# marekvinkler/NTrace

Hardware: AMD Instinct MI355X
Metric: Mrays/sec (primary + 8xAO) on Crytek Sponza (higher is better)
Workload: dtype f32

## Files before the change

include/ntrace_amd.h:

```cpp
#ifndef NTRACE_AMD_H
#define NTRACE_AMD_H

#include <stddef.h>
#include <stdint.h>

#ifdef __cplusplus
extern "C" {
#endif

#define NTR_API __attribute__((visibility("default")))

typedef enum NtrStatus {
    NTR_OK = 0,
    NTR_ERR_INVALID = -1,
    NTR_ERR_NO_DEVICE = -2,
    NTR_ERR_HIP = -3,
    NTR_ERR_LAYOUT = -4,
    NTR_ERR_UNKNOWN_KERNEL = -5,
    NTR_ERR_OVERFLOW = -6,
    NTR_ERR_NOMEM = -7
} NtrStatus;

typedef enum NtrBVHLayout {
    NTR_BVHLayout_AOS_AOS = 0,
    NTR_BVHLayout_AOS_SOA,
    NTR_BVHLayout_SOA_AOS,
    NTR_BVHLayout_SOA_SOA,
    NTR_BVHLayout_Compact,
    NTR_BVHLayout_Compact2,
    NTR_BVHLayout_CPU,
    NTR_BVHLayout_Max
} NtrBVHLayout;

typedef struct NtrKernelConfig {
    int32_t bvhLayout;
    int32_t blockWidth;
    int32_t blockHeight;
    int32_t usePersistentThreads;
} NtrKernelConfig;

typedef struct NtrRay {
    float ox, oy, oz, tmin;
    float dx, dy, dz, tmax;
} NtrRay;

typedef struct NtrRayResult {
    int32_t id;
    float   t;
    int32_t padA;
    int32_t padB;
} NtrRayResult;


NTR_API const char* ntr_last_error(void);
NTR_API int         ntr_version(void);

NTR_API int ntr_device_count(int* count);
NTR_API int ntr_set_device(int device);
NTR_API int ntr_malloc(void** d_ptr, size_t bytes);
NTR_API int ntr_free(void* d_ptr);
NTR_API int ntr_memcpy_h2d(void* d_dst, const void* h_src, size_t bytes, void* stream);
NTR_API int ntr_memcpy_d2h(void* h_dst, const void* d_src, size_t bytes, void* stream);
NTR_API int ntr_memcpy_d2d(void* d_dst, const void* d_src, size_t bytes, void* stream);
NTR_API int ntr_memset(void* d_dst, int value, size_t bytes, void* stream);
NTR_API int ntr_stream_synchronize(void* stream);


NTR_API int ntr_query_config(const char* kernelName, NtrKernelConfig* config);

NTR_API int ntr_trace_bvh(const char* kernelName, int32_t numRays, int32_t anyHit,
                          const NtrRay* d_rays, NtrRayResult* d_results,
                          const void* d_nodes, int64_t nodesBytes,
                          const void* d_triWoop, int64_t triWoopBytes, const int32_t* d_triIndex,
                          int32_t layout, uint32_t bvhFlags, void* stream, float* seconds);

NTR_API int ntr_trace_status(void* stream, uint32_t* statusBits);

NTR_API int ntr_selftest_gather_rate(int64_t tableBytes, int32_t waves, int32_t lanesPerWave, int32_t steps, void* stream, float* seconds);

NTR_API int ntr_trace_graph_reserve(int32_t launches, int32_t numRays);
NTR_API int ntr_trace_graph_release_all(void);

NTR_API int ntr_stream_release(void* stream);

NTR_API int ntr_selftest_auto_hint_table(int32_t devices, int32_t keysPerDevice, int32_t rounds, int32_t* hintedLastRound);

typedef struct NtrTracePlan {
    int32_t variant;
    int32_t launchVariant;
    int32_t launchBlocks;
    int32_t numBlocks;
    int32_t orderBlocks;
    int32_t chunk, fetchThreshold, leafSwitchBelow, octant, flatFetch, uniformPrologue, splitSlice;
    int32_t numHeads, shardRays, numBlocksIncoherent;
    int32_t numBlocksDivergent;
    int32_t wholeWave;
    int32_t prefetchAfter;
    int32_t unified;
    int32_t minipool;
    int32_t poolKConst;
    int32_t poolKFromDevice;
    int32_t minipoolWide;
    int32_t hintable;
    int32_t useAutoHint;
    int32_t predictable;
    int32_t persistentOrder;
    int32_t probeOnRefresh;
    int32_t coherentRoute;
    int32_t persistentVariant, persistentBlocks, persistentFetchThreshold;
    int32_t perrayBlocks, perrayFetchThreshold;
} NtrTracePlan;
#define NTR_PLAN_FLAG_STATS 1
#define NTR_PLAN_FLAG_CAPTURING 2
#define NTR_PLAN_FLAG_CALLER_HINT 4
NTR_API int ntr_trace_plan(const char* kernelName, int32_t numRays, int32_t anyHit, uint64_t nodesAddr, int64_t nodesBytes,
                           uint64_t triWoopAddr, int64_t triWoopBytes, uint32_t bvhFlags, int32_t numCUs, int32_t flags,
                           NtrTracePlan* plan);
NTR_API int ntr_trace_plan_hint_step(int32_t valid, int32_t predicted, int32_t uses, int32_t out[3]);
NTR_API int ntr_trace_plan_certain(int32_t anyHit, int32_t out[2]);

NTR_API int ntr_tunables_reload(void);

typedef struct NtrSchedHint NtrSchedHint;
NTR_API int ntr_sched_hint_create(NtrSchedHint** out);
NTR_API int ntr_sched_hint_destroy(NtrSchedHint* hint);
NTR_API int ntr_sched_hint_reset(NtrSchedHint* hint);
NTR_API int ntr_trace_bvh_hinted(const char* kernelName, int32_t numRays, int32_t anyHit,
                                 const NtrRay* d_rays, NtrRayResult* d_results,
                                 const void* d_nodes, int64_t nodesBytes,
                                 const void* d_triWoop, int64_t triWoopBytes, const int32_t* d_triIndex,
                                 int32_t layout, uint32_t bvhFlags, void* stream, float* seconds,
                                 NtrSchedHint* hint);

NTR_API int ntr_sched_hint_predict(NtrSchedHint* hint, const uint32_t* d_blockCost, int32_t numBlocks, void* stream);
NTR_API int ntr_bvh_leaf_depths(const void* d_nodes, int64_t nodesBytes, const void* d_triWoop, int64_t triWoopBytes,
                                const int32_t* d_triIndex, int32_t numTris, int32_t* d_depthByTri, int32_t* levels, void* stream);
NTR_API int ntr_secondary_block_costs(const NtrRayResult* d_inResults, int32_t first, int32_t count, int32_t numSamples,
                                      const int32_t* d_depthByTri, int32_t numTris, uint32_t* d_blockCost, void* stream);

NTR_API int ntr_predict_block_costs(int32_t numRays, const NtrRay* d_rays, const void* d_nodes, int64_t nodesBytes,
                                    uint32_t* d_blockCost, void* stream);

NTR_API int ntr_predict_batch_coherence(int32_t numRays, const NtrRay* d_rays, const void* d_nodes, int64_t nodesBytes,
                                        uint32_t* d_out, void* stream);

NTR_API int ntr_predict_dispatch_order(int32_t numRays, const NtrRay* d_rays, const void* d_nodes, int64_t nodesBytes,
                                       uint32_t* d_order, uint32_t* d_word, void* stream);

typedef struct {
    int32_t numBlocks;
    int32_t device;
    int32_t uses;
    int32_t valid;
    int32_t predicted;
} NtrSchedHintState;
NTR_API int ntr_sched_hint_inspect(const NtrSchedHint* hint, NtrSchedHintState* state, uint32_t* h_order, uint32_t* h_cost, void* stream);

typedef struct NtrTraceStats {
    int64_t numRays;
    int64_t numInnerVisits;
    int64_t numTriTests;
    int64_t numLeafVisits;
    int64_t numHits;
} NtrTraceStats;

NTR_API int ntr_trace_bvh_stats(const char* kernelName, int32_t numRays, int32_t anyHit,
                                const NtrRay* d_rays, NtrRayResult* d_results,
                                const void* d_nodes, int64_t nodesBytes,
                                const void* d_triWoop, int64_t triWoopBytes, const int32_t* d_triIndex,
                                int32_t layout, uint32_t bvhFlags, void* stream, NtrTraceStats* stats);

#define NTR_BVH_FINITE 1u
#define NTR_BVH_FASTDIV 2u
#define NTR_BVH_NOTINY 4u
#define NTR_BVH_ORDERED 8u
#define NTR_BVH_WIDE_LEAVES 16u
#define NTR_BATCH_DIVERGENT 0x10000u
NTR_API int ntr_bvh_validate(const void* d_nodes, int64_t nodesBytes, uint32_t* flags, void* stream);

NTR_API int ntr_selftest_division(const float* d_x, int32_t nx, const float* d_d, int32_t nd,
                                  uint32_t* mismatches, void* stream);
NTR_API int ntr_selftest_division_hard(int32_t xExp, int32_t dExp, uint64_t* pairs, uint64_t* mismatches, void* stream);


NTR_API int ntr_pixel_table(int32_t w, int32_t h, int32_t* d_indexToPixel, int32_t* d_pixelToIndex, void* stream);

NTR_API int ntr_raygen_primary(NtrRay* d_rays, int32_t* d_idToSlot, int32_t* d_slotToID,
                               const int32_t* d_indexToPixel, const float origin[3],
                               const float nscreenToWorld[16], int32_t w, int32_t h, float maxDist,
                               uint32_t kernelSeed, void* stream);

NTR_API int ntr_raygen_ao(NtrRay* d_outRays, int32_t* d_outIDToSlot, int32_t* d_outSlotToID,
                          const NtrRay* d_inRays, const NtrRayResult* d_inResults,
                          const float* d_triNormals, int32_t firstInputSlot, int32_t numInputRays,
                          int32_t numSamples, float maxDist, uint32_t kernelSeed, void* stream);

NTR_API int ntr_raygen_shadow(NtrRay* d_outRays, int32_t* d_outIDToSlot, int32_t* d_outSlotToID, const NtrRay* d_inRays,
                              const NtrRayResult* d_inResults, int32_t firstInputSlot, int32_t numInputRays, int32_t numSamples,
                              const float lightPos[3], float lightRadius, uint32_t kernelSeed, void* stream);

NTR_API int ntr_count_hits(const NtrRayResult* d_results, int32_t numRays, int32_t* count, void* stream);


typedef struct NtrLbvhResult {
    int32_t numNodes, numLeaves, numLevels, pad;
    int64_t nodesBytes, triWoopBytes, triIndexBytes;
    float   seconds;
    float   mortonMs, sortMs, woopMs, emitMs, refitMs;
} NtrLbvhResult;

NTR_API int ntr_lbvh_capacity(int32_t numTris, int64_t* nodesBytes, int64_t* triWoopBytes, int64_t* triIndexBytes);

NTR_API int ntr_lbvh_build(int32_t numTris, const int32_t* d_triVtxIndex, int32_t numVerts, const float* d_vtxPos,
                           const float sceneMin[3], const float sceneMax[3], int32_t leafSize, float epsilon,
                           void* d_nodes, int64_t nodesCapacity, void* d_triWoop, int64_t triWoopCapacity,
                           int32_t* d_triIndex, int64_t triIndexCapacity, NtrLbvhResult* result, void* stream);

typedef struct NtrHlbvhResult {
    NtrLbvhResult lbvh;
    int32_t numClusters, topNodes, topLevels, pad;
    float   clusterMs, topMs, bottomMs, pad2;
} NtrHlbvhResult;

NTR_API int ntr_hlbvh_build(int32_t numTris, const int32_t* d_triVtxIndex, int32_t numVerts, const float* d_vtxPos,
                            const float sceneMin[3], const float sceneMax[3], int32_t leafSize, float epsilon, int32_t hlbvhBits,
                            void* d_nodes, int64_t nodesCapacity, void* d_triWoop, int64_t triWoopCapacity,
                            int32_t* d_triIndex, int64_t triIndexCapacity, NtrHlbvhResult* result, void* stream);

NTR_API int ntr_lbvh_release_workspace(void);

typedef struct NtrPersistentBvhParams {
    int32_t triLimit, triMaxLimit, maxDepth, pad;
    float   ci, ct, epsilon, pad2;
} NtrPersistentBvhParams;
typedef struct NtrPersistentBvhResult {
    int32_t numNodes, numLeaves, numLevels, maxDepth;
    int32_t medianFallbacks, costLeaves, depthLeaves, pad;
    int64_t nodesBytes, triWoopBytes, triIndexBytes;
    float   seconds;
    float   prepMs, levelsMs, emitMs;
} NtrPersistentBvhResult;
NTR_API int ntr_persistent_bvh_params_default(NtrPersistentBvhParams* params);
NTR_API int ntr_persistent_bvh_build(int32_t numTris, const int32_t* d_triVtxIndex, int32_t numVerts, const float* d_vtxPos,
                                     const float sceneMin[3], const float sceneMax[3], const NtrPersistentBvhParams* params,
                                     void* d_nodes, int64_t nodesCapacity, void* d_triWoop, int64_t triWoopCapacity,
                                     int32_t* d_triIndex, int64_t triIndexCapacity, NtrPersistentBvhResult* result, void* stream);
NTR_API int ntr_persistent_bvh_scratch_bytes(int64_t* bytes);

typedef struct NtrSahDeviceResult {
    int32_t numNodes, numLeaves, numLevels, maxDepth;
    int32_t numDropped, pad[3];
    int64_t nodesBytes, triWoopBytes, triIndexBytes;
    float   seconds;
    float   prepMs, sortMs, levelsMs, emitMs;
} NtrSahDeviceResult;
NTR_API int ntr_sah_device_build(int32_t numTris, const int32_t* d_triVtxIndex, int32_t numVerts, const float* d_vtxPos,
                                 int32_t minLeafSize, int32_t maxLeafSize, void* d_nodes, int64_t nodesCapacity, void* d_triWoop,
                                 int64_t triWoopCapacity, int32_t* d_triIndex, int64_t triIndexCapacity, NtrSahDeviceResult* result,
                                 void* stream);
NTR_API int ntr_sah_device_scratch_bytes(int64_t* bytes);

typedef struct NtrBvhRefitResult {
    int32_t numNodes, numLeaves, numRows, pad;
    float   seconds;
} NtrBvhRefitResult;
NTR_API int ntr_bvh_refit(void* d_nodes, int64_t nodesBytes, void* d_triWoop, int64_t triWoopBytes,
                          const int32_t* d_triIndex, int64_t triIndexBytes,
                          int32_t numTris, const int32_t* d_triVtxIndex, int32_t numVerts, const float* d_vtxPos,
                          float epsilon, float* d_sceneBox ,
                          NtrBvhRefitResult* result , void* stream);
NTR_API int ntr_bvh_refit_scratch_bytes(int64_t* bytes);

typedef struct NtrBvhOptimizeResult {
    int32_t passes, numNodes, numLeafLinks, pad;
    int32_t formed[8], rewritten[8];
    int32_t heightBefore[8], heightAfter[8];
    float   seconds;
} NtrBvhOptimizeResult;
NTR_API int ntr_bvh_optimize(void* d_nodes, int64_t nodesBytes, int32_t passes, NtrBvhOptimizeResult* result ,
                             void* stream);
NTR_API int ntr_bvh_optimize_scratch_bytes(int64_t* bytes);

typedef struct NtrBvhSahResult {
    float   sahCost;
    int32_t numNodes, numLeaves, numTris, height;
    float   seconds;
} NtrBvhSahResult;
NTR_API int ntr_bvh_sah_cost(const void* d_nodes, int64_t nodesBytes, const void* d_triWoop, int64_t triWoopBytes,
                             NtrBvhSahResult* result, void* stream);

typedef struct NtrBvhReorderResult {
    int64_t nodesBytes, triWoopBytes, triIndexBytes;
    int32_t numNodes, numLeaves, numRows, numDroppedSlots;
    float   seconds;
} NtrBvhReorderResult;
NTR_API int ntr_bvh_reorder(const void* d_nodes, int64_t nodesBytes, const void* d_triWoop, int64_t triWoopBytes,
                            const int32_t* d_triIndex, int64_t triIndexBytes,
                            void* d_outNodes, int64_t outNodesCapacity, void* d_outTriWoop, int64_t outTriWoopCapacity,
                            int32_t* d_outTriIndex, int64_t outTriIndexCapacity,
                            NtrBvhReorderResult* result, void* stream);
NTR_API int ntr_bvh_reorder_scratch_bytes(int64_t* bytes);

NTR_API int ntr_reconstruct(int32_t rayType, int32_t numRaysPerPrimary, int32_t firstPrimary, int32_t numPrimary,
                            const int32_t* d_primarySlotToID, const NtrRayResult* d_primaryResults,
                            const int32_t* d_batchIDToSlot, const NtrRayResult* d_batchResults,
                            const uint32_t* d_triMaterialColor, const uint32_t* d_triShadedColor,
                            uint32_t* d_pixels, void* stream);

NTR_API int ntr_ray_morton_sort(int32_t numRays, const NtrRay* d_inRays, const int32_t* d_inSlotToID,
                                NtrRay* d_outRays, int32_t* d_outIDToSlot, int32_t* d_outSlotToID,
                                void* stream, float* seconds);

typedef struct NtrDist NtrDist;
#define NTR_DIST_ID_BYTES 128
NTR_API int ntr_frame_shard(int32_t numPrimary, int32_t rank, int32_t world, int32_t align, int32_t* lo, int32_t* hi);
NTR_API int ntr_frame_ao_batches(int32_t lo, int32_t hi, int32_t samples, int32_t maxBatchRays, int32_t* first, int32_t* count,
                                 int32_t capacity, int32_t* numBatches);
NTR_API int ntr_dist_unique_id(char id[NTR_DIST_ID_BYTES]);
NTR_API int ntr_dist_init(const char id[NTR_DIST_ID_BYTES], int32_t rank, int32_t world, NtrDist** out);
NTR_API int ntr_dist_init_all(int32_t numDevices, const int32_t* devices, NtrDist** out );
NTR_API int ntr_dist_info(const NtrDist* dist, int32_t* rank, int32_t* world);
NTR_API int ntr_dist_destroy(NtrDist* dist);
NTR_API int ntr_dist_broadcast(NtrDist* dist, void* d_buf, int64_t bytes, int32_t root, void* stream);
NTR_API int ntr_dist_broadcast_bvh(NtrDist* dist, void* d_nodes, int64_t nodesBytes, void* d_triWoop, int64_t triWoopBytes,
                                   int32_t* d_triIndex, int64_t triIndexBytes, int32_t root, void* stream);
NTR_API int ntr_dist_gather_records(NtrDist* dist, const NtrRayResult* d_ownRecords, int32_t numPrimary, int32_t align,
                                    NtrRayResult* d_fullRecords, int32_t root, void* stream);
NTR_API int ntr_dist_gather_records_cuts(NtrDist* dist, const NtrRayResult* d_ownRecords, const int32_t* cuts ,
                                         NtrRayResult* d_fullRecords, int32_t root, void* stream);
NTR_API int ntr_dist_gather_pixels(NtrDist* dist, const uint32_t* d_ownPixels, const int32_t* d_slotToPixel, int32_t numPrimary,
                                   int32_t align, uint32_t* d_fullPixels, uint32_t* d_scratch, int32_t root, void* stream);


typedef struct NtrHostBvh NtrHostBvh;
typedef struct NtrHostBvhInfo {
    const void*    nodes;     int64_t nodesBytes;
    const void*    triWoop;   int64_t triWoopBytes;
    const int32_t* triIndex;  int64_t triIndexBytes;
    int32_t layout;
    int32_t numInnerNodes, numLeafNodes, maxDepth;
    float   buildSeconds;
} NtrHostBvhInfo;
NTR_API int  ntr_sah_build(int32_t numTris, const int32_t* triVtxIndex ,
                           int32_t numVerts, const float* vtxPos ,
                           int32_t minLeafSize, int32_t maxLeafSize, NtrHostBvh** out);
NTR_API int  ntr_host_bvh_info(const NtrHostBvh* bvh, NtrHostBvhInfo* info);
NTR_API void ntr_host_bvh_free(NtrHostBvh* bvh);

NTR_API int ntr_host_bvh_wrap(const void* nodes, int64_t nodesBytes, const void* triWoop, int64_t triWoopBytes,
                              const int32_t* triIndex, int64_t triIndexBytes, NtrHostBvh** out);

NTR_API int ntr_host_bvh_trace(const NtrHostBvh* bvh, int32_t numRays, int32_t anyHit, const NtrRay* rays,
                               NtrRayResult* results, int32_t* visibility, int32_t numVisibility, NtrTraceStats* stats);


#define NTR_KDTREE_SPATIAL_MEDIAN 0
#define NTR_KDTREE_SAH 1
typedef struct NtrHostKdtree NtrHostKdtree;
typedef struct NtrHostKdtreeInfo {
    const void*    nodes;     int64_t nodesBytes;
    const void*    triWoop;   int64_t triWoopBytes;
    const int32_t* triIndex;  int64_t triIndexBytes;
    float   sceneMin[3], sceneMax[3];
    float   delta;
    int32_t numInnerNodes, numLeafNodes, numEmptyLeaves, numTriRefs;
    int32_t maxDepth;
    float   percentDuplicates;
    float   buildSeconds;
} NtrHostKdtreeInfo;
NTR_API int  ntr_kdtree_build(int32_t builder, int32_t numTris, const int32_t* triVtxIndex ,
                              int32_t numVerts, const float* vtxPos , int32_t maxLeafSize, NtrHostKdtree** out);
NTR_API int  ntr_host_kdtree_info(const NtrHostKdtree* kdtree, NtrHostKdtreeInfo* info);
NTR_API void ntr_host_kdtree_free(NtrHostKdtree* kdtree);

NTR_API int  ntr_host_kdtree_wrap(const void* nodes, int64_t nodesBytes, const void* triWoop, int64_t triWoopBytes,
                                  const int32_t* triIndex, int64_t triIndexBytes, const float sceneMin[3], const float sceneMax[3],
                                  NtrHostKdtree** out);

NTR_API int ntr_trace_kdtree(int32_t numRays, int32_t anyHit, const float sceneMin[3], const float sceneMax[3],
                             const NtrRay* d_rays, NtrRayResult* d_results, const void* d_nodes, int64_t nodesBytes,
                             const void* d_triWoop, int64_t triWoopBytes, const int32_t* d_triIndex, int64_t triIndexBytes,
                             void* stream, float* seconds);

typedef struct NtrKdtreeDeviceParams {
    int32_t triLimit, triMaxLimit, failureCount, pad;
    float   depthK1, depthK2, ci, ct, failRq;
} NtrKdtreeDeviceParams;
typedef struct NtrDeviceKdtree NtrDeviceKdtree;
typedef struct NtrDeviceKdtreeInfo {
    const void*    nodes;     int64_t nodesBytes;
    const void*    triWoop;   int64_t triWoopBytes;
    const int32_t* triIndex;  int64_t triIndexBytes;
    float   sceneMin[3], sceneMax[3], delta;
    int32_t numInnerNodes, numLeafNodes, numEmptyLeaves, numTriRefs;
    int32_t maxDepth;
    int32_t numLevels;
    float   percentDuplicates;
    float   seconds;
    float   prepMs, levelsMs, emitMs;
} NtrDeviceKdtreeInfo;
NTR_API int  ntr_kdtree_device_params_default(NtrKdtreeDeviceParams* params);
NTR_API int  ntr_kdtree_device_build(int32_t numTris, const int32_t* d_triVtxIndex, int32_t numVerts, const float* d_vtxPos,
                                     const NtrKdtreeDeviceParams* params, NtrDeviceKdtree** out, void* stream);
NTR_API int  ntr_device_kdtree_info(const NtrDeviceKdtree* tree, NtrDeviceKdtreeInfo* info);
NTR_API void ntr_device_kdtree_free(NtrDeviceKdtree* tree);
NTR_API int  ntr_kdtree_device_scratch_bytes(int64_t* bytes);
NTR_API int  ntr_device_kdtree_download(const NtrDeviceKdtree* tree, void* nodes, void* triWoop, int32_t* triIndex);


NTR_API int ntr_camera_decode(const char* signature, float out[16]);
NTR_API int ntr_camera_reencode(const char* signature, char* out, int32_t outSize);
NTR_API int ntr_camera_nscreen_to_world(const char* signature, int32_t viewW, int32_t viewH, float matrix[16],
                                        float position[3], float* cameraFar);

typedef struct NtrObjMesh NtrObjMesh;
NTR_API int  ntr_obj_load(const char* path, NtrObjMesh** out, int32_t* numTris, int32_t* numVerts, int32_t* numSubmeshes);
NTR_API int  ntr_obj_get(const NtrObjMesh* mesh, int32_t* triVtxIndex , float* vtxPos );
NTR_API void ntr_obj_free(NtrObjMesh* mesh);

#ifdef __cplusplus
}
#endif
#endif
```

ntrace_amd/__init__.py:

```python
from ._capi import (BvhView, RAY_DTYPE, RESULT_DTYPE, HostBvh, KernelConfig, NtrError, TraceStats, bvh_validate, lib,
                    lib_path, query_config, sah_build, trace_bvh, trace_bvh_stats, pixel_table,
                    raygen_primary, raygen_ao, raygen_shadow, count_hits, selftest_division, selftest_division_hard, bvh_leaf_depths, secondary_block_costs, lbvh_capacity,
                    lbvh_build, LbvhResult, hlbvh_build, HlbvhResult, reconstruct, ray_morton_sort, camera_decode, camera_reencode,
                    camera_nscreen_to_world, obj_load, SchedHint, trace_status, trace_plan, trace_plan_hint_step, trace_plan_certain, TracePlan, set_tunables, host_bvh_wrap, use_library, trace_graph_reserve, trace_graph_release_all, stream_release, selftest_auto_hint_table, selftest_gather_rate, frame_shard, frame_ao_batches, DistGroup,
                    lbvh_release_workspace, predict_block_costs, predict_batch_coherence, predict_dispatch_order, SchedHintState,
                    HostKdtree, kdtree_build, host_kdtree_wrap, trace_kdtree, KDTREE_SPATIAL_MEDIAN, KDTREE_SAH,
                    DeviceKdtree, KdtreeDeviceParams, kdtree_device_build, kdtree_device_params, KDTREE_DEVICE_DEFAULTS,
                    kdtree_device_scratch_bytes, PersistentBvhParams, PersistentBvhResult, persistent_bvh_params,
                    persistent_bvh_build, persistent_bvh_scratch_bytes, PERSISTENT_BVH_DEFAULTS, SahDeviceResult,
                    sah_device_build, sah_device_scratch_bytes, BvhRefitResult, bvh_refit,
                    bvh_refit_scratch_bytes, BvhOptimizeResult, BvhSahResult, bvh_optimize, bvh_optimize_scratch_bytes, bvh_sah_cost,
                    BvhReorderResult, bvh_reorder, bvh_reorder_scratch_bytes)

BVHLayout_Compact = 4
BVH_FINITE, BVH_FASTDIV, BVH_NOTINY, BVH_ORDERED, BVH_WIDE_LEAVES = 1, 2, 4, 8, 16
KERNELS = ("fermi_speculative_while_while", "tesla_persistent_while_while",
           "tesla_persistent_speculative_while_while", "kepler_dynamic_fetch")

__all__ = ["BvhView", "RAY_DTYPE", "RESULT_DTYPE", "HostBvh", "KernelConfig", "NtrError", "bvh_validate", "lib",
           "lib_path", "query_config", "sah_build", "trace_bvh", "trace_bvh_stats", "TraceStats", "pixel_table", "raygen_primary", "raygen_ao", "count_hits", "selftest_division", "selftest_division_hard", "bvh_leaf_depths", "secondary_block_costs", "lbvh_capacity", "lbvh_build", "LbvhResult", "hlbvh_build", "HlbvhResult", "reconstruct", "ray_morton_sort", "camera_decode", "camera_reencode", "camera_nscreen_to_world", "obj_load", "SchedHint", "trace_status", "set_tunables", "host_bvh_wrap", "BVHLayout_Compact", "KERNELS",
           "HostKdtree", "kdtree_build", "host_kdtree_wrap", "trace_kdtree", "KDTREE_SPATIAL_MEDIAN", "KDTREE_SAH",
           "DeviceKdtree", "KdtreeDeviceParams", "kdtree_device_build", "kdtree_device_params", "KDTREE_DEVICE_DEFAULTS",
           "kdtree_device_scratch_bytes", "PersistentBvhParams", "PersistentBvhResult", "persistent_bvh_params",
           "persistent_bvh_build", "persistent_bvh_scratch_bytes", "PERSISTENT_BVH_DEFAULTS", "SahDeviceResult",
           "sah_device_build", "sah_device_scratch_bytes", "BvhRefitResult", "bvh_refit",
           "bvh_refit_scratch_bytes", "BvhOptimizeResult", "BvhSahResult", "bvh_optimize", "bvh_optimize_scratch_bytes",
           "bvh_sah_cost", "BvhReorderResult", "bvh_reorder", "bvh_reorder_scratch_bytes"]
```

ntrace_amd/_capi.py:

```python
import ctypes as C
import os

import numpy as np

_HERE = os.path.dirname(os.path.abspath(__file__))

RAY_DTYPE = np.dtype([("ox", "<f4"), ("oy", "<f4"), ("oz", "<f4"), ("tmin", "<f4"),
                      ("dx", "<f4"), ("dy", "<f4"), ("dz", "<f4"), ("tmax", "<f4")])
RESULT_DTYPE = np.dtype([("id", "<i4"), ("t", "<f4"), ("padA", "<i4"), ("padB", "<i4")])


class NtrError(RuntimeError):
    def __init__(self, code, msg):
        super().__init__("ntrace_amd error %d: %s" % (code, msg))
        self.code = code


class SchedHintState(C.Structure):
    _fields_ = [(n, C.c_int32) for n in ("numBlocks", "device", "uses", "valid", "predicted")]


class KernelConfig(C.Structure):
    _fields_ = [("bvhLayout", C.c_int32), ("blockWidth", C.c_int32), ("blockHeight", C.c_int32),
                ("usePersistentThreads", C.c_int32)]


class TraceStats(C.Structure):
    _fields_ = [("numRays", C.c_int64), ("numInnerVisits", C.c_int64), ("numTriTests", C.c_int64),
                ("numLeafVisits", C.c_int64), ("numHits", C.c_int64)]

    def algorithmic_bytes(self):
        return (48 * self.numRays + 64 * self.numInnerVisits + 48 * self.numTriTests
                + 16 * self.numLeafVisits + 4 * self.numHits)

    def as_dict(self):
        return {k: int(getattr(self, k)) for k, _ in self._fields_}


class LbvhResult(C.Structure):
    _fields_ = [("numNodes", C.c_int32), ("numLeaves", C.c_int32), ("numLevels", C.c_int32), ("pad", C.c_int32),
                ("nodesBytes", C.c_int64), ("triWoopBytes", C.c_int64), ("triIndexBytes", C.c_int64),
                ("seconds", C.c_float), ("mortonMs", C.c_float), ("sortMs", C.c_float), ("woopMs", C.c_float),
                ("emitMs", C.c_float), ("refitMs", C.c_float)]

    def as_dict(self):
        return {k: getattr(self, k) for k, _ in self._fields_ if k != "pad"}


class HlbvhResult(C.Structure):
    _fields_ = [("lbvh", LbvhResult), ("numClusters", C.c_int32), ("topNodes", C.c_int32), ("topLevels", C.c_int32),
                ("pad", C.c_int32), ("clusterMs", C.c_float), ("topMs", C.c_float), ("bottomMs", C.c_float), ("pad2", C.c_float)]

    def as_dict(self):
        d = self.lbvh.as_dict()
        d.update({k: getattr(self, k) for k, _ in self._fields_ if k not in ("lbvh", "pad", "pad2")})
        return d


class _HostBvhInfo(C.Structure):
    _fields_ = [("nodes", C.c_void_p), ("nodesBytes", C.c_int64), ("triWoop", C.c_void_p),
                ("triWoopBytes", C.c_int64), ("triIndex", C.c_void_p), ("triIndexBytes", C.c_int64),
                ("layout", C.c_int32), ("numInnerNodes", C.c_int32), ("numLeafNodes", C.c_int32),
                ("maxDepth", C.c_int32), ("buildSeconds", C.c_float)]


class _HostKdtreeInfo(C.Structure):
    _fields_ = [("nodes", C.c_void_p), ("nodesBytes", C.c_int64), ("triWoop", C.c_void_p),
                ("triWoopBytes", C.c_int64), ("triIndex", C.c_void_p), ("triIndexBytes", C.c_int64),
                ("sceneMin", C.c_float * 3), ("sceneMax", C.c_float * 3), ("delta", C.c_float),
                ("numInnerNodes", C.c_int32), ("numLeafNodes", C.c_int32), ("numEmptyLeaves", C.c_int32), ("numTriRefs", C.c_int32),
                ("maxDepth", C.c_int32), ("percentDuplicates", C.c_float), ("buildSeconds", C.c_float)]


class KdtreeDeviceParams(C.Structure):
    _fields_ = [("triLimit", C.c_int32), ("triMaxLimit", C.c_int32), ("failureCount", C.c_int32), ("pad", C.c_int32),
                ("depthK1", C.c_float), ("depthK2", C.c_float), ("ci", C.c_float), ("ct", C.c_float), ("failRq", C.c_float)]


class PersistentBvhParams(C.Structure):
    _fields_ = [("triLimit", C.c_int32), ("triMaxLimit", C.c_int32), ("maxDepth", C.c_int32), ("pad", C.c_int32),
                ("ci", C.c_float), ("ct", C.c_float), ("epsilon", C.c_float), ("pad2", C.c_float)]


class PersistentBvhResult(C.Structure):
    _fields_ = [("numNodes", C.c_int32), ("numLeaves", C.c_int32), ("numLevels", C.c_int32), ("maxDepth", C.c_int32),
                ("medianFallbacks", C.c_int32), ("costLeaves", C.c_int32), ("depthLeaves", C.c_int32), ("pad", C.c_int32),
                ("nodesBytes", C.c_int64), ("triWoopBytes", C.c_int64), ("triIndexBytes", C.c_int64),
                ("seconds", C.c_float), ("prepMs", C.c_float), ("levelsMs", C.c_float), ("emitMs", C.c_float)]

    def as_dict(self):
        return {k: getattr(self, k) for k, _ in self._fields_ if k != "pad"}


class SahDeviceResult(C.Structure):
    _fields_ = [("numNodes", C.c_int32), ("numLeaves", C.c_int32), ("numLevels", C.c_int32), ("maxDepth", C.c_int32),
                ("numDropped", C.c_int32), ("pad", C.c_int32 * 3),
                ("nodesBytes", C.c_int64), ("triWoopBytes", C.c_int64), ("triIndexBytes", C.c_int64),
                ("seconds", C.c_float), ("prepMs", C.c_float), ("sortMs", C.c_float), ("levelsMs", C.c_float), ("emitMs", C.c_float)]

    def as_dict(self):
        return {k: getattr(self, k) for k, _ in self._fields_ if k != "pad"}


class BvhRefitResult(C.Structure):
    _fields_ = [("numNodes", C.c_int32), ("numLeaves", C.c_int32), ("numRows", C.c_int32), ("pad", C.c_int32), ("seconds", C.c_float)]

    def as_dict(self):
        return {k: getattr(self, k) for k, _ in self._fields_ if k != "pad"}


class BvhOptimizeResult(C.Structure):
    _fields_ = [("passes", C.c_int32), ("numNodes", C.c_int32), ("numLeafLinks", C.c_int32), ("pad", C.c_int32),
                ("formed", C.c_int32 * 8), ("rewritten", C.c_int32 * 8), ("heightBefore", C.c_int32 * 8), ("heightAfter", C.c_int32 * 8),
                ("seconds", C.c_float)]

    def as_dict(self):
        n = self.passes
        return {k: (list(getattr(self, k))[:n] if k in ("formed", "rewritten", "heightBefore", "heightAfter") else getattr(self, k))
                for k, _ in self._fields_ if k != "pad"}


class BvhReorderResult(C.Structure):
    _fields_ = [("nodesBytes", C.c_int64), ("triWoopBytes", C.c_int64), ("triIndexBytes", C.c_int64),
                ("numNodes", C.c_int32), ("numLeaves", C.c_int32), ("numRows", C.c_int32), ("numDroppedSlots", C.c_int32),
                ("seconds", C.c_float)]

    def as_dict(self):
        return {k: getattr(self, k) for k, _ in self._fields_}


class BvhSahResult(C.Structure):
    _fields_ = [("sahCost", C.c_float), ("numNodes", C.c_int32), ("numLeaves", C.c_int32), ("numTris", C.c_int32), ("height", C.c_int32),
                ("seconds", C.c_float)]

    def as_dict(self):
        return {k: getattr(self, k) for k, _ in self._fields_}


class _DeviceKdtreeInfo(C.Structure):
    _fields_ = [("nodes", C.c_void_p), ("nodesBytes", C.c_int64), ("triWoop", C.c_void_p),
                ("triWoopBytes", C.c_int64), ("triIndex", C.c_void_p), ("triIndexBytes", C.c_int64),
                ("sceneMin", C.c_float * 3), ("sceneMax", C.c_float * 3), ("delta", C.c_float),
                ("numInnerNodes", C.c_int32), ("numLeafNodes", C.c_int32), ("numEmptyLeaves", C.c_int32), ("numTriRefs", C.c_int32),
                ("maxDepth", C.c_int32), ("numLevels", C.c_int32), ("percentDuplicates", C.c_float), ("seconds", C.c_float),
                ("prepMs", C.c_float), ("levelsMs", C.c_float), ("emitMs", C.c_float)]


def lib_path():
    return os.environ.get("NTR_LIB_OVERRIDE") or os.path.join(_HERE, "libntrace_amd.so")


_lib = None
_libs = {}

_vp, _i32, _i64, _u32 = C.c_void_p, C.c_int32, C.c_int64, C.c_uint32
SYMBOLS = [
    ("ntr_last_error", C.c_char_p, []),
    ("ntr_version", C.c_int, []),
    ("ntr_device_count", C.c_int, [C.POINTER(C.c_int)]),
    ("ntr_set_device", C.c_int, [C.c_int]),
    ("ntr_malloc", C.c_int, [C.POINTER(_vp), C.c_size_t]),
    ("ntr_free", C.c_int, [_vp]),
    ("ntr_memcpy_h2d", C.c_int, [_vp, _vp, C.c_size_t, _vp]),
    ("ntr_memcpy_d2h", C.c_int, [_vp, _vp, C.c_size_t, _vp]),
    ("ntr_memcpy_d2d", C.c_int, [_vp, _vp, C.c_size_t, _vp]),
    ("ntr_memset", C.c_int, [_vp, C.c_int, C.c_size_t, _vp]),
    ("ntr_stream_synchronize", C.c_int, [_vp]),
    ("ntr_query_config", C.c_int, [C.c_char_p, C.POINTER(KernelConfig)]),
    ("ntr_trace_bvh", C.c_int, [C.c_char_p, _i32, _i32, _vp, _vp, _vp, _i64, _vp, _i64, _vp, _i32, _u32, _vp,
                                C.POINTER(C.c_float)]),
    ("ntr_trace_bvh_hinted", C.c_int, [C.c_char_p, _i32, _i32, _vp, _vp, _vp, _i64, _vp, _i64, _vp, _i32, _u32, _vp,
                                       C.POINTER(C.c_float), _vp]),
    ("ntr_trace_status", C.c_int, [_vp, C.POINTER(_u32)]),
    ("ntr_trace_plan", C.c_int, [C.c_char_p, _i32, _i32, C.c_uint64, _i64, C.c_uint64, _i64, _u32, _i32, _i32, _vp]),
    ("ntr_trace_plan_hint_step", C.c_int, [_i32, _i32, _i32, C.POINTER(_i32 * 3)]),
    ("ntr_trace_plan_certain", C.c_int, [_i32, C.POINTER(_i32 * 2)]),
    ("ntr_selftest_gather_rate", C.c_int, [_i64, _i32, _i32, _i32, _vp, C.POINTER(C.c_float)]),
    ("ntr_frame_shard", C.c_int, [_i32, _i32, _i32, _i32, C.POINTER(_i32), C.POINTER(_i32)]),
    ("ntr_frame_ao_batches", C.c_int, [_i32, _i32, _i32, _i32, C.POINTER(_i32), C.POINTER(_i32), _i32, C.POINTER(_i32)]),
    ("ntr_dist_unique_id", C.c_int, [C.c_char_p]),
    ("ntr_dist_init", C.c_int, [C.c_char_p, _i32, _i32, C.POINTER(_vp)]),
    ("ntr_dist_init_all", C.c_int, [_i32, C.POINTER(_i32), C.POINTER(_vp)]),
    ("ntr_dist_info", C.c_int, [_vp, C.POINTER(_i32), C.POINTER(_i32)]),
    ("ntr_dist_destroy", C.c_int, [_vp]),
    ("ntr_dist_broadcast", C.c_int, [_vp, _vp, _i64, _i32, _vp]),
    ("ntr_dist_broadcast_bvh", C.c_int, [_vp, _vp, _i64, _vp, _i64, _vp, _i64, _i32, _vp]),
    ("ntr_dist_gather_records", C.c_int, [_vp, _vp, _i32, _i32, _vp, _i32, _vp]),
    ("ntr_dist_gather_records_cuts", C.c_int, [_vp, _vp, C.POINTER(_i32), _vp, _i32, _vp]),
    ("ntr_dist_gather_pixels", C.c_int, [_vp, _vp, _vp, _i32, _i32, _vp, _vp, _i32, _vp]),
    ("ntr_tunables_reload", C.c_int, []),
    ("ntr_predict_block_costs", C.c_int, [_i32, _vp, _vp, _i64, _vp, _vp]),
    ("ntr_predict_batch_coherence", C.c_int, [_i32, _vp, _vp, _i64, _vp, _vp]),
    ("ntr_predict_dispatch_order", C.c_int, [_i32, _vp, _vp, _i64, _vp, _vp, _vp]),
    ("ntr_trace_graph_reserve", C.c_int, [_i32, _i32]),
    ("ntr_trace_graph_release_all", C.c_int, []),
    ("ntr_stream_release", C.c_int, [_vp]),
    ("ntr_selftest_auto_hint_table", C.c_int, [_i32, _i32, _i32, C.POINTER(_i32)]),
    ("ntr_lbvh_release_workspace", C.c_int, []),
    ("ntr_sched_hint_create", C.c_int, [C.POINTER(_vp)]),
    ("ntr_sched_hint_destroy", C.c_int, [_vp]),
    ("ntr_sched_hint_reset", C.c_int, [_vp]),
    ("ntr_sched_hint_predict", C.c_int, [_vp, _vp, _i32, _vp]),
    ("ntr_sched_hint_inspect", C.c_int, [_vp, _vp, _vp, _vp, _vp]),
    ("ntr_secondary_block_costs", C.c_int, [_vp, _i32, _i32, _i32, _vp, _i32, _vp, _vp]),
    ("ntr_bvh_leaf_depths", C.c_int, [_vp, _i64, _vp, _i64, _vp, _i32, _vp, C.POINTER(_i32), _vp]),
    ("ntr_selftest_division", C.c_int, [_vp, _i32, _vp, _i32, C.POINTER(_u32), _vp]),
    ("ntr_selftest_division_hard", C.c_int, [_i32, _i32, C.POINTER(C.c_uint64), C.POINTER(C.c_uint64), _vp]),
    ("ntr_trace_bvh_stats", C.c_int, [C.c_char_p, _i32, _i32, _vp, _vp, _vp, _i64, _vp, _i64, _vp, _i32, _u32, _vp,
                                      C.POINTER(TraceStats)]),
    ("ntr_bvh_validate", C.c_int, [_vp, _i64, C.POINTER(_u32), _vp]),
    ("ntr_pixel_table", C.c_int, [_i32, _i32, _vp, _vp, _vp]),
    ("ntr_raygen_primary", C.c_int, [_vp, _vp, _vp, _vp, C.POINTER(C.c_float), C.POINTER(C.c_float), _i32, _i32,
                                     C.c_float, _u32, _vp]),
    ("ntr_raygen_ao", C.c_int, [_vp, _vp, _vp, _vp, _vp, _vp, _i32, _i32, _i32, C.c_float, _u32, _vp]),
    ("ntr_raygen_shadow", C.c_int, [_vp, _vp, _vp, _vp, _vp, _i32, _i32, _i32, C.POINTER(C.c_float * 3), C.c_float, _u32, _vp]),
    ("ntr_count_hits", C.c_int, [_vp, _i32, C.POINTER(_i32), _vp]),
    ("ntr_lbvh_capacity", C.c_int, [_i32, C.POINTER(_i64), C.POINTER(_i64), C.POINTER(_i64)]),
    ("ntr_lbvh_build", C.c_int, [_i32, _vp, _i32, _vp, C.POINTER(C.c_float), C.POINTER(C.c_float), _i32, C.c_float,
                                 _vp, _i64, _vp, _i64, _vp, _i64, C.POINTER(LbvhResult), _vp]),
    ("ntr_hlbvh_build", C.c_int, [_i32, _vp, _i32, _vp, C.POINTER(C.c_float), C.POINTER(C.c_float), _i32, C.c_float, _i32,
                                  _vp, _i64, _vp, _i64, _vp, _i64, C.POINTER(HlbvhResult), _vp]),
    ("ntr_reconstruct", C.c_int, [_i32, _i32, _i32, _i32, _vp, _vp, _vp, _vp, _vp, _vp, _vp, _vp]),
    ("ntr_ray_morton_sort", C.c_int, [_i32, _vp, _vp, _vp, _vp, _vp, _vp, C.POINTER(C.c_float)]),
    ("ntr_camera_decode", C.c_int, [C.c_char_p, C.POINTER(C.c_float)]),
    ("ntr_camera_reencode", C.c_int, [C.c_char_p, C.c_char_p, _i32]),
    ("ntr_camera_nscreen_to_world", C.c_int, [C.c_char_p, _i32, _i32, C.POINTER(C.c_float), C.POINTER(C.c_float),
                                              C.POINTER(C.c_float)]),
    ("ntr_obj_load", C.c_int, [C.c_char_p, C.POINTER(_vp), C.POINTER(_i32), C.POINTER(_i32), C.POINTER(_i32)]),
    ("ntr_obj_get", C.c_int, [_vp, _vp, _vp]),
    ("ntr_obj_free", None, [_vp]),
    ("ntr_sah_build", C.c_int, [_i32, _vp, _i32, _vp, _i32, _i32, C.POINTER(_vp)]),
    ("ntr_host_bvh_info", C.c_int, [_vp, C.POINTER(_HostBvhInfo)]),
    ("ntr_host_bvh_free", None, [_vp]),
    ("ntr_host_bvh_wrap", C.c_int, [_vp, _i64, _vp, _i64, _vp, _i64, C.POINTER(_vp)]),
    ("ntr_host_bvh_trace", C.c_int, [_vp, _i32, _i32, _vp, _vp, _vp, _i32, C.POINTER(TraceStats)]),
    ("ntr_kdtree_build", C.c_int, [_i32, _i32, _vp, _i32, _vp, _i32, C.POINTER(_vp)]),
    ("ntr_kdtree_device_params_default", C.c_int, [C.POINTER(KdtreeDeviceParams)]),
    ("ntr_kdtree_device_build", C.c_int, [_i32, _vp, _i32, _vp, C.POINTER(KdtreeDeviceParams), C.POINTER(_vp), _vp]),
    ("ntr_device_kdtree_info", C.c_int, [_vp, C.POINTER(_DeviceKdtreeInfo)]),
    ("ntr_device_kdtree_free", None, [_vp]),
    ("ntr_device_kdtree_download", C.c_int, [_vp, _vp, _vp, _vp]),
    ("ntr_kdtree_device_scratch_bytes", C.c_int, [C.POINTER(_i64)]),
    ("ntr_persistent_bvh_params_default", C.c_int, [C.POINTER(PersistentBvhParams)]),
    ("ntr_persistent_bvh_build", C.c_int, [_i32, _vp, _i32, _vp, C.POINTER(C.c_float), C.POINTER(C.c_float), C.POINTER(PersistentBvhParams),
                                           _vp, _i64, _vp, _i64, _vp, _i64, C.POINTER(PersistentBvhResult), _vp]),
    ("ntr_persistent_bvh_scratch_bytes", C.c_int, [C.POINTER(_i64)]),
    ("ntr_sah_device_build", C.c_int, [_i32, _vp, _i32, _vp, _i32, _i32, _vp, _i64, _vp, _i64, _vp, _i64, C.POINTER(SahDeviceResult), _vp]),
    ("ntr_sah_device_scratch_bytes", C.c_int, [C.POINTER(_i64)]),
    ("ntr_bvh_refit", C.c_int, [_vp, _i64, _vp, _i64, _vp, _i64, _i32, _vp, _i32, _vp, C.c_float, _vp, C.POINTER(BvhRefitResult), _vp]),
    ("ntr_bvh_refit_scratch_bytes", C.c_int, [C.POINTER(_i64)]),
    ("ntr_bvh_optimize", C.c_int, [_vp, _i64, _i32, C.POINTER(BvhOptimizeResult), _vp]),
    ("ntr_bvh_optimize_scratch_bytes", C.c_int, [C.POINTER(_i64)]),
    ("ntr_bvh_sah_cost", C.c_int, [_vp, _i64, _vp, _i64, C.POINTER(BvhSahResult), _vp]),
    ("ntr_bvh_reorder", C.c_int, [_vp, _i64, _vp, _i64, _vp, _i64, _vp, _i64, _vp, _i64, _vp, _i64, C.POINTER(BvhReorderResult), _vp]),
    ("ntr_bvh_reorder_scratch_bytes", C.c_int, [C.POINTER(_i64)]),
    ("ntr_host_kdtree_info", C.c_int, [_vp, C.POINTER(_HostKdtreeInfo)]),
    ("ntr_host_kdtree_free", None, [_vp]),
    ("ntr_host_kdtree_wrap", C.c_int, [_vp, _i64, _vp, _i64, _vp, _i64, C.POINTER(C.c_float), C.POINTER(C.c_float), C.POINTER(_vp)]),
    ("ntr_trace_kdtree", C.c_int, [_i32, _i32, C.POINTER(C.c_float), C.POINTER(C.c_float), _vp, _vp, _vp, _i64, _vp, _i64, _vp, _i64,
                                   _vp, C.POINTER(C.c_float)]),
]


def _load(path):
    if path not in _libs:
        if not os.path.exists(path):
            raise ImportError("ntrace_amd: %s not found -- run `python -c 'import __graft_entry__ as g; g.build()'` "
                              "(the HIP extension is mandatory; there is no CPU fallback)" % path)
        try:
            import torch
        except ImportError:
            pass
        L = C.CDLL(path)
        for name, res, args in SYMBOLS:
            fn = getattr(L, name)
            fn.restype = res
            fn.argtypes = args
        _libs[path] = L
    return _libs[path]


def lib():
    global _lib
    if _lib is None:
        _lib = _load(lib_path())
    return _lib


def use_library(path=None):
    global _lib
    _lib = _load(path or lib_path())
    return _lib


def _check(rc):
    if rc != 0:
        raise NtrError(rc, (lib().ntr_last_error() or b"").decode("utf-8", "replace"))


def query_config(kernel):
    cfg = KernelConfig()
    _check(lib().ntr_query_config(kernel.encode(), C.byref(cfg)))
    return cfg


class SchedHint:

    def __init__(self):
        self._h = _vp()
        _check(lib().ntr_sched_hint_create(C.byref(self._h)))

    def reset(self):
        _check(lib().ntr_sched_hint_reset(self._h))

    def predict(self, d_block_cost, num_blocks, stream=0):
        _check(lib().ntr_sched_hint_predict(self._h, _vp(d_block_cost), int(num_blocks), _vp(stream)))

    def inspect(self, stream=0):
        st = SchedHintState()
        _check(lib().ntr_sched_hint_inspect(self._h, C.byref(st), None, None, _vp(stream)))
        out = {n: int(getattr(st, n)) for n, _ in st._fields_}
        if st.numBlocks > 0:
            order = np.zeros(st.numBlocks + 3, np.uint32)
            cost = np.zeros(st.numBlocks, np.uint32)
            _check(lib().ntr_sched_hint_inspect(self._h, C.byref(st), order.ctypes.data_as(_vp), cost.ctypes.data_as(_vp), _vp(stream)))
            out.update({n: int(getattr(st, n)) for n, _ in st._fields_})
            out["order"], out["words"], out["cost"] = order[:st.numBlocks], order[st.numBlocks:], cost
        return out

    def close(self):
        if self._h:
            lib().ntr_sched_hint_destroy(self._h)
            self._h = _vp()

    def __del__(self):
        try:
            self.close()
        except Exception:
            pass


def trace_bvh(kernel, num_rays, any_hit, d_rays, d_results, d_nodes, nodes_bytes, d_woop, woop_bytes, d_tri_index,
              layout=4, bvh_flags=0, stream=0, timed=True, hint=None):
    sec = C.c_float(0.0)
    args = (kernel.encode(), int(num_rays), int(bool(any_hit)), _vp(d_rays), _vp(d_results), _vp(d_nodes), int(nodes_bytes),
            _vp(d_woop), int(woop_bytes), _vp(d_tri_index), int(layout), int(bvh_flags), _vp(stream),
            C.byref(sec) if timed else None)
    if hint is None:
        _check(lib().ntr_trace_bvh(*args))
    else:
        _check(lib().ntr_trace_bvh_hinted(*args, hint._h))
    return float(sec.value) if timed else None


class TracePlan(C.Structure):
    _fields_ = [(n, C.c_int32) for n in (
        "variant", "launchVariant", "launchBlocks", "numBlocks", "orderBlocks", "chunk", "fetchThreshold", "leafSwitchBelow", "octant",
        "flatFetch", "uniformPrologue", "splitSlice", "numHeads", "shardRays", "numBlocksIncoherent", "numBlocksDivergent", "wholeWave", "prefetchAfter", "unified", "minipool", "poolKConst",
        "poolKFromDevice", "minipoolWide", "hintable", "useAutoHint", "predictable", "persistentOrder", "probeOnRefresh", "coherentRoute",
        "persistentVariant", "persistentBlocks", "persistentFetchThreshold", "perrayBlocks", "perrayFetchThreshold")]

    def as_dict(self):
        return {n: int(getattr(self, n)) for n, _ in self._fields_}


PLAN_FLAG_STATS, PLAN_FLAG_CAPTURING, PLAN_FLAG_CALLER_HINT = 1, 2, 4


def trace_plan(kernel, num_rays, any_hit, nodes_bytes, woop_bytes, nodes_addr=1 << 32, woop_addr=None, bvh_flags=0, num_cus=256, flags=0):
    if woop_addr is None:
        woop_addr = nodes_addr + nodes_bytes
    pl = TracePlan()
    _check(lib().ntr_trace_plan(kernel.encode(), int(num_rays), int(bool(any_hit)), int(nodes_addr), int(nodes_bytes), int(woop_addr),
                                int(woop_bytes), int(bvh_flags), int(num_cus), int(flags), C.byref(pl)))
    return pl


def trace_plan_hint_step(valid, predicted, uses):
    out = (_i32 * 3)()
    _check(lib().ntr_trace_plan_hint_step(int(bool(valid)), int(bool(predicted)), int(uses), C.byref(out)))
    return dict(zeroK=bool(out[0]), refresh=bool(out[1]), useOrder=bool(out[2]))


def trace_plan_certain(any_hit):
    out = (_i32 * 2)()
    _check(lib().ntr_trace_plan_certain(int(bool(any_hit)), C.byref(out)))
    return dict(certainSteps=bool(out[0]), certainDescent=bool(out[1]))


def trace_status(stream=0):
    bits = _u32(0)
    _check(lib().ntr_trace_status(_vp(stream), C.byref(bits)))
    return int(bits.value)


def selftest_gather_rate(table_bytes, waves, lanes_per_wave=64, steps=256, stream=0):
    sec = C.c_float(0.0)
    _check(lib().ntr_selftest_gather_rate(int(table_bytes), int(waves), int(lanes_per_wave), int(steps), _vp(stream), C.byref(sec)))
    return float(sec.value)


def frame_shard(num_primary, rank, world, align=64):
    lo, hi = _i32(0), _i32(0)
    _check(lib().ntr_frame_shard(int(num_primary), int(rank), int(world), int(align), C.byref(lo), C.byref(hi)))
    return int(lo.value), int(hi.value)


def frame_ao_batches(lo, hi, samples, max_batch_rays):
    n = _i32(0)
    _check(lib().ntr_frame_ao_batches(int(lo), int(hi), int(samples), int(max_batch_rays), None, None, 0, C.byref(n)))
    first, count = (_i32 * max(n.value, 1))(), (_i32 * max(n.value, 1))()
    _check(lib().ntr_frame_ao_batches(int(lo), int(hi), int(samples), int(max_batch_rays), first, count, n.value, C.byref(n)))
    return [(int(first[i]), int(count[i])) for i in range(n.value)]


class DistGroup:

    @staticmethod
    def unique_id():
        buf = C.create_string_buffer(128)
        _check(lib().ntr_dist_unique_id(buf))
        return buf.raw

    def __init__(self, uid, rank, world, _handle=None):
        if _handle is not None:
            self._h, self.rank, self.world = _handle, int(rank), int(world)
            return
        h = _vp()
        _check(lib().ntr_dist_init(C.c_char_p(uid), int(rank), int(world), C.byref(h)))
        self._h, self.rank, self.world = h, int(rank), int(world)

    @staticmethod
    def init_all(devices):
        n = len(devices)
        devs = (_i32 * n)(*[int(x) for x in devices])
        hs = (_vp * n)()
        _check(lib().ntr_dist_init_all(n, devs, hs))
        return [DistGroup(None, i, n, _handle=_vp(hs[i])) for i in range(n)]

    def broadcast(self, d_buf, nbytes, root=0, stream=0):
        _check(lib().ntr_dist_broadcast(self._h, _vp(d_buf), int(nbytes), int(root), _vp(stream)))

    def broadcast_bvh(self, d_nodes, nodes_bytes, d_woop, woop_bytes, d_tri_index, tri_index_bytes, root=0, stream=0):
        _check(lib().ntr_dist_broadcast_bvh(self._h, _vp(d_nodes), int(nodes_bytes), _vp(d_woop), int(woop_bytes), _vp(d_tri_index), int(tri_index_bytes),
                                            int(root), _vp(stream)))

    def gather_records(self, d_own, num_primary, d_full, root=0, stream=0, align=64):
        _check(lib().ntr_dist_gather_records(self._h, _vp(d_own), int(num_primary), int(align), _vp(d_full), int(root), _vp(stream)))

    def gather_records_cuts(self, d_own, cuts, d_full, root=0, stream=0):
        if len(cuts) != self.world + 1:
            raise ValueError("gather_records_cuts: %d cut points for %d ranks" % (len(cuts), self.world))
        c = (_i32 * (self.world + 1))(*[int(x) for x in cuts])
        _check(lib().ntr_dist_gather_records_cuts(self._h, _vp(d_own), c, _vp(d_full), int(root), _vp(stream)))

    def gather_pixels(self, d_own_pixels, d_slot_to_pixel, num_primary, d_full_pixels, d_scratch, root=0, stream=0, align=64):
        _check(lib().ntr_dist_gather_pixels(self._h, _vp(d_own_pixels), _vp(d_slot_to_pixel), int(num_primary), int(align), _vp(d_full_pixels), _vp(d_scratch),
                                            int(root), _vp(stream)))

    def close(self):
        if self._h:
            lib().ntr_dist_destroy(self._h)
            self._h = None


def predict_batch_coherence(num_rays, d_rays, d_nodes, nodes_bytes, d_out, stream=0):
    _check(lib().ntr_predict_batch_coherence(int(num_rays), _vp(d_rays), _vp(d_nodes), int(nodes_bytes), _vp(d_out), _vp(stream)))


def predict_dispatch_order(num_rays, d_rays, d_nodes, nodes_bytes, d_order, d_word, stream=0):
    _check(lib().ntr_predict_dispatch_order(int(num_rays), _vp(d_rays), _vp(d_nodes), int(nodes_bytes), _vp(d_order), _vp(d_word), _vp(stream)))


def predict_block_costs(num_rays, d_rays, d_nodes, nodes_bytes, d_block_cost, stream=0):
    _check(lib().ntr_predict_block_costs(int(num_rays), _vp(d_rays), _vp(d_nodes), int(nodes_bytes), _vp(d_block_cost), _vp(stream)))


def trace_graph_reserve(launches, num_rays):
    _check(lib().ntr_trace_graph_reserve(int(launches), int(num_rays)))


def trace_graph_release_all():
    _check(lib().ntr_trace_graph_release_all())


def stream_release(stream=0):
    _check(lib().ntr_stream_release(_vp(stream)))


def selftest_auto_hint_table(devices, keys_per_device, rounds=3):
    out = (_i32 * devices)()
    _check(lib().ntr_selftest_auto_hint_table(devices, keys_per_device, rounds, out))
    return [int(x) for x in out]


def lbvh_release_workspace():
    _check(lib().ntr_lbvh_release_workspace())


def set_tunables(**kv):
    for k, v in kv.items():
        if v is None:
            os.environ.pop(k, None)
        else:
            os.environ[k] = str(v)
    _check(lib().ntr_tunables_reload())


def bvh_leaf_depths(d_nodes, nodes_bytes, d_woop, woop_bytes, d_tri_index, num_tris, d_depth_by_tri, stream=0):
    m = _i32(0)
    _check(lib().ntr_bvh_leaf_depths(_vp(d_nodes), int(nodes_bytes), _vp(d_woop), int(woop_bytes), _vp(d_tri_index), int(num_tris),
                                     _vp(d_depth_by_tri), C.byref(m), _vp(stream)))
    return int(m.value)


def secondary_block_costs(d_in_results, first, count, num_samples, d_depth_by_tri, num_tris, d_block_cost, stream=0):
    _check(lib().ntr_secondary_block_costs(_vp(d_in_results), int(first), int(count), int(num_samples), _vp(d_depth_by_tri), int(num_tris),
                                           _vp(d_block_cost), _vp(stream)))


def selftest_division(d_x, nx, d_d, nd, stream=0):
    m = _u32(0)
    _check(lib().ntr_selftest_division(_vp(d_x), int(nx), _vp(d_d), int(nd), C.byref(m), _vp(stream)))
    return int(m.value)


def selftest_division_hard(x_exp, d_exp, stream=0):
    n, m = C.c_uint64(0), C.c_uint64(0)
    _check(lib().ntr_selftest_division_hard(int(x_exp), int(d_exp), C.byref(n), C.byref(m), _vp(stream)))
    return int(n.value), int(m.value)


def trace_bvh_stats(kernel, num_rays, any_hit, d_rays, d_results, d_nodes, nodes_bytes, d_woop, woop_bytes,
                    d_tri_index, layout=4, bvh_flags=0, stream=0):
    st = TraceStats()
    _check(lib().ntr_trace_bvh_stats(kernel.encode(), int(num_rays), int(bool(any_hit)), _vp(d_rays), _vp(d_results),
                                     _vp(d_nodes), int(nodes_bytes), _vp(d_woop), int(woop_bytes), _vp(d_tri_index),
                                     int(layout), int(bvh_flags), _vp(stream), C.byref(st)))
    return st


def bvh_validate(d_nodes, nodes_bytes, stream=0):
    flags = _u32(0)
    _check(lib().ntr_bvh_validate(_vp(d_nodes), int(nodes_bytes), C.byref(flags), _vp(stream)))
    return int(flags.value)


def pixel_table(w, h, d_index_to_pixel, d_pixel_to_index=0, stream=0):
    _check(lib().ntr_pixel_table(int(w), int(h), _vp(d_index_to_pixel), _vp(d_pixel_to_index), _vp(stream)))


def raygen_primary(d_rays, d_id_to_slot, d_slot_to_id, d_index_to_pixel, origin, nscreen_to_world, w, h, max_dist,
                   kernel_seed=0, stream=0):
    o = (C.c_float * 3)(*[float(x) for x in origin])
    m = (C.c_float * 16)(*[float(x) for x in np.asarray(nscreen_to_world, dtype=np.float32).reshape(-1)])
    _check(lib().ntr_raygen_primary(_vp(d_rays), _vp(d_id_to_slot), _vp(d_slot_to_id), _vp(d_index_to_pixel), o, m,
                                    int(w), int(h), float(max_dist), int(kernel_seed), _vp(stream)))


def raygen_ao(d_out_rays, d_out_id_to_slot, d_out_slot_to_id, d_in_rays, d_in_results, d_tri_normals, first_input_slot,
              num_input_rays, num_samples, max_dist, kernel_seed=0, stream=0):
    _check(lib().ntr_raygen_ao(_vp(d_out_rays), _vp(d_out_id_to_slot), _vp(d_out_slot_to_id), _vp(d_in_rays),
                               _vp(d_in_results), _vp(d_tri_normals), int(first_input_slot), int(num_input_rays),
                               int(num_samples), float(max_dist), int(kernel_seed), _vp(stream)))


def raygen_shadow(d_out_rays, d_out_id_to_slot, d_out_slot_to_id, d_in_rays, d_in_results, first_input_slot, num_input_rays, num_samples,
                  light_pos, light_radius, kernel_seed=0, stream=0):
    lp = (C.c_float * 3)(*[float(x) for x in light_pos])
    _check(lib().ntr_raygen_shadow(_vp(d_out_rays), _vp(d_out_id_to_slot), _vp(d_out_slot_to_id), _vp(d_in_rays), _vp(d_in_results),
                                   int(first_input_slot), int(num_input_rays), int(num_samples), C.byref(lp), float(light_radius),
                                   int(kernel_seed), _vp(stream)))


def count_hits(d_results, num_rays, stream=0):
    cnt = _i32(0)
    _check(lib().ntr_count_hits(_vp(d_results), int(num_rays), C.byref(cnt), _vp(stream)))
    return int(cnt.value)


def reconstruct(ray_type, rays_per_primary, first_primary, num_primary, d_primary_slot_to_id, d_primary_results,
                d_batch_id_to_slot, d_batch_results, d_tri_material_color, d_tri_shaded_color, d_pixels, stream=0):
    _check(lib().ntr_reconstruct(int(ray_type), int(rays_per_primary), int(first_primary), int(num_primary),
                                 _vp(d_primary_slot_to_id), _vp(d_primary_results), _vp(d_batch_id_to_slot),
                                 _vp(d_batch_results), _vp(d_tri_material_color), _vp(d_tri_shaded_color), _vp(d_pixels),
                                 _vp(stream)))


def ray_morton_sort(num_rays, d_in_rays, d_in_slot_to_id, d_out_rays, d_out_id_to_slot, d_out_slot_to_id, stream=0):
    sec = C.c_float(0.0)
    _check(lib().ntr_ray_morton_sort(int(num_rays), _vp(d_in_rays), _vp(d_in_slot_to_id), _vp(d_out_rays),
                                     _vp(d_out_id_to_slot), _vp(d_out_slot_to_id), _vp(stream), C.byref(sec)))
    return float(sec.value)


def lbvh_capacity(num_tris):
    a, b, c = _i64(0), _i64(0), _i64(0)
    _check(lib().ntr_lbvh_capacity(int(num_tris), C.byref(a), C.byref(b), C.byref(c)))
    return int(a.value), int(b.value), int(c.value)


def lbvh_build(num_tris, d_tri, num_verts, d_pos, scene_min, scene_max, leaf_size, epsilon, d_nodes, nodes_cap,
               d_woop, woop_cap, d_idx, idx_cap, stream=0):
    res = LbvhResult()
    mn = (C.c_float * 3)(*[float(x) for x in scene_min])
    mx = (C.c_float * 3)(*[float(x) for x in scene_max])
    _check(lib().ntr_lbvh_build(int(num_tris), _vp(d_tri), int(num_verts), _vp(d_pos), mn, mx, int(leaf_size),
                                float(epsilon), _vp(d_nodes), int(nodes_cap), _vp(d_woop), int(woop_cap), _vp(d_idx),
                                int(idx_cap), C.byref(res), _vp(stream)))
    return res


def hlbvh_build(num_tris, d_tri, num_verts, d_pos, scene_min, scene_max, leaf_size, epsilon, hlbvh_bits, d_nodes, nodes_cap,
                d_woop, woop_cap, d_idx, idx_cap, stream=0):
    res = HlbvhResult()
    mn = (C.c_float * 3)(*[float(x) for x in scene_min])
    mx = (C.c_float * 3)(*[float(x) for x in scene_max])
    _check(lib().ntr_hlbvh_build(int(num_tris), _vp(d_tri), int(num_verts), _vp(d_pos), mn, mx, int(leaf_size), float(epsilon),
                                 int(hlbvh_bits), _vp(d_nodes), int(nodes_cap), _vp(d_woop), int(woop_cap), _vp(d_idx), int(idx_cap),
                                 C.byref(res), _vp(stream)))
    return res


PERSISTENT_BVH_DEFAULTS = dict(triLimit=16, triMaxLimit=16, maxDepth=50, ci=1.0, ct=1.0, epsilon=float(np.finfo(np.float32).eps))


def persistent_bvh_params(**kw):
    p = PersistentBvhParams()
    _check(lib().ntr_persistent_bvh_params_default(C.byref(p)))
    for k, v in kw.items():
        if k not in PERSISTENT_BVH_DEFAULTS:
            raise TypeError("unknown persistent BVH parameter %r" % k)
        setattr(p, k, v)
    return p


def persistent_bvh_build(num_tris, d_tri, num_verts, d_pos, scene_min, scene_max, d_nodes, nodes_cap, d_woop, woop_cap, d_idx, idx_cap,
                         params=None, stream=0):
    if isinstance(params, dict):
        params = persistent_bvh_params(**params)
    res = PersistentBvhResult()
    mn = (C.c_float * 3)(*[float(x) for x in scene_min])
    mx = (C.c_float * 3)(*[float(x) for x in scene_max])
    _check(lib().ntr_persistent_bvh_build(int(num_tris), _vp(d_tri), int(num_verts), _vp(d_pos), mn, mx,
                                          C.byref(params) if params is not None else None, _vp(d_nodes), int(nodes_cap), _vp(d_woop),
                                          int(woop_cap), _vp(d_idx), int(idx_cap), C.byref(res), _vp(stream)))
    return res


def persistent_bvh_scratch_bytes():
    v = _i64(0)
    _check(lib().ntr_persistent_bvh_scratch_bytes(C.byref(v)))
    return int(v.value)


def sah_device_build(num_tris, d_tri, num_verts, d_pos, d_nodes, nodes_cap, d_woop, woop_cap, d_idx, idx_cap, min_leaf=1, max_leaf=1,
                     stream=0):
    res = SahDeviceResult()
    _check(lib().ntr_sah_device_build(int(num_tris), _vp(d_tri), int(num_verts), _vp(d_pos), int(min_leaf), int(max_leaf), _vp(d_nodes),
                                      int(nodes_cap), _vp(d_woop), int(woop_cap), _vp(d_idx), int(idx_cap), C.byref(res), _vp(stream)))
    return res


def sah_device_scratch_bytes():
    v = _i64(0)
    _check(lib().ntr_sah_device_scratch_bytes(C.byref(v)))
    return int(v.value)


def bvh_refit(d_nodes, nodes_bytes, d_woop, woop_bytes, d_idx, idx_bytes, num_tris, d_tri, num_verts, d_pos, epsilon=0.0, d_scene_box=0,
              stream=0, blocking=True):
    res = BvhRefitResult() if blocking else None
    _check(lib().ntr_bvh_refit(_vp(d_nodes), int(nodes_bytes), _vp(d_woop), int(woop_bytes), _vp(d_idx), int(idx_bytes), int(num_tris),
                               _vp(d_tri), int(num_verts), _vp(d_pos), float(epsilon), _vp(d_scene_box),
                               C.byref(res) if blocking else None, _vp(stream)))
    return res


def bvh_refit_scratch_bytes():
    v = _i64(0)
    _check(lib().ntr_bvh_refit_scratch_bytes(C.byref(v)))
    return int(v.value)


def bvh_optimize(d_nodes, nodes_bytes, passes=1, stream=0):
    res = BvhOptimizeResult()
    _check(lib().ntr_bvh_optimize(_vp(d_nodes), int(nodes_bytes), int(passes), C.byref(res), _vp(stream)))
    return res


def bvh_optimize_scratch_bytes():
    v = _i64(0)
    _check(lib().ntr_bvh_optimize_scratch_bytes(C.byref(v)))
    return int(v.value)


def bvh_reorder(d_nodes, nodes_bytes, d_woop, woop_bytes, d_idx, idx_bytes, d_out_nodes, out_nodes_capacity, d_out_woop, out_woop_capacity,
                d_out_idx, out_idx_capacity, stream=0, result=None):
    res = BvhReorderResult() if result is None else result
    _check(lib().ntr_bvh_reorder(_vp(d_nodes), int(nodes_bytes), _vp(d_woop), int(woop_bytes), _vp(d_idx), int(idx_bytes), _vp(d_out_nodes),
                                 int(out_nodes_capacity), _vp(d_out_woop), int(out_woop_capacity), _vp(d_out_idx), int(out_idx_capacity),
                                 C.byref(res), _vp(stream)))
    return res


def bvh_reorder_scratch_bytes():
    v = _i64(0)
    _check(lib().ntr_bvh_reorder_scratch_bytes(C.byref(v)))
    return int(v.value)


def bvh_sah_cost(d_nodes, nodes_bytes, d_woop, woop_bytes, stream=0):
    res = BvhSahResult()
    _check(lib().ntr_bvh_sah_cost(_vp(d_nodes), int(nodes_bytes), _vp(d_woop), int(woop_bytes), C.byref(res), _vp(stream)))
    return res


def camera_decode(signature):
    out = (C.c_float * 16)()
    _check(lib().ntr_camera_decode(signature.encode(), out))
    v = list(out)
    return dict(position=v[0:3], forward=v[3:6], up=v[6:9], speed=v[9], fov=v[10], near=v[11], far=v[12], keep_aligned=bool(v[13]))


def camera_reencode(signature):
    buf = C.create_string_buffer(256)
    _check(lib().ntr_camera_reencode(signature.encode(), buf, 256))
    return buf.value.decode()


def camera_nscreen_to_world(signature, w, h):
    m, p, f = (C.c_float * 16)(), (C.c_float * 3)(), C.c_float(0)
    _check(lib().ntr_camera_nscreen_to_world(signature.encode(), int(w), int(h), m, p, C.byref(f)))
    return np.array(list(m), dtype=np.float32).reshape(4, 4), np.array(list(p), dtype=np.float32), float(f.value)


def obj_load(path):
    h, nt_, nv, ns = _vp(), _i32(0), _i32(0), _i32(0)
    _check(lib().ntr_obj_load(path.encode(), C.byref(h), C.byref(nt_), C.byref(nv), C.byref(ns)))
    try:
        tri = np.zeros((nt_.value, 3), dtype=np.int32)
        pos = np.zeros((nv.value, 3), dtype=np.float32)
        _check(lib().ntr_obj_get(h, tri.ctypes.data_as(_vp), pos.ctypes.data_as(_vp)))
    finally:
        lib().ntr_obj_free(h)
    return tri, pos, int(ns.value)


class BvhView:

    def __init__(self, d_nodes, nodes_bytes, d_woop, woop_bytes, d_tri_index, flags=0, layout=4):
        self.d_nodes, self.nodes_bytes = int(d_nodes), int(nodes_bytes)
        self.d_woop, self.woop_bytes = int(d_woop), int(woop_bytes)
        self.d_tri_index, self.flags, self.layout = int(d_tri_index), int(flags), int(layout)

    def validate(self, stream=0):
        self.flags = bvh_validate(self.d_nodes, self.nodes_bytes, stream)
        return self.flags

    def trace(self, kernel, num_rays, any_hit, d_rays, d_results, stream=0, timed=True, flags=None, hint=None):
        return trace_bvh(kernel, num_rays, any_hit, d_rays, d_results, self.d_nodes, self.nodes_bytes, self.d_woop,
                         self.woop_bytes, self.d_tri_index, self.layout, self.flags if flags is None else flags,
                         stream, timed, hint)

    def trace_stats(self, kernel, num_rays, any_hit, d_rays, d_results, stream=0):
        return trace_bvh_stats(kernel, num_rays, any_hit, d_rays, d_results, self.d_nodes, self.nodes_bytes,
                               self.d_woop, self.woop_bytes, self.d_tri_index, self.layout, self.flags, stream)


class HostBvh:

    def __init__(self, nodes, woop, tri_index, info=None):
        self.nodes = nodes
        self.woop = woop
        self.tri_index = tri_index
        self.info = info or {}
        self.layout = 4
        self._h = None

    def host_trace(self, rays, any_hit=False, num_visibility=0, want_stats=False):
        if self._h is None:
            raise NtrError(-1, "host_trace needs sah_build(..., keep_handle=True)")
        rays = np.ascontiguousarray(rays)
        n = rays.shape[0]
        res = np.zeros(n, dtype=RESULT_DTYPE)
        vis = np.zeros(num_visibility, dtype=np.int32) if num_visibility else None
        st = TraceStats() if want_stats else None
        _check(lib().ntr_host_bvh_trace(self._h, n, int(bool(any_hit)), rays.ctypes.data_as(_vp), res.ctypes.data_as(_vp),
                                        vis.ctypes.data_as(_vp) if vis is not None else None, int(num_visibility),
                                        C.byref(st) if st is not None else None))
        return res, vis, st

    def close(self):
        if self._h is not None:
            lib().ntr_host_bvh_free(self._h)
            self._h = None

    def __del__(self):
        try:
            self.close()
        except Exception:
            pass


def host_bvh_wrap(nodes, woop, tri_index):
    nodes = np.ascontiguousarray(nodes).view(np.uint8).reshape(-1)
    woop = np.ascontiguousarray(woop).view(np.uint8).reshape(-1)
    tri_index = np.ascontiguousarray(tri_index, dtype=np.int32).reshape(-1)
    h = _vp()
    _check(lib().ntr_host_bvh_wrap(nodes.ctypes.data_as(_vp), nodes.nbytes, woop.ctypes.data_as(_vp), woop.nbytes,
                                   tri_index.ctypes.data_as(_vp), tri_index.nbytes, C.byref(h)))
    out = HostBvh(nodes.copy(), woop.copy(), tri_index.copy())
    out._h = h
    return out


def sah_build(tri_vtx_index, vtx_pos, min_leaf=1, max_leaf=1, keep_handle=False):
    tri = np.ascontiguousarray(tri_vtx_index, dtype=np.int32).reshape(-1, 3)
    pos = np.ascontiguousarray(vtx_pos, dtype=np.float32).reshape(-1, 3)
    h = _vp()
    _check(lib().ntr_sah_build(tri.shape[0], tri.ctypes.data_as(_vp), pos.shape[0], pos.ctypes.data_as(_vp),
                               int(min_leaf), int(max_leaf), C.byref(h)))
    try:
        info = _HostBvhInfo()
        _check(lib().ntr_host_bvh_info(h, C.byref(info)))
        nodes = np.ctypeslib.as_array(C.cast(info.nodes, C.POINTER(C.c_uint8)), (info.nodesBytes,)).copy()
        woop = np.ctypeslib.as_array(C.cast(info.triWoop, C.POINTER(C.c_uint8)), (info.triWoopBytes,)).copy()
        tidx = np.ctypeslib.as_array(C.cast(info.triIndex, C.POINTER(C.c_int32)), (info.triIndexBytes // 4,)).copy()
        meta = dict(numInnerNodes=info.numInnerNodes, numLeafNodes=info.numLeafNodes, maxDepth=info.maxDepth,
                    buildSeconds=float(info.buildSeconds))
    except Exception:
        lib().ntr_host_bvh_free(h)
        raise
    out = HostBvh(nodes, woop, tidx, meta)
    if keep_handle:
        out._h = h
    else:
        lib().ntr_host_bvh_free(h)
    return out


KDTREE_SPATIAL_MEDIAN, KDTREE_SAH = 0, 1
_KDTREE_BUILDERS = {"SpatialMedianKDTree": KDTREE_SPATIAL_MEDIAN, "SAHKDTree": KDTREE_SAH,
                    KDTREE_SPATIAL_MEDIAN: KDTREE_SPATIAL_MEDIAN, KDTREE_SAH: KDTREE_SAH}


def _f3(v):
    return (C.c_float * 3)(*[float(np.float32(x)) for x in v])


class HostKdtree:

    def __init__(self, nodes, woop, tri_index, scene_min, scene_max, delta, info=None):
        self.nodes = nodes
        self.woop = woop
        self.tri_index = tri_index
        self.scene_min = scene_min
        self.scene_max = scene_max
        self.delta = delta
        self.info = info or {}

    def trace(self, num_rays, any_hit, d_rays, d_results, d_nodes, d_woop, d_tri_index, stream=0, timed=True):
        return trace_kdtree(num_rays, any_hit, self.scene_min, self.scene_max, d_rays, d_results, d_nodes, self.nodes.nbytes,
                            d_woop, self.woop.nbytes, d_tri_index, self.tri_index.nbytes, stream, timed)


def _kdtree_from_handle(h):
    info = _HostKdtreeInfo()
    _check(lib().ntr_host_kdtree_info(h, C.byref(info)))
    nodes = np.ctypeslib.as_array(C.cast(info.nodes, C.POINTER(C.c_int32)), (info.nodesBytes // 4,)).copy().reshape(-1, 4)
    woop = np.ctypeslib.as_array(C.cast(info.triWoop, C.POINTER(C.c_uint8)), (info.triWoopBytes,)).copy()
    tidx = np.ctypeslib.as_array(C.cast(info.triIndex, C.POINTER(C.c_int32)), (info.triIndexBytes // 4,)).copy()
    meta = dict(numInnerNodes=info.numInnerNodes, numLeafNodes=info.numLeafNodes, numEmptyLeaves=info.numEmptyLeaves,
                numTriRefs=info.numTriRefs, maxDepth=info.maxDepth, percentDuplicates=float(info.percentDuplicates),
                buildSeconds=float(info.buildSeconds))
    return HostKdtree(nodes, woop, tidx, np.array(info.sceneMin[:], dtype=np.float32), np.array(info.sceneMax[:], dtype=np.float32),
                      np.float32(info.delta), meta)


def kdtree_build(tri_vtx_index, vtx_pos, builder="SAHKDTree", max_leaf=1):
    tri = np.ascontiguousarray(tri_vtx_index, dtype=np.int32).reshape(-1, 3)
    pos = np.ascontiguousarray(vtx_pos, dtype=np.float32).reshape(-1, 3)
    h = _vp()
    _check(lib().ntr_kdtree_build(_KDTREE_BUILDERS.get(builder, -1) if not isinstance(builder, int) else builder, tri.shape[0],
                                  tri.ctypes.data_as(_vp), pos.shape[0], pos.ctypes.data_as(_vp), int(max_leaf), C.byref(h)))
    try:
        return _kdtree_from_handle(h)
    finally:
        lib().ntr_host_kdtree_free(h)


def host_kdtree_wrap(nodes, woop, tri_index, scene_min, scene_max):
    nodes = np.ascontiguousarray(nodes).view(np.uint8).reshape(-1)
    woop = np.ascontiguousarray(woop).view(np.uint8).reshape(-1)
    tri_index = np.ascontiguousarray(tri_index, dtype=np.int32).reshape(-1)
    h = _vp()
    _check(lib().ntr_host_kdtree_wrap(nodes.ctypes.data_as(_vp), nodes.nbytes, woop.ctypes.data_as(_vp), woop.nbytes,
                                      tri_index.ctypes.data_as(_vp), tri_index.nbytes, _f3(scene_min), _f3(scene_max), C.byref(h)))
    try:
        return _kdtree_from_handle(h)
    finally:
        lib().ntr_host_kdtree_free(h)


def trace_kdtree(num_rays, any_hit, scene_min, scene_max, d_rays, d_results, d_nodes, nodes_bytes, d_woop, woop_bytes, d_tri_index,
                 tri_index_bytes, stream=0, timed=True):
    sec = C.c_float(0.0)
    _check(lib().ntr_trace_kdtree(int(num_rays), int(bool(any_hit)), _f3(scene_min), _f3(scene_max), _vp(d_rays), _vp(d_results),
                                  _vp(d_nodes), int(nodes_bytes), _vp(d_woop), int(woop_bytes), _vp(d_tri_index), int(tri_index_bytes),
                                  _vp(stream), C.byref(sec) if timed else None))
    return float(sec.value) if timed else None


KDTREE_DEVICE_DEFAULTS = dict(triLimit=16, triMaxLimit=16, failureCount=0, depthK1=1.2, depthK2=2.0, ci=1.0, ct=1.0, failRq=0.9)


def kdtree_device_params(**kw):
    p = KdtreeDeviceParams()
    _check(lib().ntr_kdtree_device_params_default(C.byref(p)))
    for k, v in kw.items():
        if k not in KDTREE_DEVICE_DEFAULTS:
            raise TypeError("unknown kd-tree parameter %r" % k)
        setattr(p, k, v)
    return p


class DeviceKdtree:

    def __init__(self, handle):
        self._h = handle
        info = _DeviceKdtreeInfo()
        _check(lib().ntr_device_kdtree_info(handle, C.byref(info)))
        for name, _ in _DeviceKdtreeInfo._fields_:
            v = getattr(info, name)
            setattr(self, name, v[:] if name in ("sceneMin", "sceneMax") else v)
        self.scene_min = np.array(info.sceneMin[:], dtype=np.float32)
        self.scene_max = np.array(info.sceneMax[:], dtype=np.float32)
        self.delta = np.float32(info.delta)

    @property
    def info(self):
        return {name: getattr(self, name) for name, _ in _DeviceKdtreeInfo._fields_}

    def trace(self, num_rays, any_hit, d_rays, d_results, stream=0, timed=True):
        if self._h is None:
            raise NtrError(-1, "DeviceKdtree: closed")
        return trace_kdtree(num_rays, any_hit, self.scene_min, self.scene_max, d_rays, d_results, self.nodes, self.nodesBytes,
                            self.triWoop, self.triWoopBytes, self.triIndex, self.triIndexBytes, stream, timed)

    def download(self):
        if self._h is None:
            raise NtrError(-1, "DeviceKdtree: closed")
        nodes = np.zeros(self.nodesBytes // 4, np.int32)
        woop = np.zeros(self.triWoopBytes, np.uint8)
        idx = np.zeros(self.triIndexBytes // 4, np.int32)
        _check(lib().ntr_device_kdtree_download(self._h, nodes.ctypes.data_as(_vp), woop.ctypes.data_as(_vp), idx.ctypes.data_as(_vp)))
        return nodes.reshape(-1, 4), woop, idx

    def close(self):
        if self._h is not None:
            lib().ntr_device_kdtree_free(self._h)
            self._h = None

    def __del__(self):
        try:
            self.close()
        except Exception:
            pass


def kdtree_device_scratch_bytes():
    v = _i64(0)
    _check(lib().ntr_kdtree_device_scratch_bytes(C.byref(v)))
    return int(v.value)


def kdtree_device_build(d_tri, num_tris, d_pos, num_verts, params=None, stream=0):
    if isinstance(params, dict):
        params = kdtree_device_params(**params)
    h = _vp()
    _check(lib().ntr_kdtree_device_build(int(num_tris), _vp(d_tri), int(num_verts), _vp(d_pos),
                                         C.byref(params) if params is not None else None, C.byref(h), _vp(stream)))
    return DeviceKdtree(h)
```

ntrace_amd/csrc/ntr_api.cpp:

```cpp

#include <hip/hip_runtime.h>

#include <cstdarg>
#include <cstdio>
#include <cstring>
#include <mutex>

#include "ntrace_amd.h"
#include "ntr_internal.h"
#include "compact_bvh.h"
#include "device_scratch.h"
#include "sched_state.h"
#include "trace_kernels.h"
#include "trace_plan.h"

namespace {

thread_local char g_err[512] = "";

}

namespace ntr {

int set_error(int code, const char* fmt, ...)
{
    va_list ap;
    va_start(ap, fmt);
    vsnprintf(g_err, sizeof(g_err), fmt, ap);
    va_end(ap);
    return code;
}

int hip_fail(hipError_t e, const char* what)
{
    int code = (e == hipErrorNoDevice || e == hipErrorInvalidDevice || e == hipErrorInsufficientDriver)
                   ? NTR_ERR_NO_DEVICE : NTR_ERR_HIP;
    return set_error(code, "%s: %s", what, hipGetErrorString(e));
}

bool stream_is_capturing(hipStream_t s)
{
    hipStreamCaptureStatus st = hipStreamCaptureStatusNone;
    if (hipStreamIsCapturing(s, &st) != hipSuccess) { (void)hipGetLastError(); return false; }
    return st != hipStreamCaptureStatusNone;
}

struct KernelInfo {
    const char* name;
    int variant;
    NtrKernelConfig cfg;
};

static const KernelInfo kKernels[] = {
    {"fermi_speculative_while_while", NTR_VARIANT_PERRAY,
     {NTR_BVHLayout_Compact, 64, 1, 0}},
    {"tesla_persistent_while_while", NTR_VARIANT_PERSISTENT,
     {NTR_BVHLayout_Compact, 64, NTR_TRACE_WAVES_PER_BLOCK, 1}},
    {"tesla_persistent_speculative_while_while", NTR_VARIANT_PERSISTENT,
     {NTR_BVHLayout_Compact, 64, NTR_TRACE_WAVES_PER_BLOCK, 1}},
    {"kepler_dynamic_fetch", NTR_VARIANT_PERSISTENT,
     {NTR_BVHLayout_Compact, 64, NTR_TRACE_WAVES_PER_BLOCK, 1}},
};

static const KernelInfo* find_kernel(const char* name)
{
    if (!name) return nullptr;
    for (const KernelInfo& k : kKernels)
        if (strcmp(k.name, name) == 0) return &k;
    return nullptr;
}

static TraceBatchDesc describe_batch(const KernelInfo* k, int32_t numRays, int32_t anyHit, uint64_t nodesAddr, int64_t nodesBytes,
                                     uint64_t woopAddr, int64_t triWoopBytes, uint32_t bvhFlags, bool wantStats, bool capturing,
                                     bool callerHint, int numCUs)
{
    TraceBatchDesc bd;
    bd.variant = k->variant; bd.dynamicFetch = strcmp(k->name, "kepler_dynamic_fetch") == 0;
    bd.numRays = numRays; bd.anyHit = anyHit != 0; bd.bvhFlags = bvhFlags;
    bd.nodesBytes = nodesBytes; bd.triWoopBytes = triWoopBytes;
    bd.nodesAddr = nodesAddr; bd.woopAddr = woopAddr;
    bd.wantStats = wantStats; bd.capturing = capturing; bd.callerHint = callerHint;
    bd.numCUs = numCUs;
    return bd;
}

struct TraceLaunch {
    TraceParams p{};
    TraceParams pp{};
    bool persistentSide = false, perraySide = false;
    NtrSchedHint* hint = nullptr;
    bool refresh = false;
    bool probeCoherence = false;
    TopTable* predTable = nullptr;
    PredictScratch* predScratch = nullptr;
};

static int bind_trace(DeviceState* ds, const Tunables& tun, const TracePlan& pl, bool capturing, int64_t nodesBytes, hipStream_t s,
                      NtrSchedHint* hint, TraceLaunch* L)
{
    TraceParams& p = L->p;
    const int variant = pl.variant, orderBlocks = pl.orderBlocks;
    int rc = NTR_OK;
    if (pl.useAutoHint) {
        rc = auto_hint_get(ds, p.rays, p.nodes, p.numRays, p.anyHit, s, orderBlocks, &hint);
        if (rc != NTR_OK) return rc;
    }
    L->hint = hint;
    if (hint && pl.hintable) {
        if (hint->numBlocks != orderBlocks || hint->device != ds->device) {
            rc = sched_hint_bind(hint, orderBlocks, ds->device, s);
            if (rc != NTR_OK) return rc;
        }
        const HintStep hs = plan_hint_step(tun, hint->valid, hint->predicted, hint->uses);
        if (hs.zeroK) {
            const hipError_t zk = ntr_launch_zero_words(hint->order + orderBlocks, 3, s);
            if (zk != hipSuccess) return hip_fail(zk, "zero_words launch");
        }
        L->refresh = hs.refresh;
        hint->predicted = false;
        hint->uses++;
        if (hs.useOrder) p.order = hint->order;
        if (L->refresh) {
            const hipError_t ze = ntr_launch_zero_words(hint->cost, orderBlocks, s);
            if (ze != hipSuccess) return hip_fail(ze, "zero_words launch");
            p.cost = hint->cost;
        }
    }

    if (pl.predictable && !(hint && hint->valid) && !p.order) {
        rc = top_table_get(ds, p.nodes, nodesBytes, s, false, &L->predTable);
        if (rc != NTR_OK) return rc;
        rc = predict_scratch_get(ds, s, orderBlocks, &L->predScratch);
        if (rc != NTR_OK) return rc;
        if (L->predScratch) p.order = (hint && pl.hintable) ? hint->order : L->predScratch->order;
        else L->predTable = nullptr;
    }

    L->probeCoherence = !L->predScratch && hint && L->refresh && pl.probeOnRefresh;
    if (L->probeCoherence) {
        rc = top_table_get(ds, p.nodes, nodesBytes, s, false, &L->predTable);
        if (rc != NTR_OK) return rc;
    }
    const unsigned int* word = nullptr;
    if (L->predScratch) word = L->predScratch->classCount + NTR_SCHED_PRED_CLASSES + 2;
    else if (hint && pl.hintable && hint->numBlocks == orderBlocks && hint->order) word = hint->order + orderBlocks + 2;
    const bool routed = pl.coherentRoute == 1 && word != nullptr;
    L->persistentSide = variant == NTR_VARIANT_PERSISTENT || routed;
    L->perraySide = variant != NTR_VARIANT_PERSISTENT || routed;
    if ((pl.minipool && pl.poolKFromDevice) || L->persistentSide) p.poolK = word;

    TraceParams& pp = L->pp = p;
    if (L->persistentSide) {
        rc = counter_set_take(ds, capturing, &pp.counter);
        if (rc != NTR_OK) return rc;
        pp.numBlocks = pl.persistentBlocks; pp.numBlocksIncoherent = pl.numBlocksIncoherent; pp.numBlocksDivergent = pl.numBlocksDivergent;
        pp.fetchThreshold = pl.persistentFetchThreshold;
        pp.shardRays = pl.shardRays;
        if (pp.order) {
            pp.orderBlocks = orderBlocks;
            pp.shardRays = ((orderBlocks + pp.numHeads - 1) / pp.numHeads) * 256;
        }
        pp.routeSkip = routed ? NTR_ROUTE_SKIP_COHERENT : 0;
    }
    if (routed) {
        p.routeSkip = NTR_ROUTE_SKIP_INCOHERENT;
        if (variant == NTR_VARIANT_PERSISTENT) { p.fetchThreshold = pl.perrayFetchThreshold; p.poolKConst = 1; }
    }
    return NTR_OK;
}

static int launch_trace(DeviceState* ds, const Tunables& tun, const TracePlan& pl, const TraceLaunch& L, hipStream_t s, float* seconds,
                        NtrTraceStats* stats)
{
    const TraceParams& p = L.p;
    NtrSchedHint* hint = L.hint;
    const int orderBlocks = pl.orderBlocks;
    StreamEvents<2> ev(s);
    if (seconds) {
        NTR_HIP(ev.create());
        NTR_HIP(hipStreamSynchronize(s));
        NTR_HIP(ev.record(0));
    }
    if (L.predScratch) {
        const hipError_t pe = ntr_launch_predict(p.rays, p.numRays, orderBlocks, L.predTable->table, L.predTable->count, L.predScratch->classCount,
                                                 L.predScratch->classList, (hint && pl.hintable) ? hint->order : L.predScratch->order,
                                                 (hint && pl.hintable) ? hint->order + orderBlocks + 2 : nullptr, pl.minipoolWide, s);
        if (pe != hipSuccess) return hip_fail(pe, "predict launch");
    } else if (L.probeCoherence) {
        const hipError_t ce = ntr_launch_coherence(p.rays, p.numRays, orderBlocks, L.predTable->table, L.predTable->count, hint->order + orderBlocks,
                                                  pl.minipoolWide, s);
        if (ce != hipSuccess) return hip_fail(ce, "coherence launch");
    }
    hipError_t le = hipSuccess;
    if (L.persistentSide) {
        le = ntr_launch_zero_words(L.pp.counter, kPoolHeadsMax * 16, s);
        if (le != hipSuccess) return hip_fail(le, "zero_words launch");
        le = ntr_launch_trace(pl.persistentVariant, &L.pp, pl.persistentBlocks, s);
        if (le != hipSuccess) return hip_fail(le, "trace_bvh launch");
    }
    if (L.perraySide) {
        le = pl.variant == NTR_VARIANT_PERSISTENT ? ntr_launch_trace(NTR_VARIANT_PERRAY_UNIFIED_MINI, &p, pl.perrayBlocks, s)
                                                  : ntr_launch_trace(pl.launchVariant, &p, pl.launchBlocks, s);
        if (le != hipSuccess) return hip_fail(le, "trace_bvh launch");
    }
    if (seconds) NTR_HIP(ev.record(1));
    if (L.refresh) {
        le = ntr_launch_sched_order(hint->cost, orderBlocks, tun.schedClasses, hint->order, 1, s);
        if (le != hipSuccess) return hip_fail(le, "sched_order launch");
        hint->valid = true;
    }
    if (seconds) {
        float ms = 0.0f;
        NTR_HIP(ev.elapsed(0, 1, &ms));
        *seconds = ms * 1e-3f;
        unsigned int st = 0;
        const int rc = status_fetch(ds, s, &st);
        if (rc != NTR_OK) return rc;
        if (st & NTR_STATUS_STACK_OVERFLOW) return set_error(NTR_ERR_OVERFLOW, "trace_bvh: traversal stack overflow");
    }
    if (stats) {
        unsigned long long h[4];
        NTR_HIP(hipMemcpyAsync(h, ds->stats, sizeof(h), hipMemcpyDeviceToHost, s));
        NTR_HIP(hipStreamSynchronize(s));
        stats->numRays = p.numRays;
        stats->numInnerVisits = (int64_t)h[0]; stats->numTriTests = (int64_t)h[1]; stats->numLeafVisits = (int64_t)h[2]; stats->numHits = (int64_t)h[3];
    }
    return NTR_OK;
}

static int32_t certain_steps_of(const Tunables& tun, bool anyHit) { return (tun.certainSteps >= 2 || (tun.certainSteps == 1 && anyHit)) ? 1 : 0; }

static int trace_impl(const char* kernelName, int32_t numRays, int32_t anyHit, const NtrRay* d_rays,
                      NtrRayResult* d_results, const void* d_nodes, int64_t nodesBytes, const void* d_triWoop,
                      int64_t triWoopBytes, const int32_t* d_triIndex, int32_t layout, uint32_t bvhFlags,
                      void* stream, float* seconds, NtrTraceStats* stats, NtrSchedHint* hint = nullptr)
{
    if (seconds) *seconds = 0.0f;
    if (stats) memset(stats, 0, sizeof(*stats));
    const KernelInfo* k = find_kernel(kernelName);
    if (!k) return set_error(NTR_ERR_UNKNOWN_KERNEL, "unknown kernel '%s'", kernelName ? kernelName : "(null)");
    if (numRays < 0) return set_error(NTR_ERR_INVALID, "ntr_trace_bvh: numRays < 0");
    if (numRays == 0) return NTR_OK;
    if (!d_nodes || !d_triWoop || !d_triIndex)
        return set_error(NTR_ERR_INVALID, "CudaBVHTracer: No BVH!");
    if (layout != k->cfg.bvhLayout)
        return set_error(NTR_ERR_LAYOUT, "CudaBVHTracer: Incorrect BVH layout!");
    if (!d_rays || !d_results) return set_error(NTR_ERR_INVALID, "ntr_trace_bvh: null ray/result buffer");
    int rc = check_nodes_bytes("ntr_trace_bvh", "node buffer size", nodesBytes);
    if (rc != NTR_OK) return rc;
    if (triWoopBytes < 16 || (triWoopBytes % 16) != 0 || triWoopBytes > 0xFFFFFFFFll)
        return set_error(NTR_ERR_INVALID, "ntr_trace_bvh: triWoop buffer size must be a multiple of 16 in [16, 4 GiB)");

    DeviceState* ds = nullptr;
    rc = current_device_state_ready(&ds);
    if (rc != NTR_OK) return rc;
    hipStream_t s = (hipStream_t)stream;

    const Tunables tun = tunables();
    const TraceBatchDesc bd = describe_batch(k, numRays, anyHit, (uint64_t)d_nodes, nodesBytes, (uint64_t)d_triWoop, triWoopBytes, bvhFlags,
                                             stats != nullptr, stream_is_capturing(s), hint != nullptr, ds->numCUs);
    const TracePlan pl = plan_trace(tun, bd);

    TraceLaunch L;
    TraceParams& p = L.p;
    p.numRays = numRays; p.anyHit = anyHit ? 1 : 0; p.rays = d_rays; p.results = d_results; p.bvhFlags = bvhFlags;
    p.nodes = d_nodes; p.woop = d_triWoop; p.triIndex = d_triIndex; p.nodesBytes = (uint32_t)nodesBytes; p.woopBytes = (uint32_t)triWoopBytes;
    p.status = ds->status; p.stats = ds->stats;
    p.numHeads = pl.numHeads; p.chunk = pl.chunk; p.fetchThreshold = pl.fetchThreshold; p.wholeWave = pl.wholeWave; p.prefetchAfter = pl.prefetchAfter;
    p.flatFetch = pl.flatFetch; p.uniformPrologue = pl.uniformPrologue; p.splitSlice = pl.splitSlice; p.leafSwitchBelow = pl.leafSwitchBelow;
    p.octant = pl.octant; p.poolKConst = pl.poolKConst;
    p.certainSteps = certain_steps_of(tun, anyHit != 0);
    p.certainDescent = tun.certainDescent != 0 ? 1 : 0;
    if (stats) NTR_HIP(hipMemsetAsync(ds->stats, 0, 4 * sizeof(unsigned long long), s));

    rc = bind_trace(ds, tun, pl, bd.capturing, nodesBytes, s, hint, &L);
    if (rc != NTR_OK) return rc;
    return launch_trace(ds, tun, pl, L, s, seconds, stats);
}

}

static int env_int(const char* name, int def)
{
    const char* v = getenv(name);
    return (v && *v) ? atoi(v) : def;
}

namespace ntr {
static Tunables g_tun;
static bool g_tunLoaded = false;
static std::mutex g_tunMu;

static void tunables_load_locked()
{
    Tunables t;
    t.chunk = env_int("NTR_TRACE_CHUNK", 64);
    t.fetchThreshold = env_int("NTR_TRACE_FETCH_THRESHOLD", -1);
    t.leafSwitchBelow = env_int("NTR_TRACE_LEAF_SWITCH", -1);
    t.blocksPerCU = env_int("NTR_TRACE_BLOCKS_PER_CU", 7);
    t.blocksPerCUIncoherent = env_int("NTR_TRACE_BLOCKS_PER_CU_INCOHERENT", 3);
    t.blocksPerCUDivergent = env_int("NTR_TRACE_BLOCKS_PER_CU_DIVERGENT", 4);
    t.octant = env_int("NTR_TRACE_OCTANT", 1);
    t.flatFetch = env_int("NTR_TRACE_FLAT_FETCH", 1);
    t.uniformPrologue = env_int("NTR_TRACE_UNIFORM_PROLOGUE", 1);
    t.certainSteps = env_int("NTR_TRACE_CERTAIN_STEPS", 1);
    t.certainDescent = env_int("NTR_TRACE_CERTAIN_DESCENT", 1);
    t.splitSlice = env_int("NTR_TRACE_SPLIT_SLICE", 8);
    t.wholeWave = env_int("NTR_TRACE_WHOLE_WAVE", 1);
    t.prefetchAfter = env_int("NTR_TRACE_PREFETCH_AFTER", 8);
    t.minipool = env_int("NTR_TRACE_MINIPOOL", -1);
    t.minipoolWide = env_int("NTR_TRACE_MINIPOOL_WIDE", -1);
    t.minipoolThreshold = env_int("NTR_TRACE_MINIPOOL_THRESHOLD", 48);
    t.unified = env_int("NTR_TRACE_UNIFIED", 1);
    t.poolHeads = env_int("NTR_TRACE_POOL_HEADS", 128);
    t.autoHint = env_int("NTR_TRACE_AUTO_HINT", 1);
    t.autoHintMinRays = env_int("NTR_TRACE_AUTO_HINT_MIN_RAYS", 1 << 17);
    t.route = env_int("NTR_TRACE_ROUTE", 1);
    t.persistentHints = env_int("NTR_TRACE_PERSISTENT_HINTS", 1);
    t.predict = env_int("NTR_TRACE_PREDICT", 1);
    t.predictPersistent = env_int("NTR_TRACE_PREDICT_PERSISTENT", 1);
    t.predictDepth = env_int("NTR_TRACE_PREDICT_DEPTH", 9);
    t.predictMinRays = env_int("NTR_TRACE_PREDICT_MIN_RAYS", 1 << 20);
    t.predictMinNodes = env_int("NTR_TRACE_PREDICT_MIN_NODES", 4096);
    t.schedRefreshEvery = env_int("NTR_SCHED_REFRESH_EVERY", 16);
    t.schedClasses = env_int("NTR_SCHED_CLASSES", 32);
    t.lbvhSplit = env_int("NTR_LBVH_SPLIT", 3072);
    t.lbvhAggLds = env_int("NTR_LBVH_AGG_LDS", 1);
    t.lbvhSortItems = env_int("NTR_LBVH_SORT_ITEMS", 0);
    t.lbvhAggStaged = env_int("NTR_LBVH_AGG_STAGED", -1);
    if (t.chunk < 1) t.chunk = 1;
    g_tun = t;
    g_tunLoaded = true;
}

Tunables tunables()
{
    std::lock_guard<std::mutex> lk(g_tunMu);
    if (!g_tunLoaded) tunables_load_locked();
    return g_tun;
}
}

extern "C" int ntr_tunables_reload(void)
{
    std::lock_guard<std::mutex> lk(ntr::g_tunMu);
    ntr::tunables_load_locked();
    return NTR_OK;
}


using namespace ntr;

extern "C" {

const char* ntr_last_error(void) { return g_err; }
int ntr_version(void) { return 100; }

int ntr_device_count(int* count)
{
    if (!count) return set_error(NTR_ERR_INVALID, "ntr_device_count: null argument");
    hipError_t e = hipGetDeviceCount(count);
    if (e != hipSuccess) { *count = 0; return hip_fail(e, "hipGetDeviceCount"); }
    return NTR_OK;
}

int ntr_set_device(int device) { NTR_HIP(hipSetDevice(device)); return NTR_OK; }

int ntr_malloc(void** d_ptr, size_t bytes)
{
    if (!d_ptr) return set_error(NTR_ERR_INVALID, "ntr_malloc: null argument");
    *d_ptr = nullptr;
    if (bytes == 0) return NTR_OK;
    NTR_HIP(hipMalloc(d_ptr, bytes));
    return NTR_OK;
}

int ntr_free(void* d_ptr)
{
    if (d_ptr) NTR_HIP(hipFree(d_ptr));
    return NTR_OK;
}

int ntr_memcpy_h2d(void* d, const void* h, size_t n, void* stream)
{
    if (n == 0) return NTR_OK;
    NTR_HIP(hipMemcpyAsync(d, h, n, hipMemcpyHostToDevice, (hipStream_t)stream));
    NTR_HIP(hipStreamSynchronize((hipStream_t)stream));
    return NTR_OK;
}

int ntr_memcpy_d2h(void* h, const void* d, size_t n, void* stream)
{
    if (n == 0) return NTR_OK;
    NTR_HIP(hipMemcpyAsync(h, d, n, hipMemcpyDeviceToHost, (hipStream_t)stream));
    NTR_HIP(hipStreamSynchronize((hipStream_t)stream));
    return NTR_OK;
}

int ntr_memcpy_d2d(void* dst, const void* src, size_t n, void* stream)
{
    if (n == 0) return NTR_OK;
    NTR_HIP(hipMemcpyAsync(dst, src, n, hipMemcpyDeviceToDevice, (hipStream_t)stream));
    return NTR_OK;
}

int ntr_memset(void* d, int value, size_t n, void* stream)
{
    if (n == 0) return NTR_OK;
    NTR_HIP(hipMemsetAsync(d, value, n, (hipStream_t)stream));
    return NTR_OK;
}

int ntr_stream_synchronize(void* stream)
{
    NTR_HIP(hipStreamSynchronize((hipStream_t)stream));
    return NTR_OK;
}

int ntr_query_config(const char* kernelName, NtrKernelConfig* config)
{
    if (!config) return set_error(NTR_ERR_INVALID, "ntr_query_config: null config");
    const KernelInfo* k = find_kernel(kernelName);
    if (!k) {
        config->bvhLayout = NTR_BVHLayout_Max;
        config->blockWidth = config->blockHeight = config->usePersistentThreads = 0;
        return set_error(NTR_ERR_UNKNOWN_KERNEL, "unknown kernel '%s'", kernelName ? kernelName : "(null)");
    }
    *config = k->cfg;
    return NTR_OK;
}

int ntr_trace_bvh(const char* kernelName, int32_t numRays, int32_t anyHit, const NtrRay* d_rays,
                  NtrRayResult* d_results, const void* d_nodes, int64_t nodesBytes, const void* d_triWoop,
                  int64_t triWoopBytes, const int32_t* d_triIndex, int32_t layout, uint32_t bvhFlags, void* stream,
                  float* seconds)
{
    return trace_impl(kernelName, numRays, anyHit, d_rays, d_results, d_nodes, nodesBytes, d_triWoop, triWoopBytes,
                      d_triIndex, layout, bvhFlags, stream, seconds, nullptr);
}

int ntr_trace_bvh_hinted(const char* kernelName, int32_t numRays, int32_t anyHit, const NtrRay* d_rays,
                         NtrRayResult* d_results, const void* d_nodes, int64_t nodesBytes, const void* d_triWoop,
                         int64_t triWoopBytes, const int32_t* d_triIndex, int32_t layout, uint32_t bvhFlags, void* stream,
                         float* seconds, NtrSchedHint* hint)
{
    return trace_impl(kernelName, numRays, anyHit, d_rays, d_results, d_nodes, nodesBytes, d_triWoop, triWoopBytes,
                      d_triIndex, layout, bvhFlags, stream, seconds, nullptr, hint);
}

int ntr_trace_plan(const char* kernelName, int32_t numRays, int32_t anyHit, uint64_t nodesAddr, int64_t nodesBytes, uint64_t triWoopAddr,
                   int64_t triWoopBytes, uint32_t bvhFlags, int32_t numCUs, int32_t flags, NtrTracePlan* plan)
{
    if (!plan) return set_error(NTR_ERR_INVALID, "ntr_trace_plan: null plan");
    memset(plan, 0, sizeof(*plan));
    const KernelInfo* k = find_kernel(kernelName);
    if (!k) return set_error(NTR_ERR_UNKNOWN_KERNEL, "unknown kernel '%s'", kernelName ? kernelName : "(null)");
    if (numRays < 0 || numCUs < 1 || nodesBytes < 0 || triWoopBytes < 0) return set_error(NTR_ERR_INVALID, "ntr_trace_plan: bad argument");
    const TraceBatchDesc bd = describe_batch(k, numRays, anyHit, nodesAddr, nodesBytes, triWoopAddr, triWoopBytes, bvhFlags,
                                             (flags & NTR_PLAN_FLAG_STATS) != 0, (flags & NTR_PLAN_FLAG_CAPTURING) != 0,
                                             (flags & NTR_PLAN_FLAG_CALLER_HINT) != 0, numCUs);
    *plan = plan_trace(tunables(), bd);
    return NTR_OK;
}

int ntr_trace_plan_certain(int32_t anyHit, int32_t out[2])
{
    if (!out) return set_error(NTR_ERR_INVALID, "ntr_trace_plan_certain: null argument");
    const Tunables tun = tunables();
    out[0] = certain_steps_of(tun, anyHit != 0); out[1] = tun.certainDescent != 0 ? 1 : 0;
    return NTR_OK;
}

int ntr_trace_plan_hint_step(int32_t valid, int32_t predicted, int32_t uses, int32_t out[3])
{
    if (!out || uses < 0) return set_error(NTR_ERR_INVALID, "ntr_trace_plan_hint_step: bad argument");
    const HintStep h = plan_hint_step(tunables(), valid != 0, predicted != 0, uses);
    out[0] = h.zeroK; out[1] = h.refresh; out[2] = h.useOrder;
    return NTR_OK;
}

int ntr_trace_status(void* stream, uint32_t* statusBits)
{
    if (statusBits) *statusBits = 0;
    unsigned int st = 0;
    DeviceState* ds = nullptr;
    int rc = current_device_state_ready(&ds);
    if (rc == NTR_OK) rc = status_fetch(ds, (hipStream_t)stream, &st);
    if (rc != NTR_OK) return rc;
    if (statusBits) *statusBits = st;
    if (st & NTR_STATUS_STACK_OVERFLOW)
        return set_error(NTR_ERR_OVERFLOW, "trace_bvh: traversal stack overflow in a launch since the last status check");
    return NTR_OK;
}

static int query_table(const char* fn, const void* d_nodes, int64_t nodesBytes, hipStream_t s, DeviceState** ds, TopTable** t)
{
    int rc = check_nodes_bytes(fn, "node buffer size", nodesBytes);
    if (rc == NTR_OK) rc = current_device_state(ds, "hipGetDevice(&dev)");
    if (rc == NTR_OK) rc = top_table_get(*ds, d_nodes, nodesBytes, s, false, t);
    return rc;
}

int ntr_predict_block_costs(int32_t numRays, const NtrRay* d_rays, const void* d_nodes, int64_t nodesBytes, uint32_t* d_blockCost, void* stream)
{
    if (numRays < 0) return set_error(NTR_ERR_INVALID, "ntr_predict_block_costs: numRays < 0");
    if (numRays == 0) return NTR_OK;
    if (!d_rays || !d_nodes || !d_blockCost) return set_error(NTR_ERR_INVALID, "ntr_predict_block_costs: null argument");
    DeviceState* ds = nullptr;
    TopTable* t = nullptr;
    const int rc = query_table("ntr_predict_block_costs", d_nodes, nodesBytes, (hipStream_t)stream, &ds, &t);
    if (rc != NTR_OK) return rc;
    const hipError_t e = ntr_launch_predict_costs(d_rays, numRays, (numRays + 255) / 256, t->table, t->count, d_blockCost, (hipStream_t)stream);
    if (e != hipSuccess) return hip_fail(e, "predict_costs launch");
    return NTR_OK;
}

int ntr_predict_batch_coherence(int32_t numRays, const NtrRay* d_rays, const void* d_nodes, int64_t nodesBytes, uint32_t* d_out, void* stream)
{
    if (numRays < 0) return set_error(NTR_ERR_INVALID, "ntr_predict_batch_coherence: numRays < 0");
    if (!d_out) return set_error(NTR_ERR_INVALID, "ntr_predict_batch_coherence: null argument");
    if (numRays > 0 && (!d_rays || !d_nodes)) return set_error(NTR_ERR_INVALID, "ntr_predict_batch_coherence: null argument");
    if (numRays == 0) {
        const unsigned int none[3] = {0u, 0u, 1u};
        NTR_HIP(hipMemcpyAsync(d_out, none, sizeof(none), hipMemcpyHostToDevice, (hipStream_t)stream));
        NTR_HIP(hipStreamSynchronize((hipStream_t)stream));
        return NTR_OK;
    }
    DeviceState* ds = nullptr;
    TopTable* t = nullptr;
    const int rc = query_table("ntr_predict_batch_coherence", d_nodes, nodesBytes, (hipStream_t)stream, &ds, &t);
    if (rc != NTR_OK) return rc;
    const hipError_t e = ntr_launch_coherence(d_rays, numRays, (numRays + 255) / 256, t->table, t->count, d_out, minipool_wide(tunables(), nodesBytes, numRays),
                                              (hipStream_t)stream);
    if (e != hipSuccess) return hip_fail(e, "coherence launch");
    return NTR_OK;
}

int ntr_predict_dispatch_order(int32_t numRays, const NtrRay* d_rays, const void* d_nodes, int64_t nodesBytes, uint32_t* d_order, uint32_t* d_word,
                               void* stream)
{
    if (numRays < 0) return set_error(NTR_ERR_INVALID, "ntr_predict_dispatch_order: numRays < 0");
    if (numRays == 0) return NTR_OK;
    if (!d_rays || !d_nodes || !d_order || !d_word) return set_error(NTR_ERR_INVALID, "ntr_predict_dispatch_order: null argument");
    hipStream_t s = (hipStream_t)stream;
    DeviceState* ds = nullptr;
    TopTable* t = nullptr;
    int rc = query_table("ntr_predict_dispatch_order", d_nodes, nodesBytes, s, &ds, &t);
    if (rc != NTR_OK) return rc;
    std::lock_guard<std::mutex> lk(ds->queryMu);
    const int numBlocks = (numRays + 255) / 256;
    PredictScratch* p = &ds->query;
    if (p->capBlocks < numBlocks && p->classList) NTR_HIP(hipStreamSynchronize(s));
    rc = scratch_alloc(p, numBlocks);
    if (rc != NTR_OK) return rc;
    const hipError_t e = ntr_launch_predict(d_rays, numRays, numBlocks, t->table, t->count, p->classCount, p->classList, d_order, d_word,
                                            minipool_wide(tunables(), nodesBytes, numRays), s);
    if (e != hipSuccess) return hip_fail(e, "predict launch");
    NTR_HIP(hipStreamSynchronize(s));
    return NTR_OK;
}

int ntr_secondary_block_costs(const NtrRayResult* d_inResults, int32_t first, int32_t count, int32_t numSamples, const int32_t* d_depthByTri,
                              int32_t numTris, uint32_t* d_blockCost, void* stream)
{
    if (first < 0 || count < 0 || numSamples < 1 || numTris < 0 || (count > 0 && (!d_inResults || !d_depthByTri || !d_blockCost)))
        return set_error(NTR_ERR_INVALID, "ntr_secondary_block_costs: bad argument");
    if (count == 0) return NTR_OK;
    hipStream_t s = (hipStream_t)stream;
    const int64_t blocks = ((int64_t)count * numSamples + 255) / 256;
    if (blocks > 0x7FFFFFFF) return set_error(NTR_ERR_INVALID, "ntr_secondary_block_costs: batch too large");
    hipError_t e = ntr_launch_zero_words(d_blockCost, (int)blocks, s);
    if (e == hipSuccess) e = ntr_launch_secondary_block_costs(d_inResults, first, count, numSamples, d_depthByTri, numTris, d_blockCost, s);
    if (e != hipSuccess) return hip_fail(e, "secondary_block_costs launch");
    return NTR_OK;
}

int ntr_bvh_leaf_depths(const void* d_nodes, int64_t nodesBytes, const void* d_triWoop, int64_t triWoopBytes, const int32_t* d_triIndex,
                        int32_t numTris, int32_t* d_depthByTri, int32_t* maxDepth, void* stream)
{
    if (maxDepth) *maxDepth = 0;
    if (!d_nodes || nodesBytes < 64 || (nodesBytes % 64) != 0 || nodesBytes > kMaxNodesBytes || !d_triWoop || triWoopBytes < 16 || !d_triIndex ||
        numTris < 1 || !d_depthByTri)
        return set_error(NTR_ERR_INVALID, "ntr_bvh_leaf_depths: bad argument");
    hipStream_t s = (hipStream_t)stream;
    const unsigned int capacity = (unsigned int)(nodesBytes / 64);
    unsigned int* d_q = nullptr;
    NTR_HIP(hipMalloc((void**)&d_q, (2 * (size_t)capacity + 2) * sizeof(unsigned int)));
    unsigned int* q[2] = {d_q, d_q + capacity};
    unsigned int* cnt = d_q + 2 * (size_t)capacity;
    hipError_t e = hipMemsetAsync(d_depthByTri, 0, (size_t)numTris * sizeof(int32_t), s);
    const unsigned int init[3] = {0u, 1u, 0u};
    if (e == hipSuccess) e = hipMemcpyAsync(q[0], &init[0], sizeof(unsigned int), hipMemcpyHostToDevice, s);
    if (e == hipSuccess) e = hipMemcpyAsync(cnt, &init[1], 2 * sizeof(unsigned int), hipMemcpyHostToDevice, s);
    int depth = 0;
    unsigned long long bound = 1;
    unsigned int frontier = 1;
    while (e == hipSuccess && frontier > 0 && depth < 4096) {
        const int in = depth & 1, out = in ^ 1;
        e = ntr_launch_zero_words(cnt + out, 1, s);
        const unsigned int threads = (unsigned int)(bound < capacity ? bound : capacity);
        if (e == hipSuccess)
            e = ntr_launch_leaf_depth_level(d_nodes, (unsigned int)nodesBytes, d_triWoop, (unsigned int)(triWoopBytes / 16), d_triIndex, numTris, q[in], cnt + in,
                                            q[out], cnt + out, capacity, threads, depth, d_depthByTri, s);
        depth++;
        bound = bound < capacity ? bound * 2 : bound;
        if ((depth & 3) == 0 && e == hipSuccess) {
            e = hipMemcpyAsync(&frontier, cnt + (depth & 1), sizeof(frontier), hipMemcpyDeviceToHost, s);
            if (e == hipSuccess) e = hipStreamSynchronize(s);
            if (frontier > capacity) frontier = capacity;
        }
    }
    if (e == hipSuccess) e = hipStreamSynchronize(s);
    (void)hipFree(d_q);
    if (e != hipSuccess) return hip_fail(e, "ntr_bvh_leaf_depths");
    if (depth >= 4096) return set_error(NTR_ERR_INVALID, "ntr_bvh_leaf_depths: the tree is deeper than 4096 levels (a cycle in the child references?)");
    if (maxDepth) *maxDepth = depth;
    return NTR_OK;
}

int ntr_trace_bvh_stats(const char* kernelName, int32_t numRays, int32_t anyHit, const NtrRay* d_rays,
                        NtrRayResult* d_results, const void* d_nodes, int64_t nodesBytes, const void* d_triWoop,
                        int64_t triWoopBytes, const int32_t* d_triIndex, int32_t layout, uint32_t bvhFlags,
                        void* stream, NtrTraceStats* stats)
{
    if (!stats) return set_error(NTR_ERR_INVALID, "ntr_trace_bvh_stats: null stats");
    return trace_impl(kernelName, numRays, anyHit, d_rays, d_results, d_nodes, nodesBytes, d_triWoop, triWoopBytes,
                      d_triIndex, layout, bvhFlags, stream, nullptr, stats);
}

int ntr_selftest_division(const float* d_x, int32_t nx, const float* d_d, int32_t nd, uint32_t* mismatches, void* stream)
{
    if (!mismatches || !d_x || !d_d || nx <= 0 || nd <= 0) return set_error(NTR_ERR_INVALID, "ntr_selftest_division: bad argument");
    hipStream_t s = (hipStream_t)stream;
    unsigned int* d_m = nullptr;
    NTR_HIP(hipMalloc((void**)&d_m, sizeof(unsigned int)));
    NTR_HIP(hipMemsetAsync(d_m, 0, sizeof(unsigned int), s));
    hipError_t le = ntr_launch_selftest_division(d_x, d_d, nx, nd, d_m, s);
    if (le != hipSuccess) return hip_fail(le, "selftest launch");
    unsigned int m = 0;
    NTR_HIP(hipMemcpyAsync(&m, d_m, sizeof(m), hipMemcpyDeviceToHost, s));
    NTR_HIP(hipStreamSynchronize(s));
    NTR_HIP(hipFree(d_m));
    *mismatches = m;
    return NTR_OK;
}

int ntr_selftest_division_hard(int32_t xExp, int32_t dExp, uint64_t* pairs, uint64_t* mismatches, void* stream)
{
    if (!pairs || !mismatches || xExp < -84 || xExp > 51 || dExp < -40 || dExp > 16)
        return set_error(NTR_ERR_INVALID, "ntr_selftest_division_hard: bad argument (x exponents in [-84, 51], d exponents in [-40, 16])");
    hipStream_t s = (hipStream_t)stream;
    unsigned long long* d_c = nullptr;
    NTR_HIP(hipMalloc((void**)&d_c, 2 * sizeof(unsigned long long)));
    hipError_t e = hipMemsetAsync(d_c, 0, 2 * sizeof(unsigned long long), s);
    if (e == hipSuccess) e = ntr_launch_selftest_division_hard(xExp, dExp, d_c, s);
    unsigned long long h[2] = {0, 0};
    if (e == hipSuccess) e = hipMemcpyAsync(h, d_c, sizeof(h), hipMemcpyDeviceToHost, s);
    if (e == hipSuccess) e = hipStreamSynchronize(s);
    (void)hipFree(d_c);
    if (e != hipSuccess) return hip_fail(e, "ntr_selftest_division_hard");
    *pairs = h[0];
    *mismatches = h[1];
    return NTR_OK;
}

}
```

ntrace_amd/csrc/ntr_internal.h:

```cpp
#pragma once
#include <hip/hip_runtime.h>

#include "ntrace_amd.h"

namespace ntr {
constexpr int kMaxDevices = 64;

int set_error(int code, const char* fmt, ...) __attribute__((format(printf, 2, 3)));
int hip_fail(hipError_t e, const char* what);

struct Tunables {
    int chunk, fetchThreshold, leafSwitchBelow, blocksPerCU, blocksPerCUIncoherent, blocksPerCUDivergent, poolHeads, octant, unified, flatFetch, uniformPrologue, certainSteps, certainDescent, splitSlice, wholeWave, prefetchAfter, minipool, minipoolThreshold, minipoolWide;
    int autoHint, autoHintMinRays, persistentHints, route, predict, predictPersistent, predictDepth, predictMinRays, predictMinNodes;
    int schedRefreshEvery, schedClasses;
    int lbvhSplit, lbvhAggLds, lbvhAggStaged, lbvhSortItems;
};
Tunables tunables();

bool stream_is_capturing(hipStream_t s);

size_t lbvh_sort_scratch_bytes(int n);
int lbvh_sort_codes(int n, const int32_t* d_tri, const float* d_pos, const float sceneMin[3], const float sceneMax[3], void* scratch,
                    hipStream_t s, const unsigned int** keys, const int** idx, const unsigned int** errWord);
}

extern "C" int ntr_top_table_refresh(const void* d_nodes, int64_t nodesBytes, void* stream);

#define NTR_HIP(call)                                            \
    do {                                                         \
        hipError_t _e = (call);                                  \
        if (_e != hipSuccess) return ::ntr::hip_fail(_e, #call); \
    } while (0)
```

ntrace_amd/csrc/sched_kernels.hip:

```cpp
#include <hip/hip_runtime.h>
#include <stdint.h>

#include "trace_kernels.h"

namespace ntr {

__global__ __launch_bounds__(256) void top_table_kernel(const float4* __restrict__ nodes, unsigned int nodesBytes, int depth,
                                                        float4* __restrict__ table, unsigned int* __restrict__ tableCount)
{
    __shared__ int s_q[2][1 << (NTR_TOP_DEPTH_MAX - 1)];
    __shared__ unsigned int s_cnt[2], s_out;
    const int tid = threadIdx.x;
    if (tid == 0) { s_q[0][0] = 0; s_cnt[0] = 1; s_cnt[1] = 0; s_out = 0; }
    __syncthreads();
    for (int d = 0; d < depth; d++) {
        const int cur = d & 1, nxt = cur ^ 1;
        const unsigned int n = s_cnt[cur];
        for (unsigned int e = tid; e < n; e += 256) {
            const unsigned int ofs = (unsigned int)s_q[cur][e];
            if (ofs + 64u > nodesBytes) continue;
            const float4* nd = nodes + (ofs >> 4);
            const float4 a = nd[0], b = nd[1], c = nd[2];
            const int4 ch = *reinterpret_cast<const int4*>(nd + 3);
            const unsigned int o = atomicAdd(&s_out, 2u);
            table[2 * o + 0] = a;
            table[2 * o + 1] = make_float4(c.x, c.y, 0.0f, 0.0f);
            table[2 * o + 2] = b;
            table[2 * o + 3] = make_float4(c.z, c.w, 0.0f, 0.0f);
            if (d + 1 < depth) {
                if (ch.x >= 0) s_q[nxt][atomicAdd(&s_cnt[nxt], 1u)] = ch.x;
                if (ch.y >= 0) s_q[nxt][atomicAdd(&s_cnt[nxt], 1u)] = ch.y;
            }
        }
        __syncthreads();
        if (tid == 0) s_cnt[cur] = 0;
        __syncthreads();
    }
    if (tid == 0) *tableCount = s_out;
}

constexpr int PRED_WAVES = 16;
constexpr int PRED_SAMPLE = 100;
constexpr int PRED_SAMPLE2 = 227;

__device__ __forceinline__ unsigned int block_incoherence(const float4* __restrict__ rays, int numRays, int block, const float4 o, const float4 d,
                                                          const float4* __restrict__ table)
{
    if (!(o.w < d.w)) return 8u;
    const int r2 = min(block * 256 + PRED_SAMPLE2, numRays - 1);
    const float4 o2 = rays[2 * r2], d2 = rays[2 * r2 + 1];
    const float4 a0 = table[0], a1 = table[1], b0 = table[2], b1 = table[3];
    const float ext = fmaxf(fmaxf(fmaxf(a0.y, b0.y) - fminf(a0.x, b0.x), fmaxf(a0.w, b0.w) - fminf(a0.z, b0.z)),
                            fmaxf(a1.y, b1.y) - fminf(a1.x, b1.x));
    const float dist = fmaxf(fmaxf(fabsf(o2.x - o.x), fabsf(o2.y - o.y)), fabsf(o2.z - o.z));
    if (dist > 0.125f * ext) return 1u;
    const float dot = d.x * d2.x + d.y * d2.y + d.z * d2.z;
    const float l1 = d.x * d.x + d.y * d.y + d.z * d.z, l2 = d2.x * d2.x + d2.y * d2.y + d2.z * d2.z;
    if (!(dot < 0.0f || 4.0f * dot * dot < l1 * l2)) return 0u;
    const float reach = (d.w - o.w) * (d.w - o.w) * l1;
    return reach > (0.125f * ext) * (0.125f * ext) ? 6u : 2u;
}

__global__ __launch_bounds__(PRED_WAVES * 64) void predict_kernel(const float4* __restrict__ rays, int numRays, int numBlocks,
                                                                  const float4* __restrict__ table,
                                                                  const unsigned int* __restrict__ tableCount,
                                                                  unsigned int* __restrict__ classCount, unsigned int* __restrict__ classList,
                                                                  unsigned int* __restrict__ blockCost )
{
    constexpr int PER_MAX = ((2 << NTR_TOP_DEPTH_MAX) + PRED_WAVES - 1) / PRED_WAVES;
    __shared__ float2 s_tab[PRED_WAVES][PER_MAX * 3];
    __shared__ unsigned int s_cnt[64];
    __shared__ unsigned int s_hist[NTR_SCHED_PRED_CLASSES], s_base[NTR_SCHED_PRED_CLASSES];
    const int tid = threadIdx.x, lane = tid & 63;
    const int wave = __builtin_amdgcn_readfirstlane(tid >> 6);
    const int block = blockIdx.x * 64 + lane;
    if (tid < 64) s_cnt[tid] = 0;
    if (tid < NTR_SCHED_PRED_CLASSES) s_hist[tid] = 0;
    const int nBoxes = (int)*tableCount;
    const int per = min((nBoxes + PRED_WAVES - 1) / PRED_WAVES, PER_MAX);
    const int b0 = wave * per, n = max(min(b0 + per, nBoxes) - b0, 0);
    for (int i = lane; i < n; i += 64) {
        const float4 xy = table[2 * (b0 + i)], z = table[2 * (b0 + i) + 1];
        s_tab[wave][3 * i + 0] = make_float2(xy.x, xy.y);
        s_tab[wave][3 * i + 1] = make_float2(xy.z, xy.w);
        s_tab[wave][3 * i + 2] = make_float2(z.x, z.y);
    }
    const int r = min(min(block, numBlocks - 1) * 256 + PRED_SAMPLE, numRays - 1);
    const float4 o = rays[2 * r], d = rays[2 * r + 1];
    const float ix = __frcp_rn(d.x), iy = __frcp_rn(d.y), iz = __frcp_rn(d.z);
    const float ax = -o.x * ix, ay = -o.y * iy, az = -o.z * iz;
    __syncthreads();
    unsigned int cnt = 0;
    const float2* tb = &s_tab[wave][0];
#pragma unroll 8
    for (int i = 0; i < n; i++) {
        const float2 bx = tb[3 * i], by = tb[3 * i + 1], bz = tb[3 * i + 2];
        const float x0 = fmaf(bx.x, ix, ax), x1 = fmaf(bx.y, ix, ax);
        const float y0 = fmaf(by.x, iy, ay), y1 = fmaf(by.y, iy, ay);
        const float z0 = fmaf(bz.x, iz, az), z1 = fmaf(bz.y, iz, az);
        const float tn = fmaxf(fmaxf(fminf(x0, x1), fminf(y0, y1)), fmaxf(fminf(z0, z1), o.w));
        const float tf = fminf(fminf(fmaxf(x0, x1), fmaxf(y0, y1)), fminf(fmaxf(z0, z1), d.w));
        cnt += (tn <= tf) ? 1u : 0u;
    }
    if (cnt) atomicAdd(&s_cnt[lane], cnt);
    __syncthreads();
    if (blockCost) {
        if (tid < 64 && block < numBlocks) blockCost[block] = s_cnt[lane];
        return;
    }
    if (wave == 0) {
        const unsigned int inc = (block < numBlocks && nBoxes >= 2) ? block_incoherence(rays, numRays, block, o, d, table) : 0u;
        const unsigned long long m1 = __ballot(inc == 1u), m2 = __ballot(inc == 6u), m3 = __ballot(inc == 8u);
        if (lane == 0 && m1) atomicAdd(&classCount[NTR_SCHED_PRED_CLASSES], (unsigned int)__popcll(m1));
        if (lane == 0 && (m2 | m3)) atomicAdd(&classCount[NTR_SCHED_PRED_CLASSES + 1], 4u * (unsigned int)__popcll(m2) + (unsigned int)__popcll(m3));
    }
    unsigned int cls = 0;
    if (tid < 64 && block < numBlocks) {
        cls = min(s_cnt[lane] >> 1, (unsigned int)(NTR_SCHED_PRED_CLASSES - 1));
        atomicAdd(&s_hist[cls], 1u);
        s_cnt[lane] = cls;
    }
    __syncthreads();
    if (tid < NTR_SCHED_PRED_CLASSES && s_hist[tid]) s_base[tid] = atomicAdd(&classCount[tid], s_hist[tid]);
    __syncthreads();
    if (tid < 64 && block < numBlocks) {
        unsigned int rank = 0;
        for (int j = 0; j < lane; j++) rank += (s_cnt[j] == cls) ? 1u : 0u;
        classList[(size_t)cls * numBlocks + s_base[cls] + rank] = (unsigned int)block;
    }
}

constexpr int FLATTEN_THREADS = 1024;

__device__ __forceinline__ unsigned int pool_k(unsigned int originApart, unsigned int divergenceScore, int numBlocks, int poolKWide)
{
    const unsigned int k = (originApart > 0u && 2u * originApart >= (unsigned int)numBlocks) ? (unsigned int)poolKWide : 1u;
    return k | ((numBlocks > 0 && 4u * originApart + divergenceScore >= (unsigned int)numBlocks) ? (unsigned int)NTR_BATCH_DIVERGENT : 0u);
}
__global__ __launch_bounds__(FLATTEN_THREADS) void flatten_kernel(unsigned int* __restrict__ classCount, const unsigned int* __restrict__ classList,
                                                                  int numBlocks, unsigned int* __restrict__ order,
                                                                  unsigned int* __restrict__ poolKCopy, int poolKWide)
{
    __shared__ unsigned int s_end[NTR_SCHED_PRED_CLASSES];
    const int tid = threadIdx.x;
    if (tid == 64) {
        const unsigned int k = pool_k(classCount[NTR_SCHED_PRED_CLASSES], classCount[NTR_SCHED_PRED_CLASSES + 1], numBlocks, poolKWide);
        classCount[NTR_SCHED_PRED_CLASSES] = 0;
        classCount[NTR_SCHED_PRED_CLASSES + 1] = 0;
        classCount[NTR_SCHED_PRED_CLASSES + 2] = k;
        if (poolKCopy) *poolKCopy = k;
    }
    if (tid < 64) {
        static_assert(NTR_SCHED_PRED_CLASSES == 64, "one class per lane");
        unsigned int incl = classCount[NTR_SCHED_PRED_CLASSES - 1 - tid];
#pragma unroll
        for (int off = 1; off < 64; off <<= 1) {
            const unsigned int u = (unsigned int)__shfl_up((int)incl, off);
            if (tid >= off) incl += u;
        }
        s_end[tid] = incl;
        classCount[NTR_SCHED_PRED_CLASSES - 1 - tid] = 0;
    }
    __syncthreads();
    for (int e = tid; e < numBlocks; e += FLATTEN_THREADS) {
        int k = 0;
#pragma unroll
        for (int step = 32; step > 0; step >>= 1)
            if (k + step <= NTR_SCHED_PRED_CLASSES - 1 && s_end[k + step - 1] <= (unsigned int)e) k += step;
        const unsigned int begin = k ? s_end[k - 1] : 0u;
        const int cls = NTR_SCHED_PRED_CLASSES - 1 - k;
        order[e] = classList[(size_t)cls * numBlocks + ((unsigned int)e - begin)];
    }
}

__global__ __launch_bounds__(256) void coherence_kernel(const float4* __restrict__ rays, int numRays, int numBlocks, const float4* __restrict__ table,
                                                        const unsigned int* __restrict__ tableCount, unsigned int* __restrict__ out)
{
    const int block = blockIdx.x * 256 + threadIdx.x;
    unsigned int inc = 0;
    if (block < numBlocks && *tableCount >= 2u) {
        const int r = min(block * 256 + PRED_SAMPLE, numRays - 1);
        inc = block_incoherence(rays, numRays, block, rays[2 * r], rays[2 * r + 1], table);
    }
    const unsigned long long m1 = __ballot(inc == 1u), m2 = __ballot(inc == 6u), m3 = __ballot(inc == 8u);
    if ((threadIdx.x & 63) == 0 && m1) atomicAdd(&out[0], (unsigned int)__popcll(m1));
    if ((threadIdx.x & 63) == 0 && (m2 | m3)) atomicAdd(&out[1], 4u * (unsigned int)__popcll(m2) + (unsigned int)__popcll(m3));
}
__global__ void coherence_finish_kernel(unsigned int* __restrict__ out, int numBlocks, int poolKWide)
{
    if (threadIdx.x == 0 && blockIdx.x == 0) out[2] = pool_k(out[0], out[1], numBlocks, poolKWide);
}

__global__ __launch_bounds__(256) void identity_order_kernel(unsigned int* __restrict__ order, int n)
{
    for (int i = blockIdx.x * 256 + threadIdx.x; i < n; i += gridDim.x * 256) order[i] = (unsigned int)i;
}

__global__ __launch_bounds__(256) void zero_words_kernel(unsigned int* __restrict__ p, int words)
{
    for (int i = blockIdx.x * 256 + threadIdx.x; i < words; i += gridDim.x * 256) p[i] = 0;
}

__global__ void status_exchange_kernel(unsigned int* __restrict__ status, unsigned int* __restrict__ out)
{
    if (threadIdx.x == 0 && blockIdx.x == 0) out[0] = atomicExch(status, 0u);
}

__global__ __launch_bounds__(256) void leaf_depth_level_kernel(const int4* __restrict__ nodes, unsigned int nodesBytes, const uint4* __restrict__ woop,
                                                               unsigned int woopVec4, const int* __restrict__ triIndex, int numTris,
                                                               const unsigned int* __restrict__ qin, const unsigned int* __restrict__ nIn,
                                                               unsigned int* __restrict__ qout, unsigned int* __restrict__ nOut, unsigned int capacity,
                                                               int depth, int* __restrict__ depthByTri)
{
    const unsigned int i = blockIdx.x * 256u + threadIdx.x;
    if (i >= *nIn) return;
    const unsigned int ofs = qin[i];
    if ((unsigned long long)ofs + 64ull > nodesBytes) return;
    const int4 ch = nodes[(ofs >> 4) + 3];
    const int c[2] = {ch.x, ch.y};
    for (int k = 0; k < 2; k++) {
        if (c[k] >= 0) {
            if ((c[k] & 63) == 0 && (unsigned int)c[k] != 0x76543210u) {
                const unsigned int slot = atomicAdd(nOut, 1u);
                if (slot < capacity) qout[slot] = (unsigned int)c[k];
            }
        } else {
            for (unsigned int a = (unsigned int)~c[k], guard = 0; a < woopVec4 && guard < 4096u; a += 3, guard++) {
                if (woop[a].x == 0x80000000u) break;
                const int t = triIndex[a];
                if (t >= 0 && t < numTris) depthByTri[t] = depth + 1;
            }
        }
    }
}

__global__ __launch_bounds__(256) void secondary_block_cost_kernel(const int4* __restrict__ inResults, int first, int count, int numSamples,
                                                                   const int* __restrict__ depthByTri, int numTris, unsigned int* __restrict__ blockCost)
{
    const int i = blockIdx.x * 256 + threadIdx.x;
    if (i >= count) return;
    const int id = inResults[first + i].x;
    const unsigned int d = (id >= 0 && id < numTris) ? (unsigned int)depthByTri[id] : 0u;
    if (d == 0u) return;
    const long long o0 = (long long)i * numSamples, o1 = o0 + numSamples - 1;
    for (long long b = o0 >> 8; b <= (o1 >> 8); b++) atomicMax(&blockCost[b], d);
}

}

extern "C" hipError_t ntr_launch_leaf_depth_level(const void* d_nodes, unsigned int nodesBytes, const void* d_woop, unsigned int woopVec4, const int* d_triIndex,
                                                  int numTris, const unsigned int* d_qin, const unsigned int* d_nIn, unsigned int* d_qout, unsigned int* d_nOut,
                                                  unsigned int capacity, unsigned int gridThreads, int depth, int* d_depthByTri, hipStream_t stream)
{
    if (gridThreads == 0) return hipSuccess;
    hipLaunchKernelGGL(ntr::leaf_depth_level_kernel, dim3((gridThreads + 255u) / 256u), dim3(256), 0, stream, (const int4*)d_nodes, nodesBytes,
                       (const uint4*)d_woop, woopVec4, d_triIndex, numTris, d_qin, d_nIn, d_qout, d_nOut, capacity, depth, d_depthByTri);
    return hipGetLastError();
}

extern "C" hipError_t ntr_launch_secondary_block_costs(const void* d_inResults, int first, int count, int numSamples, const int* d_depthByTri, int numTris,
                                                       unsigned int* d_blockCost, hipStream_t stream)
{
    if (count <= 0) return hipSuccess;
    hipLaunchKernelGGL(ntr::secondary_block_cost_kernel, dim3((count + 255) / 256), dim3(256), 0, stream, (const int4*)d_inResults, first, count, numSamples,
                       d_depthByTri, numTris, d_blockCost);
    return hipGetLastError();
}

extern "C" hipError_t ntr_launch_status_exchange(unsigned int* d_status, unsigned int* d_out, hipStream_t stream)
{
    hipLaunchKernelGGL(ntr::status_exchange_kernel, dim3(1), dim3(64), 0, stream, d_status, d_out);
    return hipGetLastError();
}

extern "C" hipError_t ntr_launch_top_table(const void* d_nodes, unsigned int nodesBytes, int depth, void* d_table,
                                           unsigned int* d_tableCount, hipStream_t stream)
{
    if (depth < 1) depth = 1;
    if (depth > NTR_TOP_DEPTH_MAX) depth = NTR_TOP_DEPTH_MAX;
    hipLaunchKernelGGL(ntr::top_table_kernel, dim3(1), dim3(256), 0, stream, (const float4*)d_nodes, nodesBytes, depth, (float4*)d_table,
                       d_tableCount);
    return hipGetLastError();
}

extern "C" hipError_t ntr_launch_predict(const void* d_rays, int numRays, int numBlocks, const void* d_table,
                                         const unsigned int* d_tableCount, unsigned int* d_classCount, unsigned int* d_classList,
                                         unsigned int* d_order, unsigned int* d_poolKCopy, int poolKWide, hipStream_t stream)
{
    const int grid = (numBlocks + 63) / 64;
    hipLaunchKernelGGL(ntr::predict_kernel, dim3(grid), dim3(ntr::PRED_WAVES * 64), 0, stream, (const float4*)d_rays, numRays, numBlocks,
                       (const float4*)d_table, d_tableCount, d_classCount, d_classList, (unsigned int*)nullptr);
    hipLaunchKernelGGL(ntr::flatten_kernel, dim3(1), dim3(ntr::FLATTEN_THREADS), 0, stream, d_classCount, (const unsigned int*)d_classList,
                       numBlocks, d_order, d_poolKCopy, poolKWide);
    return hipGetLastError();
}

extern "C" hipError_t ntr_launch_predict_costs(const void* d_rays, int numRays, int numBlocks, const void* d_table,
                                               const unsigned int* d_tableCount, unsigned int* d_blockCost, hipStream_t stream)
{
    const int grid = (numBlocks + 63) / 64;
    hipLaunchKernelGGL(ntr::predict_kernel, dim3(grid), dim3(ntr::PRED_WAVES * 64), 0, stream, (const float4*)d_rays, numRays, numBlocks,
                       (const float4*)d_table, d_tableCount, (unsigned int*)nullptr, (unsigned int*)nullptr, d_blockCost);
    return hipGetLastError();
}

extern "C" hipError_t ntr_launch_coherence(const void* d_rays, int numRays, int numBlocks, const void* d_table, const unsigned int* d_tableCount,
                                           unsigned int* d_out, int poolKWide, hipStream_t stream)
{
    hipLaunchKernelGGL(ntr::zero_words_kernel, dim3(1), dim3(256), 0, stream, d_out, 3);
    if (numBlocks > 0)
        hipLaunchKernelGGL(ntr::coherence_kernel, dim3((numBlocks + 255) / 256), dim3(256), 0, stream, (const float4*)d_rays, numRays, numBlocks,
                           (const float4*)d_table, d_tableCount, d_out);
    hipLaunchKernelGGL(ntr::coherence_finish_kernel, dim3(1), dim3(64), 0, stream, d_out, numBlocks, poolKWide);
    return hipGetLastError();
}

extern "C" hipError_t ntr_launch_identity_order(unsigned int* d_order, int numBlocks, hipStream_t stream)
{
    if (numBlocks <= 0) return hipSuccess;
    int grid = (numBlocks + 255) / 256;
    if (grid > 1024) grid = 1024;
    hipLaunchKernelGGL(ntr::identity_order_kernel, dim3(grid), dim3(256), 0, stream, d_order, numBlocks);
    return hipGetLastError();
}

extern "C" hipError_t ntr_launch_zero_words(void* d_ptr, int words, hipStream_t stream)
{
    if (words <= 0) return hipSuccess;
    int grid = (words + 255) / 256;
    if (grid > 1024) grid = 1024;
    hipLaunchKernelGGL(ntr::zero_words_kernel, dim3(grid), dim3(256), 0, stream, (unsigned int*)d_ptr, words);
    return hipGetLastError();
}

namespace ntr {

constexpr int SCHED_THREADS = 256;
constexpr int SCHED_MAX_CLASSES = 64;

template <int MAXC>
__global__ __launch_bounds__(SCHED_THREADS) void sched_order_kernel(const unsigned int* __restrict__ cost, int numBlocks, int classes,
                                                                    int keepIfAllZero, unsigned int* __restrict__ order)
{
    __shared__ unsigned int s_cnt[MAXC][SCHED_THREADS];
    __shared__ unsigned int s_tot[MAXC][SCHED_THREADS / 64];
    __shared__ unsigned int s_red[SCHED_THREADS / 64];
    const int tid = threadIdx.x, lane = tid & 63, wave = tid >> 6;
    const int seg = (numBlocks + SCHED_THREADS - 1) / SCHED_THREADS;
    const int b0 = min(tid * seg, numBlocks), b1 = min(b0 + seg, numBlocks);

    unsigned int mx = 0;
    for (int i = tid; i < numBlocks; i += SCHED_THREADS) mx = max(mx, cost[i]);
#pragma unroll
    for (int off = 32; off > 0; off >>= 1) mx = max(mx, (unsigned int)__shfl_xor((int)mx, off));
    if (lane == 0) s_red[wave] = mx;
    for (int c = 0; c < classes; c++) s_cnt[c][tid] = 0;
    __syncthreads();
    mx = 0;
    for (int w = 0; w < SCHED_THREADS / 64; w++) mx = max(mx, s_red[w]);
    if (keepIfAllZero && mx == 0u) return;
    const float toClass = (float)classes / ((float)mx + 1.0f);
    auto cls = [&](unsigned int c) { return (classes - 1) - min((int)((float)c * toClass), classes - 1); };

    for (int i = b0; i < b1; i++) s_cnt[cls(cost[i])][tid]++;
    __syncthreads();
    unsigned int v[MAXC], incl[MAXC];
#pragma unroll
    for (int c = 0; c < MAXC; c++) {
        v[c] = c < classes ? s_cnt[c][tid] : 0u;
        incl[c] = v[c];
    }
#pragma unroll
    for (int off = 1; off < 64; off <<= 1) {
#pragma unroll
        for (int c = 0; c < MAXC; c++) {
            const unsigned int u = (unsigned int)__shfl_up((int)incl[c], off);
            if (lane >= off) incl[c] += u;
        }
    }
    if (lane == 63) {
#pragma unroll
        for (int c = 0; c < MAXC; c++) s_tot[c][wave] = incl[c];
    }
    __syncthreads();
    unsigned int running = 0;
#pragma unroll
    for (int c = 0; c < MAXC; c++) {
        if (c < classes) {
            unsigned int before = 0, total = 0;
#pragma unroll
            for (int w = 0; w < SCHED_THREADS / 64; w++) {
                const unsigned int t = s_tot[c][w];
                if (w < wave) before += t;
                total += t;
            }
            s_cnt[c][tid] = running + before + incl[c] - v[c];
            running += total;
        }
    }
    for (int i = b0; i < b1; i++) {
        const int c = cls(cost[i]);
        order[s_cnt[c][tid]++] = (unsigned int)i;
    }
}

}

extern "C" hipError_t ntr_launch_sched_order(const unsigned int* d_cost, int numBlocks, int classes, unsigned int* d_order,
                                             int keepIfAllZero, hipStream_t stream)
{
    if (classes < 1) classes = 1;
    if (classes > ntr::SCHED_MAX_CLASSES) classes = ntr::SCHED_MAX_CLASSES;
    if (classes <= 32)
        hipLaunchKernelGGL(ntr::sched_order_kernel<32>, dim3(1), dim3(ntr::SCHED_THREADS), 0, stream, d_cost, numBlocks, classes, keepIfAllZero, d_order);
    else
        hipLaunchKernelGGL(ntr::sched_order_kernel<ntr::SCHED_MAX_CLASSES>, dim3(1), dim3(ntr::SCHED_THREADS), 0, stream, d_cost, numBlocks, classes, keepIfAllZero, d_order);
    return hipGetLastError();
}
```

ntrace_amd/csrc/sched_state.cpp:

```cpp

#include <new>

#include "sched_state.h"
#include "trace_kernels.h"
#include "trace_plan.h"

namespace ntr {

static constexpr size_t kTopTableBytes = (((size_t)2 << NTR_TOP_DEPTH_MAX) + 16) * 32;
static constexpr int kScratchSpares = 4;
static constexpr int kScratchLive = 16;

static std::atomic<DeviceState*> g_state[kMaxDevices];
static std::mutex g_stateMu;

int current_device_state(DeviceState** out, const char* what)
{
    int dev = 0;
    const hipError_t e = hipGetDevice(&dev);
    if (e != hipSuccess) return hip_fail(e, what);
    if (dev < 0 || dev >= kMaxDevices) return set_error(NTR_ERR_INVALID, "device index %d out of range", dev);
    DeviceState* ds = g_state[dev].load(std::memory_order_acquire);
    if (!ds) {
        std::lock_guard<std::mutex> lk(g_stateMu);
        ds = g_state[dev].load(std::memory_order_relaxed);
        if (!ds) {
            ds = new (std::nothrow) DeviceState();
            if (!ds) return set_error(NTR_ERR_NOMEM, "out of host memory (scheduling state of device %d)", dev);
            ds->device = dev;
            g_state[dev].store(ds, std::memory_order_release);
        }
    }
    *out = ds;
    return NTR_OK;
}

static int alloc_device_memory(DeviceState& s)
{
    const int dev = s.device;
    hipDeviceProp_t prop;
    NTR_HIP(hipGetDeviceProperties(&prop, dev));
    s.numCUs = prop.multiProcessorCount;
    NTR_HIP(hipMalloc((void**)&s.counters, (kNumCounters + kPinnedCounters) * kPoolHeadsMax * 64));
    NTR_HIP(hipMalloc((void**)&s.status, 64));
    NTR_HIP(hipMalloc((void**)&s.stats, 256));
    NTR_HIP(hipMemset(s.status, 0, 64));
    return NTR_OK;
}

int current_device_state_ready(DeviceState** out)
{
    int rc = current_device_state(out);
    if (rc != NTR_OK || (*out)->ready.load(std::memory_order_acquire)) return rc;
    DeviceState& s = **out;
    std::lock_guard<std::mutex> lk(s.mu);
    if (s.ready.load(std::memory_order_relaxed)) return NTR_OK;
    rc = alloc_device_memory(s);
    if (rc != NTR_OK) {
        if (s.counters) (void)hipFree(s.counters);
        if (s.status) (void)hipFree(s.status);
        if (s.stats) (void)hipFree(s.stats);
        s.counters = nullptr; s.status = nullptr; s.stats = nullptr;
        return rc;
    }
    s.ready.store(true, std::memory_order_release);
    return NTR_OK;
}

int status_fetch(DeviceState* ds, hipStream_t s, unsigned int* bits)
{
    *bits = 0;
    unsigned int st = 0;
    std::lock_guard<std::mutex> lk(ds->statusMu);
    const hipError_t xe = ntr_launch_status_exchange(ds->status, ds->status + 8, s);
    if (xe != hipSuccess) return hip_fail(xe, "status_exchange launch");
    NTR_HIP(hipMemcpyAsync(&st, ds->status + 8, sizeof(st), hipMemcpyDeviceToHost, s));
    NTR_HIP(hipStreamSynchronize(s));
    *bits = st;
    return NTR_OK;
}

int counter_set_take(DeviceState* ds, bool capturing, int32_t** out)
{
    std::lock_guard<std::mutex> lk(ds->mu);
    if (capturing) {
        if (ds->nextPinned >= kPinnedCounters)
            return set_error(NTR_ERR_NOMEM, "ntr_trace_bvh: more than %d persistent launches captured into HIP graphs", kPinnedCounters);
        *out = ds->counters + kPoolHeadsMax * 16 * (kNumCounters + ds->nextPinned++);
    } else {
        *out = ds->counters + kPoolHeadsMax * 16 * ds->next;
        ds->next = (ds->next + 1) % kNumCounters;
    }
    return NTR_OK;
}

int top_table_get(DeviceState* ds, const void* d_nodes, int64_t nodesBytes, hipStream_t s, bool rebuild, TopTable** out)
{
    std::lock_guard<std::mutex> lk(ds->mu);
    const bool capturing = stream_is_capturing(s);
    TopTable* t = nullptr;
    TopTable* lru = nullptr;
    for (auto& e : ds->top) {
        if (e.nodes == d_nodes && e.bytes == nodesBytes) { t = &e; break; }
        if (!e.pinned && (!lru || e.lastUse < lru->lastUse)) lru = &e;
    }
    bool build = rebuild;
    if (!t) {
        if (!lru) return set_error(NTR_ERR_NOMEM, "ntr_trace_bvh: every top-of-tree table is held by a captured HIP graph");
        if (capturing) return set_error(NTR_ERR_INVALID, "ntr_trace_bvh: first launch on a BVH cannot be captured (trace it once, or call ntr_bvh_validate, before capturing)");
        t = lru;
        if (!t->table) {
            NTR_HIP(hipMalloc(&t->table, kTopTableBytes));
            NTR_HIP(hipMalloc((void**)&t->count, sizeof(unsigned int)));
        }
        t->nodes = d_nodes; t->bytes = nodesBytes;
        build = true;
    }
    t->lastUse = ++ds->clock;
    if (capturing) t->pinned = true;
    if (build) {
        const hipError_t e = ntr_launch_top_table(d_nodes, (unsigned int)nodesBytes, tunables().predictDepth, t->table, t->count, s);
        if (e != hipSuccess) return hip_fail(e, "top_table launch");
    }
    *out = t;
    return NTR_OK;
}

int scratch_alloc(PredictScratch* p, int numBlocks)
{
    if (!p->classCount) {
        NTR_HIP(hipMalloc((void**)&p->classCount, NTR_SCHED_PRED_WORDS * sizeof(unsigned int)));
        NTR_HIP(hipMemset(p->classCount, 0, NTR_SCHED_PRED_WORDS * sizeof(unsigned int)));
    }
    if (p->capBlocks < numBlocks) {
        if (p->classList) { (void)hipFree(p->classList); (void)hipFree(p->order); p->classList = p->order = nullptr; p->capBlocks = 0; }
        NTR_HIP(hipMalloc((void**)&p->classList, (size_t)NTR_SCHED_PRED_CLASSES * numBlocks * sizeof(unsigned int)));
        NTR_HIP(hipMalloc((void**)&p->order, (size_t)numBlocks * sizeof(unsigned int)));
        p->capBlocks = numBlocks;
    }
    return NTR_OK;
}

static void scratch_free(PredictScratch* p)
{
    if (p->classCount) (void)hipFree(p->classCount);
    if (p->classList) (void)hipFree(p->classList);
    if (p->order) (void)hipFree(p->order);
    *p = PredictScratch();
}

static int scratch_count_spares(DeviceState* ds, int numBlocks)
{
    int n = 0;
    for (auto& e : ds->scratch)
        if (e.state == PredictScratch::SPARE && e.capBlocks >= numBlocks) n++;
    return n;
}

static int scratch_provision_spares(DeviceState* ds, int numBlocks, int want)
{
    int have = scratch_count_spares(ds, numBlocks);
    for (auto& e : ds->scratch) {
        if (have >= want) break;
        if (e.state == PredictScratch::SPARE && e.capBlocks < numBlocks) {
            const int rc = scratch_alloc(&e, numBlocks);
            if (rc != NTR_OK) return rc;
            have++;
        }
    }
    for (auto& e : ds->scratch) {
        if (have >= want) break;
        if (e.state != PredictScratch::FREE) continue;
        const int rc = scratch_alloc(&e, numBlocks);
        if (rc != NTR_OK) return rc;
        e.state = PredictScratch::SPARE;
        have++;
    }
    return NTR_OK;
}

int predict_scratch_get(DeviceState* ds, hipStream_t s, int numBlocks, PredictScratch** out)
{
    std::lock_guard<std::mutex> lk(ds->mu);
    const bool capturing = stream_is_capturing(s);
    if (capturing) {
        PredictScratch* best = nullptr;
        for (auto& e : ds->scratch)
            if (e.state == PredictScratch::SPARE && e.capBlocks >= numBlocks && (!best || e.capBlocks < best->capBlocks)) best = &e;
        if (!best) { *out = nullptr; return NTR_OK; }
        best->state = PredictScratch::PINNED;
        best->lastUse = ++ds->clock;
        *out = best;
        return NTR_OK;
    }
    PredictScratch* p = nullptr;
    PredictScratch* lru = nullptr;
    PredictScratch* empty = nullptr;
    int live = 0;
    for (auto& e : ds->scratch) {
        if (e.state == PredictScratch::LIVE) {
            live++;
            if (e.stream == (void*)s) { p = &e; break; }
            if (!lru || e.lastUse < lru->lastUse) lru = &e;
        } else if (e.state == PredictScratch::FREE && !empty) {
            empty = &e;
        }
    }
    if (!p) {
        p = (empty && live < kScratchLive) ? empty : (lru ? lru : empty);
        if (!p) return set_error(NTR_ERR_NOMEM, "ntr_trace_bvh: every prediction scratch is held by a captured HIP graph (ntr_trace_graph_release_all)");
        if (p->state == PredictScratch::LIVE) {
            NTR_HIP(hipDeviceSynchronize());
            scratch_free(p);
        }
    } else if (p->capBlocks < numBlocks && p->classList) {
        NTR_HIP(hipStreamSynchronize(s));
    }
    int rc = scratch_alloc(p, numBlocks);
    if (rc != NTR_OK) return rc;
    p->state = PredictScratch::LIVE;
    p->stream = (void*)s;
    p->lastUse = ++ds->clock;
    rc = scratch_provision_spares(ds, numBlocks, kScratchSpares);
    if (rc != NTR_OK) return rc;
    *out = p;
    return NTR_OK;
}

static void sched_hint_release(NtrSchedHint* h)
{
    if (h->order) (void)hipFree(h->order);
    if (h->cost) (void)hipFree(h->cost);
    h->order = h->cost = nullptr;
    h->numBlocks = 0; h->capBlocks = 0; h->uses = 0; h->valid = false; h->predicted = false;
}

int sched_hint_bind(NtrSchedHint* h, int numBlocks, int dev, hipStream_t s)
{
    if (h->device != dev || h->capBlocks < numBlocks || !h->order) {
        sched_hint_release(h);
        NTR_HIP(hipMalloc((void**)&h->order, ((size_t)numBlocks + 3) * sizeof(unsigned int)));
        NTR_HIP(hipMalloc((void**)&h->cost, (size_t)numBlocks * sizeof(unsigned int)));
        h->capBlocks = numBlocks;
        h->device = dev;
    }
    if (h->numBlocks != numBlocks) {
        h->numBlocks = numBlocks;
        h->uses = 0; h->valid = false; h->predicted = false;
        const hipError_t e = ntr_launch_identity_order(h->order, numBlocks, s);
        if (e != hipSuccess) return hip_fail(e, "identity_order launch");
    }
    return NTR_OK;
}

static void auto_hint_release_async(NtrSchedHint* h, hipStream_t s)
{
    if (h->order) (void)hipFreeAsync(h->order, s);
    if (h->cost) (void)hipFreeAsync(h->cost, s);
    h->order = h->cost = nullptr;
    h->numBlocks = 0; h->uses = 0; h->valid = false; h->predicted = false;
}

static AutoHint* auto_hint_lookup(DeviceState* ds, const void* d_rays, const void* d_nodes, int numRays, int anyHit, void* stream,
                                  NtrSchedHint** evicted, bool* noEntry)
{
    *evicted = nullptr;
    *noEntry = false;
    AutoHint* hit = nullptr;
    AutoHint* freeE = nullptr;
    for (auto& e : ds->autoHints) {
        if (e.used && e.rays == d_rays && e.nodes == d_nodes && e.numRays == numRays && e.anyHit == anyHit && e.stream == stream) { hit = &e; break; }
        if (!e.used && !freeE) freeE = &e;
    }
    if (hit) {
        hit->lastUse = ++ds->clock;
        hit->sightings++;
        return hit;
    }
    AutoHint* v = freeE;
    if (!v) {
        for (auto& e : ds->autoHints) {
            if (e.hint.order && e.stream != stream) continue;
            if (!v || e.lastUse < v->lastUse) v = &e;
        }
        if (!v) { *noEntry = true; return nullptr; }
        if (v->hint.order) *evicted = &v->hint;
    }
    v->rays = d_rays; v->nodes = d_nodes; v->numRays = numRays; v->anyHit = anyHit; v->stream = stream;
    v->used = true;
    v->sightings = 1;
    v->lastUse = ++ds->clock;
    v->hint.uses = 0; v->hint.valid = false;
    return nullptr;
}

int auto_hint_get(DeviceState* ds, const void* d_rays, const void* d_nodes, int numRays, int anyHit, hipStream_t s, int numBlocks,
                  NtrSchedHint** out)
{
    *out = nullptr;
    const int dev = ds->device;
    std::lock_guard<std::mutex> lk(ds->mu);
    NtrSchedHint* evicted = nullptr;
    bool noEntry = false;
    AutoHint* hit = auto_hint_lookup(ds, d_rays, d_nodes, numRays, anyHit, (void*)s, &evicted, &noEntry);
    if (evicted) auto_hint_release_async(evicted, s);
    if (!hit) return NTR_OK;
    NtrSchedHint* h = &hit->hint;
    if (h->numBlocks != numBlocks || h->device != dev) {
        if (h->order) auto_hint_release_async(h, s);
        unsigned int* order = nullptr;
        unsigned int* cost = nullptr;
        if (hipMallocAsync((void**)&order, ((size_t)numBlocks + 3) * sizeof(unsigned int), s) != hipSuccess) { (void)hipGetLastError(); return NTR_OK; }
        if (hipMallocAsync((void**)&cost, (size_t)numBlocks * sizeof(unsigned int), s) != hipSuccess) { (void)hipGetLastError(); (void)hipFreeAsync(order, s); return NTR_OK; }
        h->order = order; h->cost = cost;
        h->numBlocks = numBlocks;
        h->device = dev;
        h->uses = 0; h->valid = false;
        if (ntr_launch_identity_order(order, numBlocks, s) != hipSuccess) {
            (void)hipGetLastError();
            auto_hint_release_async(h, s);
            return NTR_OK;
        }
    }
    *out = h;
    return NTR_OK;
}

}

using namespace ntr;

extern "C" {

int ntr_top_table_refresh(const void* d_nodes, int64_t nodesBytes, void* stream)
{
    DeviceState* ds = nullptr;
    const int rc = current_device_state(&ds, "hipGetDevice(&dev)");
    if (rc != NTR_OK) return rc;
    TopTable* t = nullptr;
    return top_table_get(ds, d_nodes, nodesBytes, (hipStream_t)stream, true, &t);
}

int ntr_trace_graph_reserve(int32_t launches, int32_t numRays)
{
    if (launches < 0 || numRays < 0) return set_error(NTR_ERR_INVALID, "ntr_trace_graph_reserve: negative argument");
    DeviceState* ds = nullptr;
    int rc = current_device_state_ready(&ds);
    if (rc != NTR_OK) return rc;
    const int numBlocks = (numRays + 255) / 256;
    std::lock_guard<std::mutex> lk(ds->mu);
    if (numBlocks > 0 && launches > 0) {
        rc = scratch_provision_spares(ds, numBlocks, launches);
        if (rc != NTR_OK) return rc;
        if (scratch_count_spares(ds, numBlocks) < launches)
            return set_error(NTR_ERR_NOMEM, "ntr_trace_graph_reserve: at most %d prediction scratches exist (ntr_trace_graph_release_all returns the pinned ones)", kScratch);
    }
    return NTR_OK;
}

int ntr_trace_graph_release_all(void)
{
    DeviceState* ds = nullptr;
    const int rc = current_device_state(&ds, "hipGetDevice(&dev)");
    if (rc != NTR_OK) return rc;
    NTR_HIP(hipDeviceSynchronize());
    std::lock_guard<std::mutex> lk(ds->mu);
    for (auto& e : ds->scratch)
        if (e.state == PredictScratch::PINNED) e.state = PredictScratch::SPARE;
    for (auto& t : ds->top) t.pinned = false;
    ds->nextPinned = 0;
    return NTR_OK;
}

int ntr_stream_release(void* stream)
{
    DeviceState* ds = nullptr;
    const int rc = current_device_state(&ds, "hipGetDevice(&dev)");
    if (rc != NTR_OK) return rc;
    hipStream_t s = (hipStream_t)stream;
    if (stream_is_capturing(s)) return set_error(NTR_ERR_INVALID, "ntr_stream_release: the stream is being captured");
    NTR_HIP(hipStreamSynchronize(s));
    std::lock_guard<std::mutex> lk(ds->mu);
    for (auto& e : ds->autoHints)
        if (e.used && e.stream == stream) {
            if (e.hint.order) auto_hint_release_async(&e.hint, s);
            e = AutoHint();
        }
    for (auto& e : ds->scratch)
        if (e.state == PredictScratch::LIVE && e.stream == stream) scratch_free(&e);
    return NTR_OK;
}

int ntr_selftest_auto_hint_table(int32_t devices, int32_t keysPerDevice, int32_t rounds, int32_t* hintedLastRound)
{
    if (devices < 1 || devices > kMaxDevices || keysPerDevice < 1 || rounds < 1 || !hintedLastRound)
        return set_error(NTR_ERR_INVALID, "ntr_selftest_auto_hint_table: bad argument");
    for (int d = 0; d < devices; d++) hintedLastRound[d] = 0;
    DeviceState* fake = new (std::nothrow) DeviceState[devices];
    if (!fake) return set_error(NTR_ERR_NOMEM, "ntr_selftest_auto_hint_table: out of host memory");
    for (int r = 0; r < rounds; r++)
        for (int k = 0; k < keysPerDevice; k++)
            for (int d = 0; d < devices; d++) {
                NtrSchedHint* evicted = nullptr;
                bool noEntry = false;
                std::lock_guard<std::mutex> lk(fake[d].mu);
                AutoHint* hit = auto_hint_lookup(&fake[d], (const void*)(uintptr_t)(0x1000 + 64 * k), (const void*)(uintptr_t)0x10, 1 << 20, k & 1,
                                                 (void*)(uintptr_t)(d + 1), &evicted, &noEntry);
                if (hit) hit->hint.order = (unsigned int*)(uintptr_t)1;
                if (hit && r == rounds - 1) hintedLastRound[d]++;
            }
    delete[] fake;
    return NTR_OK;
}

int ntr_sched_hint_create(NtrSchedHint** out)
{
    if (!out) return set_error(NTR_ERR_INVALID, "ntr_sched_hint_create: null out");
    *out = new (std::nothrow) NtrSchedHint();
    return *out ? NTR_OK : set_error(NTR_ERR_NOMEM, "ntr_sched_hint_create: out of memory");
}

int ntr_sched_hint_destroy(NtrSchedHint* hint)
{
    if (!hint) return NTR_OK;
    sched_hint_release(hint);
    delete hint;
    return NTR_OK;
}

int ntr_sched_hint_reset(NtrSchedHint* hint)
{
    if (!hint) return set_error(NTR_ERR_INVALID, "ntr_sched_hint_reset: null hint");
    hint->uses = 0;
    hint->valid = false;
    hint->predicted = false;
    return NTR_OK;
}

int ntr_sched_hint_inspect(const NtrSchedHint* hint, NtrSchedHintState* state, uint32_t* h_order, uint32_t* h_cost, void* stream)
{
    if (!hint || !state) return set_error(NTR_ERR_INVALID, "ntr_sched_hint_inspect: null argument");
    if (hint->numBlocks == 0 && (h_order || h_cost)) return set_error(NTR_ERR_INVALID, "ntr_sched_hint_inspect: the hint is not bound (it has no arrays)");
    hipStream_t s = (hipStream_t)stream;
    if (hint->numBlocks > 0) {
        NTR_HIP(hipStreamSynchronize(s));
        if (h_order) NTR_HIP(hipMemcpyAsync(h_order, hint->order, ((size_t)hint->numBlocks + 3) * sizeof(unsigned int), hipMemcpyDeviceToHost, s));
        if (h_cost) NTR_HIP(hipMemcpyAsync(h_cost, hint->cost, (size_t)hint->numBlocks * sizeof(unsigned int), hipMemcpyDeviceToHost, s));
        if (h_order || h_cost) NTR_HIP(hipStreamSynchronize(s));
    }
    state->numBlocks = hint->numBlocks;
    state->device = hint->device;
    state->uses = hint->uses;
    state->valid = hint->valid ? 1 : 0;
    state->predicted = hint->predicted ? 1 : 0;
    return NTR_OK;
}

int ntr_sched_hint_predict(NtrSchedHint* hint, const uint32_t* d_blockCost, int32_t numBlocks, void* stream)
{
    if (!hint || !d_blockCost || numBlocks < 1) return set_error(NTR_ERR_INVALID, "ntr_sched_hint_predict: bad argument");
    hipStream_t s = (hipStream_t)stream;
    int dev = 0;
    NTR_HIP(hipGetDevice(&dev));
    if (hint->numBlocks != numBlocks || hint->device != dev) {
        const int rc = sched_hint_bind(hint, numBlocks, dev, s);
        if (rc != NTR_OK) return rc;
    }
    NTR_HIP(hipMemcpyAsync(hint->cost, d_blockCost, (size_t)numBlocks * sizeof(unsigned int), hipMemcpyDeviceToDevice, s));
    hipError_t le = ntr_launch_sched_order(hint->cost, numBlocks, tunables().schedClasses, hint->order, 0, s);
    if (le == hipSuccess) le = ntr_launch_zero_words(hint->order + numBlocks, 3, s);
    if (le != hipSuccess) return hip_fail(le, "sched_order launch");
    hint->uses = 0;
    hint->valid = true;
    hint->predicted = true;
    return NTR_OK;
}

}
```

ntrace_amd/csrc/sched_state.h:

```cpp
#pragma once
#include <hip/hip_runtime.h>

#include <atomic>
#include <mutex>

#include "ntr_internal.h"

struct NtrSchedHint {
    unsigned int* order = nullptr;
    unsigned int* cost = nullptr;
    int numBlocks = 0;
    int capBlocks = 0;
    int device = -1;
    int uses = 0;
    bool valid = false;
    bool predicted = false;
};

namespace ntr {

struct TopTable {
    const void* nodes = nullptr;
    int64_t bytes = 0;
    void* table = nullptr;
    unsigned int* count = nullptr;
    unsigned long long lastUse = 0;
    bool pinned = false;
};
constexpr int kTopTables = 16;

struct PredictScratch {
    enum State { FREE = 0, LIVE, SPARE, PINNED };
    State state = FREE;
    void* stream = nullptr;
    unsigned int* classCount = nullptr;
    unsigned int* classList = nullptr;
    unsigned int* order = nullptr;
    int capBlocks = 0;
    unsigned long long lastUse = 0;
};
constexpr int kScratch = 48;

struct AutoHint {
    const void* rays = nullptr;
    const void* nodes = nullptr;
    void* stream = nullptr;
    int numRays = 0, anyHit = 0;
    bool used = false;
    int sightings = 0;
    unsigned long long lastUse = 0;
    NtrSchedHint hint;
};
constexpr int kAutoHints = 96;

constexpr int kNumCounters = 64;
constexpr int kPinnedCounters = 192;

struct DeviceState {
    int device = -1;
    std::mutex mu;
    std::atomic<bool> ready{false};
    int numCUs = 0;
    int32_t* counters = nullptr;
    unsigned int* status = nullptr;
    unsigned long long* stats = nullptr;
    int next = 0;
    int nextPinned = 0;
    unsigned long long clock = 0;
    TopTable top[kTopTables];
    PredictScratch scratch[kScratch];
    AutoHint autoHints[kAutoHints];
    std::mutex queryMu;
    PredictScratch query;
    std::mutex statusMu;
};

int current_device_state(DeviceState** out, const char* what = "hipGetDevice");
int current_device_state_ready(DeviceState** out);
int status_fetch(DeviceState* ds, hipStream_t s, unsigned int* bits);

int top_table_get(DeviceState* ds, const void* d_nodes, int64_t nodesBytes, hipStream_t s, bool rebuild, TopTable** out);
int scratch_alloc(PredictScratch* p, int numBlocks);
int predict_scratch_get(DeviceState* ds, hipStream_t s, int numBlocks, PredictScratch** out);
int auto_hint_get(DeviceState* ds, const void* d_rays, const void* d_nodes, int numRays, int anyHit, hipStream_t s, int numBlocks, NtrSchedHint** out);
int sched_hint_bind(NtrSchedHint* h, int numBlocks, int dev, hipStream_t s);
int counter_set_take(DeviceState* ds, bool capturing, int32_t** out);

}
```

ntrace_amd/csrc/trace_kernels.h:

```cpp
#pragma once
#include <hip/hip_runtime.h>
#include <stdint.h>

#include "ntrace_amd.h"

#ifndef NTR_TRACE_WAVES_PER_BLOCK
#define NTR_TRACE_WAVES_PER_BLOCK 4
#endif
#ifndef NTR_TRACE_MIN_WAVES_PER_SIMD
#define NTR_TRACE_MIN_WAVES_PER_SIMD 1
#endif
#ifndef NTR_TRACE_PERSISTENT_MIN_WAVES_PER_SIMD
#define NTR_TRACE_PERSISTENT_MIN_WAVES_PER_SIMD 1
#endif

#define NTR_VARIANT_PERRAY 0
#define NTR_VARIANT_PERSISTENT 1
#define NTR_VARIANT_PERRAY_STATS 2
#define NTR_VARIANT_PERSISTENT_UNIFIED 5
#define NTR_VARIANT_PERRAY_UNIFIED_W1 6
#define NTR_MINIPOOL_MAX_K 16
#define NTR_VARIANT_PERRAY_UNIFIED_MINI 7

#define NTR_ROUTE_SKIP_COHERENT 1
#define NTR_ROUTE_SKIP_INCOHERENT 2
#define NTR_BATCH_WORD_K(w) ((w) & 0xFFFFu)
#define NTR_BATCH_WORD_INCOHERENT(w) (NTR_BATCH_WORD_K(w) > 1u || ((w) & NTR_BATCH_DIVERGENT) != 0u)

#define NTR_STATUS_STACK_OVERFLOW 1u


namespace ntr {

struct TraceParams {
    int32_t numRays;
    int32_t anyHit;
    const NtrRay* rays;
    NtrRayResult* results;
    const void* nodes;
    const void* woop;
    uint32_t nodesBytes;
    uint32_t woopBytes;
    const int32_t* triIndex;
    int32_t* counter;
    unsigned int* status;
    int32_t chunk;
    int32_t shardRays;
    int32_t numHeads;
    int32_t numBlocks;
    int32_t numBlocksIncoherent;
    int32_t numBlocksDivergent;
    int32_t orderBlocks;
    int32_t fetchThreshold;
    int32_t wholeWave;
    int32_t prefetchAfter;
    uint32_t bvhFlags;
    int32_t leafSwitchBelow;
    int32_t octant;
    int32_t flatFetch;
    int32_t uniformPrologue;
    int32_t certainSteps;
    int32_t certainDescent;
    int32_t splitSlice;
    const unsigned int* order;
    unsigned int* cost;
    unsigned long long* stats;
    const unsigned int* poolK;
    int32_t poolKConst;
    int32_t routeSkip;
};

}

extern "C" hipError_t ntr_launch_trace(int variant, const ntr::TraceParams* p, int numBlocks, hipStream_t stream);
#define NTR_TOP_DEPTH_MAX 10
#define NTR_SCHED_PRED_CLASSES 64
#define NTR_SCHED_PRED_WORDS (NTR_SCHED_PRED_CLASSES + 3)
extern "C" hipError_t ntr_launch_top_table(const void* d_nodes, unsigned int nodesBytes, int depth, void* d_table,
                                           unsigned int* d_tableCount, hipStream_t stream);
extern "C" hipError_t ntr_launch_predict(const void* d_rays, int numRays, int numBlocks, const void* d_table,
                                         const unsigned int* d_tableCount, unsigned int* d_classCount, unsigned int* d_classList,
                                         unsigned int* d_order, unsigned int* d_poolKCopy, int poolKWide, hipStream_t stream);
extern "C" hipError_t ntr_launch_predict_costs(const void* d_rays, int numRays, int numBlocks, const void* d_table,
                                               const unsigned int* d_tableCount, unsigned int* d_blockCost, hipStream_t stream);
extern "C" hipError_t ntr_launch_coherence(const void* d_rays, int numRays, int numBlocks, const void* d_table, const unsigned int* d_tableCount,
                                           unsigned int* d_out, int poolKWide, hipStream_t stream);
extern "C" hipError_t ntr_launch_leaf_depth_level(const void* d_nodes, unsigned int nodesBytes, const void* d_woop, unsigned int woopVec4, const int* d_triIndex,
                                                  int numTris, const unsigned int* d_qin, const unsigned int* d_nIn, unsigned int* d_qout, unsigned int* d_nOut,
                                                  unsigned int capacity, unsigned int gridThreads, int depth, int* d_depthByTri, hipStream_t stream);
extern "C" hipError_t ntr_launch_secondary_block_costs(const void* d_inResults, int first, int count, int numSamples, const int* d_depthByTri, int numTris,
                                                       unsigned int* d_blockCost, hipStream_t stream);
extern "C" hipError_t ntr_launch_zero_words(void* d_ptr, int words, hipStream_t stream);
extern "C" hipError_t ntr_launch_status_exchange(unsigned int* d_status, unsigned int* d_out, hipStream_t stream);
extern "C" hipError_t ntr_launch_sched_order(const unsigned int* d_cost, int numBlocks, int classes, unsigned int* d_order,
                                             int keepIfAllZero, hipStream_t stream);
extern "C" hipError_t ntr_launch_identity_order(unsigned int* d_order, int numBlocks, hipStream_t stream);
extern "C" hipError_t ntr_launch_selftest_division(const float* d_x, const float* d_d, int nx, int nd,
                                                   unsigned int* d_mismatches, hipStream_t stream);
extern "C" hipError_t ntr_launch_selftest_division_hard(int xe0, int de0, unsigned long long* d_counts, hipStream_t stream);
```

ntrace_amd/csrc/trace_plan.h:

```cpp
#pragma once
#include <stdint.h>
#include <string.h>

#include "ntrace_amd.h"
#include "ntr_internal.h"
#include "trace_kernels.h"

namespace ntr {

static constexpr int kPoolHeadsMax = 1024;

struct TraceBatchDesc {
    int variant;
    bool dynamicFetch;
    int32_t numRays;
    bool anyHit;
    int64_t nodesBytes, triWoopBytes;
    uint64_t nodesAddr, woopAddr;
    uint32_t bvhFlags;
    bool wantStats;
    bool capturing;
    bool callerHint;
    int numCUs;
};

typedef NtrTracePlan TracePlan;

inline int minipool_wide(const Tunables& tun, int64_t nodesBytes, int numRays)
{
    if (tun.minipoolWide >= 2 && tun.minipoolWide <= NTR_MINIPOOL_MAX_K) return tun.minipoolWide;
    return (nodesBytes >= (int64_t)32 << 20 && numRays >= (3 << 19)) ? 4 : 2;
}

inline TracePlan plan_trace(const Tunables& tun, const TraceBatchDesc& b)
{
    TracePlan pl;
    memset(&pl, 0, sizeof(pl));
    pl.chunk = tun.chunk;
    {
        const uint64_t an = b.nodesAddr, aw = b.woopAddr;
        const uint64_t lo = an < aw ? an : aw;
        const uint64_t hiN = an + (uint64_t)b.nodesBytes, hiW = aw + (uint64_t)b.triWoopBytes;
        const bool oneWindow = ((hiN > hiW ? hiN : hiW) - lo) <= 0xFFFFFFFFull;
        pl.flatFetch = (tun.flatFetch != 0 && b.nodesBytes >= 64 && b.triWoopBytes >= 64 && oneWindow) ? 1 : 0;
    }
    pl.uniformPrologue = tun.uniformPrologue != 0 ? 1 : 0;
    pl.wholeWave = tun.wholeWave != 0 ? 1 : 0;
    pl.prefetchAfter = tun.prefetchAfter;
    pl.splitSlice = tun.splitSlice > 0 ? tun.splitSlice : 0;
    pl.leafSwitchBelow = tun.leafSwitchBelow >= 0 ? tun.leafSwitchBelow : (b.anyHit ? 24 : 32);
    pl.octant = tun.octant;
    pl.numHeads = 8;
    pl.poolKConst = 1;
    pl.minipoolWide = minipool_wide(tun, b.nodesBytes, b.numRays);
    pl.orderBlocks = (b.numRays + 255) / 256;
    const bool bigEnough = b.numRays >= tun.predictMinRays && b.nodesBytes >= (int64_t)tun.predictMinNodes * 64 && tun.predict != 0;

    pl.variant = b.wantStats ? NTR_VARIANT_PERRAY_STATS : b.variant;

    const bool route = tun.route != 0 && !b.wantStats;
    if (route && b.variant == NTR_VARIANT_PERSISTENT && b.anyHit) {
        pl.variant = NTR_VARIANT_PERRAY;
        pl.coherentRoute = 2;
    }
    const bool routedPersistentName = route && b.variant == NTR_VARIANT_PERSISTENT && !b.anyHit && bigEnough && (256 % pl.chunk) == 0 &&
                                      tun.minipool < 0 && tun.predictPersistent != 0;
    const bool persistentDynamic = (b.variant == NTR_VARIANT_PERSISTENT && !routedPersistentName) ? b.dynamicFetch : true;
    pl.unified = persistentDynamic && tun.unified != 0;
    pl.persistentFetchThreshold = tun.fetchThreshold >= 0 ? tun.fetchThreshold : (persistentDynamic ? (pl.unified ? 48 : 24) : 0);
    pl.fetchThreshold = pl.persistentFetchThreshold;

    constexpr int blockThreads = NTR_TRACE_WAVES_PER_BLOCK * 64;
    auto persistent_grid = [&]() {
        const int blocksPerCU = tun.blocksPerCU;
        pl.persistentBlocks = b.numCUs * blocksPerCU;
        const int needed = (b.numRays + blockThreads - 1) / blockThreads;
        if (pl.persistentBlocks > needed) pl.persistentBlocks = needed;
        const int chunksTotal = (b.numRays + pl.chunk - 1) / pl.chunk;
        pl.numHeads = tun.poolHeads < 8 ? 8 : (tun.poolHeads > kPoolHeadsMax ? kPoolHeadsMax : tun.poolHeads & ~7);
        if (persistentDynamic && tun.blocksPerCUIncoherent > 0 && tun.blocksPerCUIncoherent < blocksPerCU) {
            pl.numBlocksIncoherent = b.numCUs * tun.blocksPerCUIncoherent;
            if (pl.numBlocksIncoherent > pl.persistentBlocks) pl.numBlocksIncoherent = pl.persistentBlocks;
        }
        if (persistentDynamic && tun.blocksPerCUDivergent > 0 && tun.blocksPerCUDivergent < blocksPerCU) {
            pl.numBlocksDivergent = b.numCUs * tun.blocksPerCUDivergent;
            if (pl.numBlocksDivergent > pl.persistentBlocks) pl.numBlocksDivergent = pl.persistentBlocks;
        }
        pl.shardRays = ((chunksTotal + pl.numHeads - 1) / pl.numHeads) * pl.chunk;
        pl.persistentVariant = pl.unified ? NTR_VARIANT_PERSISTENT_UNIFIED : NTR_VARIANT_PERSISTENT;
    };
    if (pl.variant == NTR_VARIANT_PERSISTENT) {
        persistent_grid();
        pl.numBlocks = pl.persistentBlocks;
    } else {
        pl.numBlocks = (b.numRays + blockThreads - 1) / blockThreads;
    }
    pl.hintable = pl.variant == NTR_VARIANT_PERRAY || (pl.variant == NTR_VARIANT_PERSISTENT && (256 % pl.chunk) == 0 && tun.persistentHints != 0);
    pl.useAutoHint = !b.callerHint && !b.wantStats && tun.autoHint != 0 && pl.hintable && b.numRays >= tun.autoHintMinRays && !b.capturing;

    pl.persistentOrder = pl.variant == NTR_VARIANT_PERSISTENT && tun.predictPersistent != 0 && (256 % pl.chunk) == 0;
    pl.predictable = (pl.variant == NTR_VARIANT_PERRAY || pl.persistentOrder) && !b.anyHit && bigEnough;
    pl.probeOnRefresh = pl.variant == NTR_VARIANT_PERRAY && !b.anyHit && tun.minipool < 0 && bigEnough;

    pl.launchVariant = pl.variant;
    pl.launchBlocks = pl.numBlocks;
    if (pl.variant == NTR_VARIANT_PERSISTENT) pl.launchVariant = pl.persistentVariant;
    if (pl.variant == NTR_VARIANT_PERRAY) {
        pl.launchVariant = NTR_VARIANT_PERRAY_UNIFIED_W1;
        pl.launchBlocks = pl.numBlocks * 4;
        if (tun.minipool != 0 && !b.anyHit) {
            pl.launchVariant = NTR_VARIANT_PERRAY_UNIFIED_MINI;
            pl.minipool = true;
            pl.fetchThreshold = tun.minipoolThreshold;
            pl.poolKConst = tun.minipool > 0 ? tun.minipool : 1;
            pl.poolKFromDevice = tun.minipool < 0;
        }
    }

    if (route && !b.anyHit && bigEnough && (256 % pl.chunk) == 0) {
        if (pl.variant == NTR_VARIANT_PERRAY && pl.launchVariant == NTR_VARIANT_PERRAY_UNIFIED_MINI && pl.poolKFromDevice) {
            pl.coherentRoute = 1;
            persistent_grid();
        } else if (pl.variant == NTR_VARIANT_PERSISTENT && tun.minipool < 0 && pl.predictable) {
            pl.coherentRoute = 1;
        }
    }
    if (pl.coherentRoute == 1) {
        pl.perrayBlocks = pl.orderBlocks * 4;
        pl.perrayFetchThreshold = tun.minipoolThreshold;
    }
    return pl;
}

struct HintStep {
    bool zeroK;
    bool refresh;
    bool useOrder;
};
inline HintStep plan_hint_step(const Tunables& tun, bool valid, bool predicted, int uses)
{
    HintStep h;
    const bool firstOfPrediction = predicted && valid;
    h.zeroK = uses == 0 && !firstOfPrediction;
    const int every = tun.schedRefreshEvery;
    const long long late = 4ll * every;
    h.refresh = uses < 3 || every <= 1 || (uses < late ? (uses == every || uses == 2 * every) : (uses % late) == 0);
    if (firstOfPrediction) h.refresh = false;
    h.useOrder = valid;
    return h;
}

}
```

Baseline: 17040.

## Skip redundant routed trace launch using host-mirrored coherence belief

Prediction and coherence kernels now write their batch coherence word, tagged with a generation number, into host-mapped coherent pinned memory. When routing is active, the host polls this mirror and launches only the per-ray or only the persistent trace kernel, instead of both kernels where each skips the other's work. A generation counter invalidates stale beliefs whenever the hint is reset, rebound or re-predicted. The belief lags by at least one call, so a wrong guess still gives correct results but takes the unrouted path. Launch counters and selftest entry points are also added.

```diff
diff --git a/include/ntrace_amd.h b/include/ntrace_amd.h
--- a/include/ntrace_amd.h
+++ b/include/ntrace_amd.h
@@ -117,6 +117,8 @@
                            uint64_t triWoopAddr, int64_t triWoopBytes, uint32_t bvhFlags, int32_t numCUs, int32_t flags,
                            NtrTracePlan* plan);
 NTR_API int ntr_trace_plan_hint_step(int32_t valid, int32_t predicted, int32_t uses, int32_t out[3]);
+NTR_API int ntr_trace_plan_sides(int32_t coherentRoute, int32_t persistent, int32_t capturing, int32_t belief, int32_t out[4]);
+NTR_API int ntr_trace_launch_counts(uint64_t out[4]);
 NTR_API int ntr_trace_plan_certain(int32_t anyHit, int32_t out[2]);
 
 NTR_API int ntr_tunables_reload(void);
@@ -155,6 +157,8 @@
     int32_t predicted;
 } NtrSchedHintState;
 NTR_API int ntr_sched_hint_inspect(const NtrSchedHint* hint, NtrSchedHintState* state, uint32_t* h_order, uint32_t* h_cost, void* stream);
+NTR_API int ntr_sched_hint_route(const NtrSchedHint* hint, int32_t* belief);
+NTR_API int ntr_selftest_hint_mirror(uint32_t word, int32_t out[5]);
 
 typedef struct NtrTraceStats {
     int64_t numRays;
diff --git a/ntrace_amd/__init__.py b/ntrace_amd/__init__.py
--- a/ntrace_amd/__init__.py
+++ b/ntrace_amd/__init__.py
@@ -2,7 +2,7 @@
                     lib_path, query_config, sah_build, trace_bvh, trace_bvh_stats, pixel_table,
                     raygen_primary, raygen_ao, raygen_shadow, count_hits, selftest_division, selftest_division_hard, bvh_leaf_depths, secondary_block_costs, lbvh_capacity,
                     lbvh_build, LbvhResult, hlbvh_build, HlbvhResult, reconstruct, ray_morton_sort, camera_decode, camera_reencode,
-                    camera_nscreen_to_world, obj_load, SchedHint, trace_status, trace_plan, trace_plan_hint_step, trace_plan_certain, TracePlan, set_tunables, host_bvh_wrap, use_library, trace_graph_reserve, trace_graph_release_all, stream_release, selftest_auto_hint_table, selftest_gather_rate, frame_shard, frame_ao_batches, DistGroup,
+                    camera_nscreen_to_world, obj_load, SchedHint, trace_status, trace_plan, trace_plan_hint_step, trace_plan_certain, trace_plan_sides, trace_launch_counts, selftest_hint_mirror, TracePlan, set_tunables, host_bvh_wrap, use_library, trace_graph_reserve, trace_graph_release_all, stream_release, selftest_auto_hint_table, selftest_gather_rate, frame_shard, frame_ao_batches, DistGroup,
                     lbvh_release_workspace, predict_block_costs, predict_batch_coherence, predict_dispatch_order, SchedHintState,
                     HostKdtree, kdtree_build, host_kdtree_wrap, trace_kdtree, KDTREE_SPATIAL_MEDIAN, KDTREE_SAH,
                     DeviceKdtree, KdtreeDeviceParams, kdtree_device_build, kdtree_device_params, KDTREE_DEVICE_DEFAULTS,
diff --git a/ntrace_amd/_capi.py b/ntrace_amd/_capi.py
--- a/ntrace_amd/_capi.py
+++ b/ntrace_amd/_capi.py
@@ -175,6 +175,8 @@
     ("ntr_trace_plan", C.c_int, [C.c_char_p, _i32, _i32, C.c_uint64, _i64, C.c_uint64, _i64, _u32, _i32, _i32, _vp]),
     ("ntr_trace_plan_hint_step", C.c_int, [_i32, _i32, _i32, C.POINTER(_i32 * 3)]),
     ("ntr_trace_plan_certain", C.c_int, [_i32, C.POINTER(_i32 * 2)]),
+    ("ntr_trace_plan_sides", C.c_int, [_i32, _i32, _i32, _i32, C.POINTER(_i32 * 4)]),
+    ("ntr_trace_launch_counts", C.c_int, [C.POINTER(C.c_uint64 * 4)]),
     ("ntr_selftest_gather_rate", C.c_int, [_i64, _i32, _i32, _i32, _vp, C.POINTER(C.c_float)]),
     ("ntr_frame_shard", C.c_int, [_i32, _i32, _i32, _i32, C.POINTER(_i32), C.POINTER(_i32)]),
     ("ntr_frame_ao_batches", C.c_int, [_i32, _i32, _i32, _i32, C.POINTER(_i32), C.POINTER(_i32), _i32, C.POINTER(_i32)]),
@@ -202,6 +204,8 @@
     ("ntr_sched_hint_reset", C.c_int, [_vp]),
     ("ntr_sched_hint_predict", C.c_int, [_vp, _vp, _i32, _vp]),
     ("ntr_sched_hint_inspect", C.c_int, [_vp, _vp, _vp, _vp, _vp]),
+    ("ntr_sched_hint_route", C.c_int, [_vp, C.POINTER(_i32)]),
+    ("ntr_selftest_hint_mirror", C.c_int, [_u32, C.POINTER(_i32 * 5)]),
     ("ntr_secondary_block_costs", C.c_int, [_vp, _i32, _i32, _i32, _vp, _i32, _vp, _vp]),
     ("ntr_bvh_leaf_depths", C.c_int, [_vp, _i64, _vp, _i64, _vp, _i32, _vp, C.POINTER(_i32), _vp]),
     ("ntr_selftest_division", C.c_int, [_vp, _i32, _vp, _i32, C.POINTER(_u32), _vp]),
@@ -328,6 +332,11 @@
             out["order"], out["words"], out["cost"] = order[:st.numBlocks], order[st.numBlocks:], cost
         return out
 
+    def route(self):
+        belief = _i32(-1)
+        _check(lib().ntr_sched_hint_route(self._h, C.byref(belief)))
+        return int(belief.value)
+
     def close(self):
         if self._h:
             lib().ntr_sched_hint_destroy(self._h)
@@ -380,6 +389,24 @@
     out = (_i32 * 3)()
     _check(lib().ntr_trace_plan_hint_step(int(bool(valid)), int(bool(predicted)), int(uses), C.byref(out)))
     return dict(zeroK=bool(out[0]), refresh=bool(out[1]), useOrder=bool(out[2]))
+
+
+def trace_plan_sides(coherent_route, persistent, capturing, belief):
+    out = (_i32 * 4)()
+    _check(lib().ntr_trace_plan_sides(int(coherent_route), int(bool(persistent)), int(bool(capturing)), int(belief), C.byref(out)))
+    return dict(perray=bool(out[0]), persistent=bool(out[1]), perraySkip=int(out[2]), persistentSkip=int(out[3]))
+
+
+def selftest_hint_mirror(word):
+    out = (_i32 * 5)()
+    _check(lib().ntr_selftest_hint_mirror(int(word), C.byref(out)))
+    return [int(v) for v in out]
+
+
+def trace_launch_counts():
+    out = (C.c_uint64 * 4)()
+    _check(lib().ntr_trace_launch_counts(C.byref(out)))
+    return dict(bodies=int(out[0]), skipBodies=int(out[1]), zeroWords=int(out[2]), schedOrder=int(out[3]))
 
 
 def trace_plan_certain(any_hit):
diff --git a/ntrace_amd/csrc/ntr_api.cpp b/ntrace_amd/csrc/ntr_api.cpp
--- a/ntrace_amd/csrc/ntr_api.cpp
+++ b/ntrace_amd/csrc/ntr_api.cpp
@@ -1,6 +1,7 @@
 
 #include <hip/hip_runtime.h>
 
+#include <atomic>
 #include <cstdarg>
 #include <cstdio>
 #include <cstring>
@@ -84,6 +85,21 @@
     return bd;
 }
 
+enum { kCountBodies = 0, kCountSkipBodies, kCountZeroWords, kCountSchedOrder, kCounts };
+static std::atomic<uint64_t> g_launchCounts[kCounts];
+static void count_launch(int what) { g_launchCounts[what].fetch_add(1, std::memory_order_relaxed); }
+static hipError_t zero_words_counted(void* d_ptr, int words, hipStream_t s)
+{
+    count_launch(kCountZeroWords);
+    return ntr_launch_zero_words(d_ptr, words, s);
+}
+static hipError_t trace_counted(int variant, const TraceParams* p, int numBlocks, hipStream_t s)
+{
+    count_launch(kCountBodies);
+    if (p->routeSkip != 0) count_launch(kCountSkipBodies);
+    return ntr_launch_trace(variant, p, numBlocks, s);
+}
+
 struct TraceLaunch {
     TraceParams p{};
     TraceParams pp{};
@@ -93,6 +109,8 @@
     bool probeCoherence = false;
     TopTable* predTable = nullptr;
     PredictScratch* predScratch = nullptr;
+    unsigned long long* mirror = nullptr;
+    unsigned int generation = 0;
 };
 
 static int bind_trace(DeviceState* ds, const Tunables& tun, const TracePlan& pl, bool capturing, int64_t nodesBytes, hipStream_t s,
@@ -111,17 +129,20 @@
             rc = sched_hint_bind(hint, orderBlocks, ds->device, s);
             if (rc != NTR_OK) return rc;
         }
+        rc = sched_hint_mirror_ensure(hint, s);
+        if (rc != NTR_OK) return rc;
         const HintStep hs = plan_hint_step(tun, hint->valid, hint->predicted, hint->uses);
         if (hs.zeroK) {
-            const hipError_t zk = ntr_launch_zero_words(hint->order + orderBlocks, 3, s);
+            const hipError_t zk = zero_words_counted(hint->order + orderBlocks, 3, s);
             if (zk != hipSuccess) return hip_fail(zk, "zero_words launch");
+            sched_hint_start_over(hint);
         }
         L->refresh = hs.refresh;
         hint->predicted = false;
         hint->uses++;
         if (hs.useOrder) p.order = hint->order;
         if (L->refresh) {
-            const hipError_t ze = ntr_launch_zero_words(hint->cost, orderBlocks, s);
+            const hipError_t ze = zero_words_counted(hint->cost, orderBlocks, s);
             if (ze != hipSuccess) return hip_fail(ze, "zero_words launch");
             p.cost = hint->cost;
         }
@@ -145,9 +166,13 @@
     if (L->predScratch) word = L->predScratch->classCount + NTR_SCHED_PRED_CLASSES + 2;
     else if (hint && pl.hintable && hint->numBlocks == orderBlocks && hint->order) word = hint->order + orderBlocks + 2;
     const bool routed = pl.coherentRoute == 1 && word != nullptr;
-    L->persistentSide = variant == NTR_VARIANT_PERSISTENT || routed;
-    L->perraySide = variant != NTR_VARIANT_PERSISTENT || routed;
-    if ((pl.minipool && pl.poolKFromDevice) || L->persistentSide) p.poolK = word;
+    if (hint && pl.hintable && !capturing) { L->mirror = hint->mirror; L->generation = hint->generation; }
+    int belief = -1;
+    if (routed && !L->predScratch && tun.routeBelief != 0) belief = sched_hint_poll(hint);
+    const RouteSides sides = plan_route_sides(routed ? 1 : (pl.coherentRoute == 1 ? 0 : pl.coherentRoute), variant == NTR_VARIANT_PERSISTENT, capturing, belief);
+    L->persistentSide = sides.persistent;
+    L->perraySide = sides.perray;
+    if ((pl.minipool && pl.poolKFromDevice) || L->persistentSide || routed) p.poolK = word;
 
     TraceParams& pp = L->pp = p;
     if (L->persistentSide) {
@@ -160,10 +185,10 @@
             pp.orderBlocks = orderBlocks;
             pp.shardRays = ((orderBlocks + pp.numHeads - 1) / pp.numHeads) * 256;
         }
-        pp.routeSkip = routed ? NTR_ROUTE_SKIP_COHERENT : 0;
+        pp.routeSkip = sides.persistentSkip;
     }
     if (routed) {
-        p.routeSkip = NTR_ROUTE_SKIP_INCOHERENT;
+        p.routeSkip = sides.perraySkip;
         if (variant == NTR_VARIANT_PERSISTENT) { p.fetchThreshold = pl.perrayFetchThreshold; p.poolKConst = 1; }
     }
     return NTR_OK;
@@ -184,27 +209,29 @@
     if (L.predScratch) {
         const hipError_t pe = ntr_launch_predict(p.rays, p.numRays, orderBlocks, L.predTable->table, L.predTable->count, L.predScratch->classCount,
                                                  L.predScratch->classList, (hint && pl.hintable) ? hint->order : L.predScratch->order,
-                                                 (hint && pl.hintable) ? hint->order + orderBlocks + 2 : nullptr, pl.minipoolWide, s);
+                                                 (hint && pl.hintable) ? hint->order + orderBlocks + 2 : nullptr, pl.minipoolWide,
+                                                 L.mirror, L.generation, s);
         if (pe != hipSuccess) return hip_fail(pe, "predict launch");
     } else if (L.probeCoherence) {
         const hipError_t ce = ntr_launch_coherence(p.rays, p.numRays, orderBlocks, L.predTable->table, L.predTable->count, hint->order + orderBlocks,
-                                                  pl.minipoolWide, s);
+                                                  pl.minipoolWide, L.mirror, L.generation, s);
         if (ce != hipSuccess) return hip_fail(ce, "coherence launch");
     }
     hipError_t le = hipSuccess;
     if (L.persistentSide) {
-        le = ntr_launch_zero_words(L.pp.counter, kPoolHeadsMax * 16, s);
+        le = zero_words_counted(L.pp.counter, kPoolHeadsMax * 16, s);
         if (le != hipSuccess) return hip_fail(le, "zero_words launch");
-        le = ntr_launch_trace(pl.persistentVariant, &L.pp, pl.persistentBlocks, s);
+        le = trace_counted(pl.persistentVariant, &L.pp, pl.persistentBlocks, s);
         if (le != hipSuccess) return hip_fail(le, "trace_bvh launch");
     }
     if (L.perraySide) {
-        le = pl.variant == NTR_VARIANT_PERSISTENT ? ntr_launch_trace(NTR_VARIANT_PERRAY_UNIFIED_MINI, &p, pl.perrayBlocks, s)
-                                                  : ntr_launch_trace(pl.launchVariant, &p, pl.launchBlocks, s);
+        le = pl.variant == NTR_VARIANT_PERSISTENT ? trace_counted(NTR_VARIANT_PERRAY_UNIFIED_MINI, &p, pl.perrayBlocks, s)
+                                                  : trace_counted(pl.launchVariant, &p, pl.launchBlocks, s);
         if (le != hipSuccess) return hip_fail(le, "trace_bvh launch");
     }
     if (seconds) NTR_HIP(ev.record(1));
     if (L.refresh) {
+        count_launch(kCountSchedOrder);
         le = ntr_launch_sched_order(hint->cost, orderBlocks, tun.schedClasses, hint->order, 1, s);
         if (le != hipSuccess) return hip_fail(le, "sched_order launch");
         hint->valid = true;
@@ -315,6 +342,7 @@
     t.poolHeads = env_int("NTR_TRACE_POOL_HEADS", 128);
     t.autoHint = env_int("NTR_TRACE_AUTO_HINT", 1);
     t.autoHintMinRays = env_int("NTR_TRACE_AUTO_HINT_MIN_RAYS", 1 << 17);
+    t.routeBelief = env_int("NTR_TRACE_ROUTE_BELIEF", 1);
     t.route = env_int("NTR_TRACE_ROUTE", 1);
     t.persistentHints = env_int("NTR_TRACE_PERSISTENT_HINTS", 1);
     t.predict = env_int("NTR_TRACE_PREDICT", 1);
@@ -479,6 +507,21 @@
     return NTR_OK;
 }
 
+int ntr_trace_plan_sides(int32_t coherentRoute, int32_t persistent, int32_t capturing, int32_t belief, int32_t out[4])
+{
+    if (!out) return set_error(NTR_ERR_INVALID, "ntr_trace_plan_sides: null argument");
+    const RouteSides r = plan_route_sides(coherentRoute, persistent != 0, capturing != 0, belief);
+    out[0] = r.perray; out[1] = r.persistent; out[2] = r.perraySkip; out[3] = r.persistentSkip;
+    return NTR_OK;
+}
+
+int ntr_trace_launch_counts(uint64_t out[4])
+{
+    if (!out) return set_error(NTR_ERR_INVALID, "ntr_trace_launch_counts: null argument");
+    for (int i = 0; i < kCounts; i++) out[i] = g_launchCounts[i].load(std::memory_order_relaxed);
+    return NTR_OK;
+}
+
 int ntr_trace_status(void* stream, uint32_t* statusBits)
 {
     if (statusBits) *statusBits = 0;
@@ -531,7 +574,7 @@
     const int rc = query_table("ntr_predict_batch_coherence", d_nodes, nodesBytes, (hipStream_t)stream, &ds, &t);
     if (rc != NTR_OK) return rc;
     const hipError_t e = ntr_launch_coherence(d_rays, numRays, (numRays + 255) / 256, t->table, t->count, d_out, minipool_wide(tunables(), nodesBytes, numRays),
-                                              (hipStream_t)stream);
+                                              nullptr, 0u, (hipStream_t)stream);
     if (e != hipSuccess) return hip_fail(e, "coherence launch");
     return NTR_OK;
 }
@@ -554,7 +597,7 @@
     rc = scratch_alloc(p, numBlocks);
     if (rc != NTR_OK) return rc;
     const hipError_t e = ntr_launch_predict(d_rays, numRays, numBlocks, t->table, t->count, p->classCount, p->classList, d_order, d_word,
-                                            minipool_wide(tunables(), nodesBytes, numRays), s);
+                                            minipool_wide(tunables(), nodesBytes, numRays), nullptr, 0u, s);
     if (e != hipSuccess) return hip_fail(e, "predict launch");
     NTR_HIP(hipStreamSynchronize(s));
     return NTR_OK;
diff --git a/ntrace_amd/csrc/ntr_internal.h b/ntrace_amd/csrc/ntr_internal.h
--- a/ntrace_amd/csrc/ntr_internal.h
+++ b/ntrace_amd/csrc/ntr_internal.h
@@ -11,7 +11,7 @@
 
 struct Tunables {
     int chunk, fetchThreshold, leafSwitchBelow, blocksPerCU, blocksPerCUIncoherent, blocksPerCUDivergent, poolHeads, octant, unified, flatFetch, uniformPrologue, certainSteps, certainDescent, splitSlice, wholeWave, prefetchAfter, minipool, minipoolThreshold, minipoolWide;
-    int autoHint, autoHintMinRays, persistentHints, route, predict, predictPersistent, predictDepth, predictMinRays, predictMinNodes;
+    int autoHint, autoHintMinRays, persistentHints, route, routeBelief, predict, predictPersistent, predictDepth, predictMinRays, predictMinNodes;
     int schedRefreshEvery, schedClasses;
     int lbvhSplit, lbvhAggLds, lbvhAggStaged, lbvhSortItems;
 };
diff --git a/ntrace_amd/csrc/sched_kernels.hip b/ntrace_amd/csrc/sched_kernels.hip
--- a/ntrace_amd/csrc/sched_kernels.hip
+++ b/ntrace_amd/csrc/sched_kernels.hip
@@ -132,6 +132,12 @@
 
 constexpr int FLATTEN_THREADS = 1024;
 
+__device__ __forceinline__ void mirror_store(unsigned long long* mirror, unsigned int generation, unsigned int word)
+{
+    if (!mirror) return;
+    *(volatile unsigned long long*)mirror = ((unsigned long long)word << 32) | (unsigned long long)generation;
+    __threadfence_system();
+}
 __device__ __forceinline__ unsigned int pool_k(unsigned int originApart, unsigned int divergenceScore, int numBlocks, int poolKWide)
 {
     const unsigned int k = (originApart > 0u && 2u * originApart >= (unsigned int)numBlocks) ? (unsigned int)poolKWide : 1u;
@@ -139,7 +145,8 @@
 }
 __global__ __launch_bounds__(FLATTEN_THREADS) void flatten_kernel(unsigned int* __restrict__ classCount, const unsigned int* __restrict__ classList,
                                                                   int numBlocks, unsigned int* __restrict__ order,
-                                                                  unsigned int* __restrict__ poolKCopy, int poolKWide)
+                                                                  unsigned int* __restrict__ poolKCopy, int poolKWide,
+                                                                  unsigned long long* mirror, unsigned int generation)
 {
     __shared__ unsigned int s_end[NTR_SCHED_PRED_CLASSES];
     const int tid = threadIdx.x;
@@ -148,7 +155,7 @@
         classCount[NTR_SCHED_PRED_CLASSES] = 0;
         classCount[NTR_SCHED_PRED_CLASSES + 1] = 0;
         classCount[NTR_SCHED_PRED_CLASSES + 2] = k;
-        if (poolKCopy) *poolKCopy = k;
+        if (poolKCopy) { *poolKCopy = k; mirror_store(mirror, generation, k); }
     }
     if (tid < 64) {
         static_assert(NTR_SCHED_PRED_CLASSES == 64, "one class per lane");
@@ -186,9 +193,14 @@
     if ((threadIdx.x & 63) == 0 && m1) atomicAdd(&out[0], (unsigned int)__popcll(m1));
     if ((threadIdx.x & 63) == 0 && (m2 | m3)) atomicAdd(&out[1], 4u * (unsigned int)__popcll(m2) + (unsigned int)__popcll(m3));
 }
-__global__ void coherence_finish_kernel(unsigned int* __restrict__ out, int numBlocks, int poolKWide)
-{
-    if (threadIdx.x == 0 && blockIdx.x == 0) out[2] = pool_k(out[0], out[1], numBlocks, poolKWide);
+__global__ void coherence_finish_kernel(unsigned int* __restrict__ out, int numBlocks, int poolKWide, unsigned long long* mirror,
+                                        unsigned int generation)
+{
+    if (threadIdx.x == 0 && blockIdx.x == 0) {
+        const unsigned int k = pool_k(out[0], out[1], numBlocks, poolKWide);
+        out[2] = k;
+        mirror_store(mirror, generation, k);
+    }
 }
 
 __global__ __launch_bounds__(256) void identity_order_kernel(unsigned int* __restrict__ order, int n)
@@ -285,13 +297,14 @@
 
 extern "C" hipError_t ntr_launch_predict(const void* d_rays, int numRays, int numBlocks, const void* d_table,
                                          const unsigned int* d_tableCount, unsigned int* d_classCount, unsigned int* d_classList,
-                                         unsigned int* d_order, unsigned int* d_poolKCopy, int poolKWide, hipStream_t stream)
+                                         unsigned int* d_order, unsigned int* d_poolKCopy, int poolKWide, unsigned long long* d_mirror,
+                                         unsigned int generation, hipStream_t stream)
 {
     const int grid = (numBlocks + 63) / 64;
     hipLaunchKernelGGL(ntr::predict_kernel, dim3(grid), dim3(ntr::PRED_WAVES * 64), 0, stream, (const float4*)d_rays, numRays, numBlocks,
                        (const float4*)d_table, d_tableCount, d_classCount, d_classList, (unsigned int*)nullptr);
     hipLaunchKernelGGL(ntr::flatten_kernel, dim3(1), dim3(ntr::FLATTEN_THREADS), 0, stream, d_classCount, (const unsigned int*)d_classList,
-                       numBlocks, d_order, d_poolKCopy, poolKWide);
+                       numBlocks, d_order, d_poolKCopy, poolKWide, d_mirror, generation);
     return hipGetLastError();
 }
 
@@ -305,13 +318,14 @@
 }
 
 extern "C" hipError_t ntr_launch_coherence(const void* d_rays, int numRays, int numBlocks, const void* d_table, const unsigned int* d_tableCount,
-                                           unsigned int* d_out, int poolKWide, hipStream_t stream)
+                                           unsigned int* d_out, int poolKWide, unsigned long long* d_mirror, unsigned int generation,
+                                           hipStream_t stream)
 {
     hipLaunchKernelGGL(ntr::zero_words_kernel, dim3(1), dim3(256), 0, stream, d_out, 3);
     if (numBlocks > 0)
         hipLaunchKernelGGL(ntr::coherence_kernel, dim3((numBlocks + 255) / 256), dim3(256), 0, stream, (const float4*)d_rays, numRays, numBlocks,
                            (const float4*)d_table, d_tableCount, d_out);
-    hipLaunchKernelGGL(ntr::coherence_finish_kernel, dim3(1), dim3(64), 0, stream, d_out, numBlocks, poolKWide);
+    hipLaunchKernelGGL(ntr::coherence_finish_kernel, dim3(1), dim3(64), 0, stream, d_out, numBlocks, poolKWide, d_mirror, generation);
     return hipGetLastError();
 }
 
diff --git a/ntrace_amd/csrc/sched_state.cpp b/ntrace_amd/csrc/sched_state.cpp
--- a/ntrace_amd/csrc/sched_state.cpp
+++ b/ntrace_amd/csrc/sched_state.cpp
@@ -1,4 +1,5 @@
 
+#include <cstring>
 #include <new>
 
 #include "sched_state.h"
@@ -45,6 +46,8 @@
     NTR_HIP(hipMalloc((void**)&s.status, 64));
     NTR_HIP(hipMalloc((void**)&s.stats, 256));
     NTR_HIP(hipMemset(s.status, 0, 64));
+    NTR_HIP(hipHostMalloc((void**)&s.autoMirrors, kAutoHints * sizeof(unsigned long long), hipHostMallocPortable | hipHostMallocMapped | hipHostMallocCoherent));
+    memset(s.autoMirrors, 0, kAutoHints * sizeof(unsigned long long));
     return NTR_OK;
 }
 
@@ -60,7 +63,8 @@
         if (s.counters) (void)hipFree(s.counters);
         if (s.status) (void)hipFree(s.status);
         if (s.stats) (void)hipFree(s.stats);
-        s.counters = nullptr; s.status = nullptr; s.stats = nullptr;
+        if (s.autoMirrors) (void)hipHostFree(s.autoMirrors);
+        s.counters = nullptr; s.status = nullptr; s.stats = nullptr; s.autoMirrors = nullptr;
         return rc;
     }
     s.ready.store(true, std::memory_order_release);
@@ -227,6 +231,28 @@
     return NTR_OK;
 }
 
+void sched_hint_start_over(NtrSchedHint* h)
+{
+    if (++h->generation == 0u) h->generation = 1u;
+    h->belief = -1;
+}
+
+int sched_hint_poll(NtrSchedHint* h)
+{
+    if (!h->mirror) return h->belief = -1;
+    const unsigned long long m = __atomic_load_n(h->mirror, __ATOMIC_RELAXED);
+    if ((unsigned int)m == h->generation) h->belief = NTR_BATCH_WORD_INCOHERENT((unsigned int)(m >> 32)) ? 1 : 0;
+    return h->belief;
+}
+
+int sched_hint_mirror_ensure(NtrSchedHint* h, hipStream_t s)
+{
+    if (h->mirror || stream_is_capturing(s)) return NTR_OK;
+    NTR_HIP(hipHostMalloc((void**)&h->mirror, sizeof(unsigned long long), hipHostMallocPortable | hipHostMallocMapped | hipHostMallocCoherent));
+    *h->mirror = 0ull;
+    return NTR_OK;
+}
+
 static void sched_hint_release(NtrSchedHint* h)
 {
     if (h->order) (void)hipFree(h->order);
@@ -243,10 +269,14 @@
         NTR_HIP(hipMalloc((void**)&h->cost, (size_t)numBlocks * sizeof(unsigned int)));
         h->capBlocks = numBlocks;
         h->device = dev;
-    }
+        sched_hint_start_over(h);
+    }
+    const int mrc = sched_hint_mirror_ensure(h, s);
+    if (mrc != NTR_OK) return mrc;
     if (h->numBlocks != numBlocks) {
         h->numBlocks = numBlocks;
         h->uses = 0; h->valid = false; h->predicted = false;
+        sched_hint_start_over(h);
         const hipError_t e = ntr_launch_identity_order(h->order, numBlocks, s);
         if (e != hipSuccess) return hip_fail(e, "identity_order launch");
     }
@@ -291,6 +321,7 @@
     v->sightings = 1;
     v->lastUse = ++ds->clock;
     v->hint.uses = 0; v->hint.valid = false;
+    sched_hint_start_over(&v->hint);
     return nullptr;
 }
 
@@ -316,6 +347,8 @@
         h->numBlocks = numBlocks;
         h->device = dev;
         h->uses = 0; h->valid = false;
+        h->mirror = ds->autoMirrors + (hit - ds->autoHints);
+        sched_hint_start_over(h);
         if (ntr_launch_identity_order(order, numBlocks, s) != hipSuccess) {
             (void)hipGetLastError();
             auto_hint_release_async(h, s);
@@ -384,7 +417,10 @@
     for (auto& e : ds->autoHints)
         if (e.used && e.stream == stream) {
             if (e.hint.order) auto_hint_release_async(&e.hint, s);
+            const unsigned int generation = e.hint.generation;
             e = AutoHint();
+            e.hint.generation = generation;
+            sched_hint_start_over(&e.hint);
         }
     for (auto& e : ds->scratch)
         if (e.state == PredictScratch::LIVE && e.stream == stream) scratch_free(&e);
@@ -413,6 +449,25 @@
     return NTR_OK;
 }
 
+int ntr_selftest_hint_mirror(uint32_t word, int32_t out[5])
+{
+    if (!out) return set_error(NTR_ERR_INVALID, "ntr_selftest_hint_mirror: null argument");
+    NtrSchedHint h;
+    unsigned long long m = 0;
+    h.mirror = &m;
+    out[0] = sched_hint_poll(&h);
+    m = ((unsigned long long)word << 32) | h.generation;
+    out[1] = sched_hint_poll(&h);
+    sched_hint_start_over(&h);
+    out[2] = sched_hint_poll(&h);
+    m = ((unsigned long long)word << 32) | h.generation;
+    out[3] = sched_hint_poll(&h);
+    h.generation = 0xFFFFFFFFu;
+    sched_hint_start_over(&h);
+    out[4] = (int32_t)h.generation;
+    return NTR_OK;
+}
+
 int ntr_sched_hint_create(NtrSchedHint** out)
 {
     if (!out) return set_error(NTR_ERR_INVALID, "ntr_sched_hint_create: null out");
@@ -424,6 +479,10 @@
 {
     if (!hint) return NTR_OK;
     sched_hint_release(hint);
+    if (hint->mirror) {
+        (void)hipDeviceSynchronize();
+        (void)hipHostFree(hint->mirror);
+    }
     delete hint;
     return NTR_OK;
 }
@@ -434,6 +493,7 @@
     hint->uses = 0;
     hint->valid = false;
     hint->predicted = false;
+    sched_hint_start_over(hint);
     return NTR_OK;
 }
 
@@ -470,10 +530,18 @@
     hipError_t le = ntr_launch_sched_order(hint->cost, numBlocks, tunables().schedClasses, hint->order, 0, s);
     if (le == hipSuccess) le = ntr_launch_zero_words(hint->order + numBlocks, 3, s);
     if (le != hipSuccess) return hip_fail(le, "sched_order launch");
+    sched_hint_start_over(hint);
     hint->uses = 0;
     hint->valid = true;
     hint->predicted = true;
     return NTR_OK;
 }
 
-}
+int ntr_sched_hint_route(const NtrSchedHint* hint, int32_t* belief)
+{
+    if (!hint || !belief) return set_error(NTR_ERR_INVALID, "ntr_sched_hint_route: null argument");
+    *belief = sched_hint_poll(const_cast<NtrSchedHint*>(hint));
+    return NTR_OK;
+}
+
+}
diff --git a/ntrace_amd/csrc/sched_state.h b/ntrace_amd/csrc/sched_state.h
--- a/ntrace_amd/csrc/sched_state.h
+++ b/ntrace_amd/csrc/sched_state.h
@@ -15,6 +15,9 @@
     int uses = 0;
     bool valid = false;
     bool predicted = false;
+    unsigned long long* mirror = nullptr;
+    unsigned int generation = 1;
+    int belief = -1;
 };
 
 namespace ntr {
@@ -73,6 +76,7 @@
     std::mutex queryMu;
     PredictScratch query;
     std::mutex statusMu;
+    unsigned long long* autoMirrors = nullptr;
 };
 
 int current_device_state(DeviceState** out, const char* what = "hipGetDevice");
@@ -84,6 +88,9 @@
 int predict_scratch_get(DeviceState* ds, hipStream_t s, int numBlocks, PredictScratch** out);
 int auto_hint_get(DeviceState* ds, const void* d_rays, const void* d_nodes, int numRays, int anyHit, hipStream_t s, int numBlocks, NtrSchedHint** out);
 int sched_hint_bind(NtrSchedHint* h, int numBlocks, int dev, hipStream_t s);
+void sched_hint_start_over(NtrSchedHint* h);
+int sched_hint_poll(NtrSchedHint* h);
+int sched_hint_mirror_ensure(NtrSchedHint* h, hipStream_t s);
 int counter_set_take(DeviceState* ds, bool capturing, int32_t** out);
 
 }
diff --git a/ntrace_amd/csrc/trace_kernels.h b/ntrace_amd/csrc/trace_kernels.h
--- a/ntrace_amd/csrc/trace_kernels.h
+++ b/ntrace_amd/csrc/trace_kernels.h
@@ -80,11 +80,13 @@
                                            unsigned int* d_tableCount, hipStream_t stream);
 extern "C" hipError_t ntr_launch_predict(const void* d_rays, int numRays, int numBlocks, const void* d_table,
                                          const unsigned int* d_tableCount, unsigned int* d_classCount, unsigned int* d_classList,
-                                         unsigned int* d_order, unsigned int* d_poolKCopy, int poolKWide, hipStream_t stream);
+                                         unsigned int* d_order, unsigned int* d_poolKCopy, int poolKWide, unsigned long long* d_mirror,
+                                         unsigned int generation, hipStream_t stream);
 extern "C" hipError_t ntr_launch_predict_costs(const void* d_rays, int numRays, int numBlocks, const void* d_table,
                                                const unsigned int* d_tableCount, unsigned int* d_blockCost, hipStream_t stream);
 extern "C" hipError_t ntr_launch_coherence(const void* d_rays, int numRays, int numBlocks, const void* d_table, const unsigned int* d_tableCount,
-                                           unsigned int* d_out, int poolKWide, hipStream_t stream);
+                                           unsigned int* d_out, int poolKWide, unsigned long long* d_mirror, unsigned int generation,
+                                           hipStream_t stream);
 extern "C" hipError_t ntr_launch_leaf_depth_level(const void* d_nodes, unsigned int nodesBytes, const void* d_woop, unsigned int woopVec4, const int* d_triIndex,
                                                   int numTris, const unsigned int* d_qin, const unsigned int* d_nIn, unsigned int* d_qout, unsigned int* d_nOut,
                                                   unsigned int capacity, unsigned int gridThreads, int depth, int* d_depthByTri, hipStream_t stream);
diff --git a/ntrace_amd/csrc/trace_plan.h b/ntrace_amd/csrc/trace_plan.h
--- a/ntrace_amd/csrc/trace_plan.h
+++ b/ntrace_amd/csrc/trace_plan.h
@@ -132,6 +132,25 @@
     return pl;
 }
 
+struct RouteSides {
+    bool perray, persistent;
+    int perraySkip, persistentSkip;
+};
+inline RouteSides plan_route_sides(int coherentRoute, bool persistent, bool capturing, int belief)
+{
+    RouteSides r;
+    r.perray = !persistent; r.persistent = persistent;
+    r.perraySkip = r.persistentSkip = 0;
+    if (coherentRoute != 1) return r;
+    if (capturing || (belief != 0 && belief != 1)) {
+        r.perray = r.persistent = true;
+        r.perraySkip = NTR_ROUTE_SKIP_INCOHERENT; r.persistentSkip = NTR_ROUTE_SKIP_COHERENT;
+    } else {
+        r.perray = belief == 0; r.persistent = belief == 1;
+    }
+    return r;
+}
+
 struct HintStep {
     bool zeroK;
     bool refresh;
```

After: 17160 (median of 6 runs). About the same (+0.7%).
